# pangenome/sweepga

Hardware: AMD Instinct MI355X
Metric: PAF mappings/sec through plane-sweep+scaffold filter, 1/2/4/8 MI355X (higher is better)
Workload: dtype u32 coordinates, f64 scores; 1 GPU; BASELINE.json configs[3] (synthetic 100 M mappings across 10 k (q,t) groups, 100-genome pangenome shape; S-pan in SURVEY.md 8d): 100000000 mappings per GPU over 9900 genome-pair groups (100 single-chromosome genomes), pipeline=default; flags=(defaults), mappings_per_gpu=100000000, groups_per_gpu=9900

## Files before the change

### sweepga_amd/csrc/swg_chain.hip

```cpp
#include <cmath>
#include <type_traits>

#include "swg_scaffold_internal.h"

namespace swg_scaf {
namespace {

__global__ __launch_bounds__(EW) void sortA_keys_kernel(uint64_t M, const uint32_t* __restrict__ a_idx,
                                                        const uint32_t* __restrict__ q_id,
                                                        const uint32_t* __restrict__ t_id,
                                                        const uint8_t* __restrict__ strand,
                                                        const uint32_t* __restrict__ q_start, uint32_t n_seq,
                                                        int pos_bits, uint64_t* __restrict__ key) {
  uint64_t a = (uint64_t)swg_xcd_block(blockIdx.x, gridDim.x) * EW + threadIdx.x;
  if (a >= M) return;
  const uint32_t i = a_idx[a];
  const uint64_t g = ((uint64_t)q_id[i] * n_seq + t_id[i]) * 2 + (strand[i] ? 1 : 0);
  key[a] = (g << pos_bits) | q_start[i];
}

__global__ __launch_bounds__(EW) void sortA_words_kernel(uint64_t M, const uint32_t* __restrict__ a_idx,
                                                         const uint32_t* __restrict__ q_id, const uint32_t* __restrict__ t_id,
                                                         const uint8_t* __restrict__ strand, uint32_t n_seq, int idx_bits,
                                                         uint64_t* __restrict__ words,
// ... 1417 lines not shown
                ld = d;
                lj2 = j;
              }
            }
          }
          if (!__any(in)) break;
        }
        uint64_t cand = __ballot(lj2 != NONE);
        while (cand) {
          const int l = __builtin_ctzll(cand);
          cand &= cand - 1;
          const uint64_t d = readlane_u64(ld, l);
          const uint32_t j = readlane_u32(lj2, l);
          if (d < best_d || (d == best_d && j < best_j)) {
            best_d = d;
            best_j = j;
          }
        }
      }
      if (best_j == NONE) continue;
      const bool in_ring = best_j - base < (uint32_t)BIGW;
      if (lane == 0) {
        if (in_ring) ring[best_j % BIGW] = best_d;
        __hip_atomic_store(best_j < be ? &own[best_j] : &prev[best_j], best_d, __ATOMIC_RELAXED, __HIP_MEMORY_SCOPE_AGENT);
        (best_j < be ? pred_own : pred_prev)[best_j] = i;
      }
      if (!in_ring) __builtin_amdgcn_fence(__ATOMIC_RELEASE, "workgroup");
      }
    }
  }
}


static int walk_plain_knob() {
  const char* e = getenv("SWG_WALK_PLAIN");
  return e && e[0] == '1';
}

constexpr int WALK_HASH = 256;

__device__ __forceinline__ void wave_lds_sync() {
  __builtin_amdgcn_fence(__ATOMIC_RELEASE, "wavefront");
  __builtin_amdgcn_s_waitcnt(0xc07f);
  __builtin_amdgcn_wave_barrier();
  __builtin_amdgcn_fence(__ATOMIC_ACQUIRE, "wavefront");
}

template <int BIGW, bool FUSED, bool SPEC>
__global__ __launch_bounds__(64) void chain_walk_kernel(uint32_t n_blocks, const SpecBlock* __restrict__ desc, uint32_t m,
                                                        const uint64_t* __restrict__ s_grp,
                                                        const uint32_t* __restrict__ s_qs,
                                                        const uint32_t* __restrict__ s_qe,
                                                        const uint32_t* __restrict__ s_ts,
                                                        const uint32_t* __restrict__ s_te,
                                                        const uint32_t* __restrict__ s_gidx,
                                                        const uint32_t* __restrict__ group_begin, uint32_t n_groups,
                                                        uint64_t max_gap, const unsigned long long* __restrict__ c_d,
                                                        const uint32_t* __restrict__ c_j, const uint32_t* __restrict__ c_n,
                                                        unsigned long long* own, unsigned long long* prev,
                                                        uint32_t* __restrict__ pred_own, uint32_t* __restrict__ pred_prev,
                                                        unsigned long long* __restrict__ wstats,
                                                        const uint32_t* __restrict__ n_blocks_dev = nullptr,
                                                        const uint32_t* __restrict__ gate = nullptr,
                                                        int walk_plain_lists = 0) {
  constexpr bool spec = SPEC;
  if (gate && *gate == 0) return;
  if (n_blocks_dev) n_blocks = min(n_blocks, *n_blocks_dev);
  const bool pair_desc = s_gidx == nullptr;
  __shared__ unsigned long long ring[BIGW];
  __shared__ uint32_t rq[BIGW], rt[BIGW], re[BIGW];
  __shared__ uint32_t hcnt[WALK_HASH];
  __shared__ uint32_t hnum[WALK_HASH];
  __shared__ unsigned long long l_fd[64];
  __shared__ uint32_t l_fj[64];
  const int lane = threadIdx.x;
  const uint64_t INF = ~0ull;
  const uint64_t fifth = max_gap / 5;
  const uint32_t gap32 = max_gap > 0xffffffffull ? 0xffffffffu : (uint32_t)max_gap;
  const uint32_t fifth32 = fifth > 0xffffffffull ? 0xffffffffu : (uint32_t)fifth;
  const bool wrap = max_gap == ~0ull;
  const bool can_cut = max_gap < (uint64_t(1) << 31);
  const bool fast_keys = max_gap <= (uint64_t(1) << 22) && !walk_plain_lists;
  for (int k = lane; k < WALK_HASH; k += 64) {
    hcnt[k] = 0xffffffffu;
    hnum[k] = 0;
  }
  wave_lds_sync();
  for (uint32_t bk = blockIdx.x; bk < n_blocks; bk += gridDim.x) {
    const SpecBlock D = desc[bk];
    const uint32_t b = D.bb, be = D.be, ue = D.ue;
    if (be <= b || ue - b < 2) continue;
    if (!SPEC && pair_desc && be - b >= LABEL_CAP_ELEMS) continue;
    auto view_ptr = [&](uint32_t p) -> unsigned long long* { return (spec && p >= be) ? &prev[p] : &own[p]; };
    auto view_load = [&](uint32_t p) -> uint64_t {
      return __hip_atomic_load(view_ptr(p), __ATOMIC_RELAXED, __HIP_MEMORY_SCOPE_AGENT);
    };
    uint32_t base = b;
    bool far_any = SPEC;
    wave_lds_sync();
    for (uint32_t p = b + lane; p < b + BIGW; p += 64) {
      const bool ok = p < ue;
      ring[p % BIGW] = (ok && SPEC) ? view_load(p) : INF;
      rq[p % BIGW] = ok ? s_qs[p] : 0xffffffffu;
      rt[p % BIGW] = ok ? s_ts[p] : 0u;
      re[p % BIGW] = ok ? s_te[p] : 0u;
    }
    wave_lds_sync();
    auto current = [&](uint32_t j) -> uint64_t {
      if (j - base < (uint32_t)BIGW) return ring[j % BIGW];
      return far_any ? view_load(j) : INF;
    };
    struct Pre {
      uint64_t view;
      uint32_t q, t, e;
      uint64_t bd[KC];
      uint32_t bj[KC];
      uint32_t nv;
      uint32_t qe, ts, te, minus, ei;
    };
    auto prefetch = [&](uint32_t i0n, uint32_t base_n, bool refill) {
      Pre P;
      P.view = INF;
      P.q = 0xffffffffu;
      P.t = P.e = 0;
      if (refill) {
        const uint32_t pn = base_n + BIGW - 64 + lane;
        if (pn < ue) {
          if (far_any) P.view = view_load(pn);
          P.q = s_qs[pn];
          P.t = s_ts[pn];
          P.e = s_te[pn];
        }
      }
      const uint32_t i = i0n + lane;
      const bool valid = i < be && i + 1 < ue;
#pragma unroll
      for (int c = 0; c < KC; ++c) {
        P.bd[c] = INF;
        P.bj[c] = NONE;
      }
      P.nv = 0;
      P.qe = P.ts = P.te = P.minus = 0;
      P.ei = ue;
      if (valid) {
        if (!spec && !pair_desc) {
          const uint32_t g = s_gidx[i];
          const uint32_t ge = (g + 1 < n_groups) ? group_begin[g + 1] : m;
          if (ge < P.ei) P.ei = ge;
        }
        if (FUSED) {
          P.qe = s_qe[i];
          P.ts = s_ts[i];
          P.te = s_te[i];
          P.minus = pair_desc ? D.pad : (uint32_t)(s_grp[i] & 1ull);
        } else {
#pragma unroll
          for (int c = 0; c < KC; ++c) {
            P.bd[c] = c_d[(uint64_t)c * m + i];
            P.bj[c] = c_j[(uint64_t)c * m + i];
          }
          P.nv = c_n[i];
        }
      }
      return P;
    };
    Pre cur = prefetch(b, base, false);
    bool far_dirty = false;
    for (uint32_t i0 = b; i0 < be && i0 + 1 < ue; i0 += 64) {
      if (i0 != b) {
        const uint32_t pn = base + BIGW + lane;
        if (far_dirty && pn < ue) cur.view = view_load(pn);
        far_dirty = false;
        wave_lds_sync();
        ring[pn % BIGW] = cur.view;
        rq[pn % BIGW] = cur.q;
        rt[pn % BIGW] = cur.t;
        re[pn % BIGW] = cur.e;
        base += 64;
        wave_lds_sync();
      }
      const bool more = i0 + 64 < be && i0 + 65 < ue;
      Pre nxt = cur;
      if (more) nxt = prefetch(i0 + 64, base + 64, true);
      const uint32_t i = i0 + lane;
      const bool valid = i < be && i + 1 < ue;
      uint64_t bd[KC];
      uint32_t bj[KC];
      uint32_t nv = cur.nv;
#pragma unroll
      for (int c = 0; c < KC; ++c) {
        bd[c] = cur.bd[c];
        bj[c] = cur.bj[c];
      }
      const uint32_t e_i = cur.ei;
      bool listed = false;
      uint32_t j_next = i + 1;
      bool open_next = valid;
      if (FUSED && fast_keys) {
        const uint32_t qe_i = cur.qe;
        const bool minus = cur.minus != 0;
        const uint64_t bound64 = (uint64_t)qe_i + max_gap;
        const uint32_t bound = bound64 > 0xffffffffull ? 0xffffffffu : (uint32_t)bound64;
        const uint32_t r_i = minus ? cur.ts : cur.te;
        const uint32_t* r_ring = minus ? re : rt;
        const uint32_t e_ring = min(e_i, base + (uint32_t)BIGW);
        constexpr uint64_t KEY_INF = 0x7ff0000000000000ull, KEY_BIT = 1ull << 62;
        double kb[KC];
#pragma unroll
        for (int c = 0; c < KC; ++c) kb[c] = __longlong_as_double((long long)KEY_INF);
        uint32_t off = 1, cnt = 0, sl = ((i + 1) % BIGW) * 4u;
        const uint32_t off_end = e_ring > i ? e_ring - i : 0u;
        uint32_t gap_v = gap32, fifth_v = fifth32, key_hi = (uint32_t)(KEY_BIT >> 32);
        asm volatile("" : "+v"(gap_v), "+v"(fifth_v), "+v"(key_hi));
        const char* const rq_b = reinterpret_cast<const char*>(rq);
        const char* const rr_b = reinterpret_cast<const char*>(r_ring);
        bool open = valid;
        for (;;) {
          const bool in = open && off < off_end;
          if (__ballot(in) == 0ull) break;
          uint32_t qs_j = *reinterpret_cast<const uint32_t*>(rq_b + sl), r_j = *reinterpret_cast<const uint32_t*>(rr_b + sl);
          asm volatile("" : "+v"(qs_j), "+v"(r_j));
          const bool inw = in && qs_j <= bound;
          open = open && !(in && qs_j > bound);
          const uint32_t q_gap = absdiff_vv(qs_j, qe_i), r_gap = absdiff_vv(r_j, r_i);
          const uint32_t lim_q = qs_j < qe_i ? fifth_v : gap_v;
          const uint32_t lim_r = ((r_j > r_i) != minus) ? gap_v : fifth_v;
          const bool ok = inw && q_gap <= lim_q && r_gap <= lim_r;
          const uint32_t qa = q_gap << 8, ra = r_gap << 8;
          const uint64_t add = ((uint64_t)key_hi << 32) | off;
          uint64_t key = (uint64_t)qa * qa + ((uint64_t)ra * ra + add);
          key = ok ? key : KEY_INF;
          cnt += ok ? 1u : 0u;
          const uint32_t step = in ? 1u : 0u;
          off += step;
          sl = (sl + (step << 2)) & (BIGW * 4u - 1u);
          double t = __longlong_as_double((long long)key);
#pragma unroll
          for (int c = 0; c < KC; ++c) {
            double hi = t;
            if (c + 1 < KC) asm("v_max_f64 %0, %1, %2" : "=v"(hi) : "v"(kb[c]), "v"(t));
            asm("v_min_f64 %0, %0, %1" : "+v"(kb[c]) : "v"(t));
            t = hi;
          }
        }
        const uint32_t j = i + off;
        nv = cnt < (uint32_t)KC + 1u ? cnt : (uint32_t)KC + 1u;
#pragma unroll
        for (int c = 0; c < KC; ++c) {
          const uint64_t bits = (uint64_t)__double_as_longlong(kb[c]);
          const bool none = bits == KEY_INF;
          bd[c] = none ? INF : (bits & ~KEY_BIT) >> 16;
          bj[c] = none ? NONE : i + (uint32_t)(bits & 0xffffu);
        }
        listed = true;
        j_next = j;
        open_next = open;
      }
      if (FUSED && valid && (!listed || (open_next && j_next < e_i))) {
        const uint32_t qe_i = cur.qe;
        const bool minus = cur.minus != 0;
        const uint64_t bound64 = (uint64_t)qe_i + max_gap;
        const uint32_t bound = bound64 > 0xffffffffull ? 0xffffffffu : (uint32_t)bound64;
        const uint32_t r_i = minus ? cur.ts : cur.te;
        const uint32_t* r_ring = minus ? re : rt;
        const uint32_t* __restrict__ r_mem = minus ? s_te : s_ts;
        auto consider = [&](uint32_t j, uint32_t qs_j, uint32_t r_j) {
          const uint32_t q_gap = absdiff_vv(qs_j, qe_i), r_gap = absdiff_vv(r_j, r_i);
          const uint32_t lim_q = qs_j >= qe_i ? gap32 : fifth32;
          const uint32_t lim_r = (minus ? r_j <= r_i : r_j >= r_i) ? gap32 : fifth32;
          if ((q_gap > lim_q) | (r_gap > lim_r)) return;
          const uint64_t d = (uint64_t)q_gap * q_gap + (uint64_t)r_gap * r_gap;
          if (nv <= (uint32_t)KC) ++nv;
          if (d < bd[KC - 1]) {
            uint64_t cd = d;
            uint32_t cj = j;
            bool placed = false;
#pragma unroll
            for (int c = 0; c < KC; ++c) {
              if (placed || cd < bd[c]) {
                placed = true;
                const uint64_t td = bd[c];
                const uint32_t tj = bj[c];
                bd[c] = cd;
                bj[c] = cj;
                cd = td;
                cj = tj;
              }
            }
          }
        };
        const uint32_t e_ring = listed ? j_next : min(e_i, base + (uint32_t)BIGW);
        uint32_t j = j_next;
        bool open = true;
        for (; j < e_ring; ++j) {
          uint32_t qs_j = rq[j % BIGW], r_j = r_ring[j % BIGW];
          asm volatile("" : "+v"(qs_j), "+v"(r_j));
          if (qs_j > bound) {
            open = false;
            break;
          }
          consider(j, qs_j, r_j);
        }
        if (open)
          for (; j < e_i; ++j) {
            const uint32_t qs_j = s_qs[j];
            if (qs_j > bound) break;
            consider(j, qs_j, r_mem[j]);
          }
      }
      uint32_t acc = 0;
#pragma unroll
      for (int c = 0; c < KC; ++c)
        if ((uint32_t)c < nv && bd[c] < current(bj[c])) acc |= 1u << c;
      uint64_t fd = INF;
      uint32_t fj = NONE;
#pragma unroll
      for (int c = KC - 1; c >= 0; --c)
        if (acc & (1u << c)) {
          fd = bd[c];
          fj = bj[c];
        }
      constexpr bool PAIR_TEST = SPEC;
      const uint32_t hs = fj & (WALK_HASH - 1);
      if (fj != NONE) {
        atomicMin(&hcnt[hs], (uint32_t)lane);
        if (PAIR_TEST) atomicAdd(&hnum[hs], 1u);
      }
      if (PAIR_TEST) {
        l_fd[lane] = fd;
        l_fj[lane] = fj;
      }
      wave_lds_sync();
      bool shared_j = false;
      if (fj != NONE) {
        const uint32_t low = hcnt[hs];
        if (low != (uint32_t)lane) shared_j = !PAIR_TEST || hnum[hs] > 2u || (l_fj[low] == fj && (uint64_t)l_fd[low] <= fd);
      }
      wave_lds_sync();
      if (fj != NONE) {
        hcnt[hs] = 0xffffffffu;
        if (PAIR_TEST) hnum[hs] = 0;
      }
      uint64_t work = __ballot(shared_j || (fj == NONE && nv > (uint32_t)KC));
      if (wstats && lane == 0) {
        atomicAdd(&wstats[0], 1ull);
        atomicAdd(&wstats[1], (unsigned long long)__popcll(work));
      }
      uint32_t committed = 0;
      auto commit = [&](uint32_t upto) {
        const bool me = (uint32_t)lane >= committed && (uint32_t)lane < upto && fj != NONE;
        const bool inr = me && (fj - base < (uint32_t)BIGW);
        if (inr) atomicMin(&ring[fj % BIGW], (unsigned long long)fd);
        wave_lds_sync();
        if (inr && (uint64_t)ring[fj % BIGW] == fd) {
          ((spec && fj >= be) ? pred_prev : pred_own)[fj] = i;
          if (spec && fj >= be)
            __hip_atomic_store(&prev[fj], fd, __ATOMIC_RELAXED, __HIP_MEMORY_SCOPE_AGENT);
        }
        uint64_t far = __ballot(me && !inr);
        if (far) {
          far_dirty = true;
          if (!far_any) {
            for (uint32_t p = base + BIGW + lane; p < ue; p += 64) own[p] = INF;
            __threadfence();
            far_any = true;
          }
        }
        while (far) {
          const int l = __builtin_ctzll(far);
          far &= far - 1;
          if (lane == l) {
            const unsigned long long old = atomicMin(view_ptr(fj), (unsigned long long)fd);
            if (old > fd) ((spec && fj >= be) ? pred_prev : pred_own)[fj] = i;
          }
        }
        committed = upto;
      };
      while (work) {
        const int l = __builtin_ctzll(work);
        work &= work - 1;
        const uint32_t nv_l = readlane_u32(nv, l), acc_l = readlane_u32(acc, l);
        uint64_t nd = INF;
        uint32_t nj = NONE;
        const uint64_t lower = l ? (~0ull >> (64 - l)) : 0ull;
#pragma unroll
        for (int c = 0; c < KC; ++c) {
          if (nj == NONE && (acc_l & (1u << c))) {
            const uint64_t d = readlane_u64(bd[c], l);
            const uint32_t j = readlane_u32(bj[c], l);
            if ((__ballot(fj == j && fd <= d) & lower) == 0) {
              nd = d;
              nj = j;
            }
          }
        }
        if (nj == NONE && nv_l > (uint32_t)KC) {
          commit((uint32_t)l);
          if (wstats && lane == 0) atomicAdd(&wstats[2], 1ull);
          const uint32_t ii = i0 + l;
          const uint64_t qe_l = s_qe[ii], ts_l = s_ts[ii], te_l = s_te[ii];
          const bool minus_l = pair_desc ? D.pad != 0 : (s_grp[ii] & 1ull) != 0;
          const uint32_t e_l = readlane_u32(e_i, l);
          const uint64_t bound = qe_l + max_gap;
          uint64_t ld = INF;
          uint32_t lj2 = NONE;
          for (uint32_t j0 = ii + 1; j0 < e_l; j0 += 64) {
            if (wstats && lane == 0) atomicAdd(&wstats[3], 1ull);
            if (can_cut) {
              const uint64_t wmin = wave_min_u64(ld);
              const uint64_t q0 = (j0 - base) < (uint32_t)BIGW ? (uint64_t)rq[j0 % BIGW] : (uint64_t)s_qs[j0];
              if (wmin != INF && q0 >= qe_l && (q0 - qe_l) * (q0 - qe_l) >= wmin) break;
            }
            const uint32_t j = j0 + lane;
            bool in = j < e_l;
            const bool inring = in && (j - base) < (uint32_t)BIGW;
            uint64_t qs_j = 0;
            if (in) {
              qs_j = inring ? rq[j % BIGW] : s_qs[j];
              in = qs_j <= bound;
            }
            if (in) {
              uint64_t d;
              const uint64_t ts_j = inring ? rt[j % BIGW] : s_ts[j], te_j = inring ? re[j % BIGW] : s_te[j];
              if (chain_dist(minus_l, qe_l, ts_l, te_l, qs_j, ts_j, te_j, max_gap, fifth, &d)) {
                const uint64_t cur = current(j);
                if (d < cur && d < ld) {
                  ld = d;
                  lj2 = j;
                }
              }
            }
            if (!__any(in)) break;
          }
          uint64_t cand = __ballot(lj2 != NONE);
          while (cand) {
            const int c2 = __builtin_ctzll(cand);
            cand &= cand - 1;
            const uint64_t d = readlane_u64(ld, c2);
            const uint32_t j = readlane_u32(lj2, c2);
            if (d < nd || (d == nd && j < nj)) {
              nd = d;
              nj = j;
            }
          }
        }
        const uint32_t old_j = readlane_u32(fj, l);
        if (lane == l) {
          fd = nd;
          fj = nj;
        }
        if (nj != NONE && nj != old_j) {
          const uint64_t woken = __ballot(fj == nj && fd >= nd) & ~lower & ~(1ull << l);
          if (wstats && lane == 0) atomicAdd(&wstats[4], (unsigned long long)__popcll(woken & ~work));
          work |= woken;
        }
      }
      commit(64u);
      cur = nxt;
    }
  }
}


constexpr uint32_t PAIR_LONG_WINDOW_MAX = 512;
__global__ __launch_bounds__(EW) void pair_long_plan_kernel(uint32_t cap_long, const uint32_t* __restrict__ n_long_dev,
                                                            const uint32_t* __restrict__ long_list, const SpecBlock* __restrict__ chunks,
                                                            const uint32_t* __restrict__ s_qs, const uint32_t* __restrict__ s_qe,
                                                            uint64_t max_gap, SpecBlock* __restrict__ desc, uint32_t cap_spec,
                                                            uint32_t* __restrict__ counters ,
                                                            unsigned long long* __restrict__ ext, uint32_t* __restrict__ flags,
                                                            uint32_t fallback_bit) {
  __shared__ uint32_t wmaxs[EW / 64];
  __shared__ uint32_t sh_off;
  const uint32_t n_long = *n_long_dev < cap_long ? *n_long_dev : cap_long;
  for (uint32_t c = blockIdx.x; c < n_long; c += gridDim.x) {
    const SpecBlock D = chunks[long_list[c]];
    const uint32_t b = D.bb, e = D.be;
    uint32_t ml = 0;
    for (uint32_t p = b + threadIdx.x; p < e; p += EW) {
      const uint32_t len = s_qe[p] - s_qs[p];
      ml = len > ml ? len : ml;
      ext[p] = ~0ull;
    }
#pragma unroll
    for (int o = 32; o > 0; o >>= 1) {
      const uint32_t t = __shfl_xor(ml, o, 64);
      if (t > ml) ml = t;
    }
    __syncthreads();
    if ((threadIdx.x & 63) == 0) wmaxs[threadIdx.x >> 6] = ml;
    __syncthreads();
    for (int k = 0; k < EW / 64; ++k)
      if (wmaxs[k] > ml) ml = wmaxs[k];
    const uint64_t reach = (uint64_t)ml + (max_gap > (uint64_t(1) << 33) ? (uint64_t(1) << 33) : max_gap);
    uint32_t w = 0;
    for (uint32_t p0 = b + threadIdx.x * 64u; p0 < e; p0 += EW * 64u) {
      const uint32_t last = p0 + 63 < e ? p0 + 63 : e - 1;
      const uint64_t bound = (uint64_t)s_qs[last] + reach;
      uint32_t lo = last + 1, hi = e;
      while (lo < hi) {
        const uint32_t mid = lo + ((hi - lo) >> 1);
        if ((uint64_t)s_qs[mid] <= bound)
          lo = mid + 1;
        else
          hi = mid;
      }
      const uint32_t x = lo - 1 - p0;
      w = x > w ? x : w;
    }
#pragma unroll
    for (int o = 32; o > 0; o >>= 1) {
      const uint32_t t = __shfl_xor(w, o, 64);
      if (t > w) w = t;
    }
    __syncthreads();
    if ((threadIdx.x & 63) == 0) wmaxs[threadIdx.x >> 6] = w;
    __syncthreads();
    for (int k = 0; k < EW / 64; ++k)
      if (wmaxs[k] > w) w = wmaxs[k];
    if (w > PAIR_LONG_WINDOW_MAX) {
      if (threadIdx.x == 0) atomicOr(flags, fallback_bit);
      continue;
    }
    uint32_t S = ((w + 1 + 63) / 64) * 64;
    if (S < 512) S = 512;
    const uint32_t nb = (e - b + S - 1) / S;
    if (threadIdx.x == 0) sh_off = atomicAdd(&counters[0], nb);
    __syncthreads();
    const uint32_t off = sh_off;
    if (off + nb > cap_spec) {
      if (threadIdx.x == 0) counters[1] = 1;
      continue;
    }
    for (uint32_t k = threadIdx.x; k < nb; k += EW) {
      SpecBlock d;
      d.ue = e;
      d.bb = b + k * S;
      d.be = d.bb + S < e ? d.bb + S : e;
      d.pad = D.pad;
      desc[off + k] = d;
    }
  }
}
__global__ void pair_long_verdict_kernel(const uint32_t* __restrict__ counters, const uint32_t* __restrict__ changed_last,
                                         uint32_t* __restrict__ flags, uint32_t bit) {
  if (threadIdx.x == 0 && blockIdx.x == 0 && (counters[1] || *changed_last)) atomicOr(flags, bit);
}

__global__ __launch_bounds__(EW) void chunk_flag_kernel(uint32_t n_units, const uint32_t* __restrict__ unit_begin,
                                                        const uint8_t* __restrict__ is_big, uint8_t* __restrict__ flag) {
  uint32_t u = blockIdx.x * EW + threadIdx.x;
  if (u >= n_units) return;
  bool f = u == 0 || is_big[u] || is_big[u - 1];
  if (!f) f = unit_begin[u] / WALK_CHUNK != unit_begin[u - 1] / WALK_CHUNK;
// ... 927 lines not shown
```

### sweepga_amd/csrc/swg_chain_table.hip

```cpp
#include "swg_scaffold_internal.h"

namespace swg_scaf {
namespace {

__global__ __launch_bounds__(EW) void seg_compose_kernel(uint64_t m, const uint32_t* __restrict__ s_gidx,
                                                         const uint32_t* __restrict__ v, int complement,
                                                         uint64_t* __restrict__ out) {
  uint64_t p = (uint64_t)blockIdx.x * EW + threadIdx.x;
  if (p < m) out[p] = ((uint64_t)s_gidx[p] << 32) | (complement ? 0xffffffffu - v[p] : v[p]);
}
__global__ __launch_bounds__(EW) void group_first_from_scan_kernel(uint64_t m, const uint32_t* __restrict__ head_flag,
                                                                   const uint64_t* __restrict__ run_max,
                                                                   uint32_t* __restrict__ group_first) {
  uint64_t p = (uint64_t)blockIdx.x * EW + threadIdx.x;
  if (p >= m) return;
  if (p + 1 == m || head_flag[p + 1]) {
    const uint64_t v = run_max[p];
    group_first[(uint32_t)(v >> 32)] = 0xffffffffu - (uint32_t)v;
  }
}

constexpr int HEAD_SPAN = 1024;
__global__ __launch_bounds__(EW) void head_init_kernel(uint64_t m, const uint32_t* __restrict__ pred,
                                                       uint32_t* __restrict__ hd, const uint8_t* __restrict__ only,
// ... 183 lines not shown
    unsigned long long L[U];
    bool live[U];
    uint32_t first_i = 0xffffffffu;
    unsigned long long first_L = 0;
#pragma unroll
    for (int u = 0; u < U; ++u) {
      const uint64_t i = i0 + u;
      live[u] = i < n && alive[i] != 0;
      L[u] = live[u] ? ((unsigned long long)seq_genome[q_id[i]] << 32) | seq_genome[t_id[i]] : 0ull;
      if (live[u] && first_i == 0xffffffffu) {
        first_i = (uint32_t)i;
        first_L = L[u];
      }
    }
    uint32_t vmin = first_i;
#pragma unroll
    for (int o = 32; o > 0; o >>= 1) {
      const uint32_t x = __shfl_xor(vmin, o, 64);
      if (x < vmin) vmin = x;
    }
    if (vmin == 0xffffffffu) continue;
    const uint64_t holder = __ballot(first_i == vmin);
    const unsigned long long L0 = __shfl(first_L, __builtin_ctzll(holder), 64);
    bool same = true;
#pragma unroll
    for (int u = 0; u < U; ++u) same = same && (!live[u] || L[u] == L0);
    if (__all(same)) {
      if (lane == 0) {
        uint32_t* slot = pair_slot(table, (uint32_t)(L0 >> 32), (uint32_t)L0);
        if (*slot > vmin) atomicMin(slot, vmin);
      }
    } else {
#pragma unroll
      for (int u = 0; u < U; ++u)
        if (live[u]) {
          uint32_t* slot = pair_slot(table, (uint32_t)(L[u] >> 32), (uint32_t)L[u]);
          if (*slot > (uint32_t)(i0 + u)) atomicMin(slot, (uint32_t)(i0 + u));
        }
    }
  }
}

__global__ __launch_bounds__(EW) void genome_pair_first_groups_kernel(uint32_t n_groups, const uint32_t* __restrict__ group_begin,
                                                                      const uint32_t* __restrict__ s_idx,
                                                                      const uint32_t* __restrict__ group_first,
                                                                      const uint32_t* __restrict__ q_id,
                                                                      const uint32_t* __restrict__ t_id,
                                                                      const uint32_t* __restrict__ seq_genome, PairTable table) {
  uint32_t g = blockIdx.x * EW + threadIdx.x;
  if (g >= n_groups) return;
  const uint32_t i = s_idx[group_begin[g]];
  atomicMin(pair_slot(table, seq_genome[q_id[i]], seq_genome[t_id[i]]), group_first[g]);
}

__device__ __forceinline__ uint32_t heads_before(const uint32_t* __restrict__ ch_head, uint32_t nc, uint32_t p) {
  uint32_t l = 0, r = nc;
  while (l < r) {
    const uint32_t mid = l + ((r - l) >> 1);
    if (ch_head[mid] < p)
      l = mid + 1;
    else
      r = mid;
  }
  return l;
}
__global__ __launch_bounds__(EW) void group_keys_kernel(uint32_t n_groups, const uint32_t* __restrict__ group_begin,
                                                        uint32_t m, const uint32_t* __restrict__ ch_head, uint32_t nc,
                                                        const uint32_t* __restrict__ s_idx,
                                                        const uint32_t* __restrict__ group_first,
                                                        const uint32_t* __restrict__ q_id,
                                                        const uint32_t* __restrict__ t_id,
                                                        const uint32_t* __restrict__ seq_genome, bool pair_major,
                                                        PairTable gp_first, int idx_bits,
                                                        uint64_t* __restrict__ g_key, uint32_t* __restrict__ g_val,
                                                        uint32_t* __restrict__ g_first_chain,
                                                        uint32_t* __restrict__ g_nchains) {
  uint32_t g = blockIdx.x * EW + threadIdx.x;
  if (g >= n_groups) return;
  const uint32_t b = group_begin[g];
  const uint32_t first = heads_before(ch_head, nc, b);
  const uint32_t next = (g + 1 < n_groups) ? heads_before(ch_head, nc, group_begin[g + 1]) : nc;
  (void)m;
  g_first_chain[g] = first;
  g_nchains[g] = next - first;
  const uint32_t i = s_idx[b];
  uint64_t hi = 0;
  if (pair_major) hi = pair_get(gp_first, seq_genome[q_id[i]], seq_genome[t_id[i]]);
  g_key[g] = (hi << idx_bits) | group_first[g];
  g_val[g] = g;
}
__global__ __launch_bounds__(EW) void group_sizes_sorted_kernel(uint32_t n_groups, const uint32_t* __restrict__ g_sorted,
                                                                const uint32_t* __restrict__ g_nchains,
                                                                uint32_t* __restrict__ sizes) {
  uint32_t r = blockIdx.x * EW + threadIdx.x;
  if (r < n_groups) sizes[r] = g_nchains[g_sorted[r]];
}
__global__ __launch_bounds__(EW) void group_base_kernel(uint32_t n_groups, const uint32_t* __restrict__ g_sorted,
                                                        const uint32_t* __restrict__ base_sorted,
                                                        uint32_t* __restrict__ g_base) {
  uint32_t r = blockIdx.x * EW + threadIdx.x;
  if (r < n_groups) g_base[g_sorted[r]] = base_sorted[r];
}
__global__ __launch_bounds__(EW) void chain_place_kernel(uint64_t nc, const uint32_t* __restrict__ ch_head,
                                                         const uint32_t* __restrict__ s_gidx,
                                                         const uint32_t* __restrict__ g_first_chain,
                                                         const uint32_t* __restrict__ g_base, uint32_t* __restrict__ order) {
  uint64_t c = (uint64_t)blockIdx.x * EW + threadIdx.x;
  if (c >= nc) return;
  const uint32_t g = s_gidx[ch_head[c]];
  order[g_base[g] + ((uint32_t)c - g_first_chain[g])] = (uint32_t)c;
}

__global__ __launch_bounds__(EW) void chain_ok_kernel(uint64_t m, const uint32_t* __restrict__ is_head,
                                                      const uint32_t* __restrict__ s_qs, const uint32_t* __restrict__ h_qe,
                                                      const uint32_t* __restrict__ h_ts, const uint32_t* __restrict__ h_te,
                                                      const unsigned long long* __restrict__ h_sm,
                                                      const unsigned long long* __restrict__ h_sb,
                                                      const uint64_t* __restrict__ s_grp, uint64_t min_len,
                                                      double min_ident, uint8_t* __restrict__ ok_head,
                                                      HeadRec* __restrict__ rec, const uint8_t* __restrict__ only,
                                                      const uint8_t* __restrict__ span) {
  const uint64_t n_span = (m + HEAD_SPAN - 1) / HEAD_SPAN;
  for (uint64_t sp = blockIdx.x; sp < n_span; sp += gridDim.x) {
    if (span && !span[sp]) continue;
    for (int k = threadIdx.x; k < HEAD_SPAN; k += EW) {
      const uint64_t p = sp * HEAD_SPAN + k;
      if (p >= m) break;
      if (only && !only[p]) continue;
      bool ok = false;
      if (is_head[p] != 0) {
        const uint64_t total_length = (uint64_t)h_qe[p] - (uint64_t)s_qs[p];
        ok = total_length >= min_len;
        if (ok) {
          const double wid = chain_weighted_identity(total_length, h_sm[p], h_sb[p]);
          ok = wid >= min_ident;
          if (ok) {
            HeadRec hr;
            hr.qs = s_qs[p];
            hr.qe = h_qe[p];
            hr.ts = h_ts[p];
            hr.te = h_te[p];
            hr.wid = wid;
            hr.grp = s_grp[p];
            rec[p] = hr;
          }
        }
      }
      ok_head[p] = ok ? 1 : 0;
    }
  }
}

constexpr int LABEL_CAP = (int)(WALK_CHUNK + BIG_UNIT);
constexpr int LABEL_FAST = 1536;
constexpr int LABEL_NT = 512;
static_assert(LABEL_FAST * (2 + 2 + 3 * 4) >= LABEL_CAP * 2, "the two layouts share one LDS buffer");
template <int NT, bool MB>
__global__ __launch_bounds__(NT) void chain_label_kernel(uint32_t n_chunks, const SpecBlock* __restrict__ chunks,
                                                         const uint32_t* __restrict__ pred,
                                                         const uint32_t* __restrict__ s_qs, const uint32_t* __restrict__ s_qe,
                                                         const uint32_t* __restrict__ s_ts, const uint32_t* __restrict__ s_te,
                                                         const uint32_t* __restrict__ s_m, const uint32_t* __restrict__ s_b,
                                                         const uint64_t* __restrict__ s_grp,
                                                         uint64_t min_len, double min_ident, uint32_t* __restrict__ hd,
                                                         uint8_t* __restrict__ ok_head, HeadRec* __restrict__ rec,
                                                         unsigned long long* __restrict__ n_heads,
                                                         const uint32_t* __restrict__ n_chunks_dev = nullptr) {
  if (n_chunks_dev) n_chunks = min(n_chunks, *n_chunks_dev);
  __shared__ uint32_t lds[LABEL_FAST * (MB ? 6 : 4)];
  uint16_t* succ = reinterpret_cast<uint16_t*>(lds);
  uint16_t* l_hd = succ + LABEL_FAST;
  uint32_t* l_qe = lds + LABEL_FAST;
  uint32_t* l_ts = l_qe + LABEL_FAST;
  uint32_t* l_te = l_ts + LABEL_FAST;
  uint32_t* l_m = MB ? l_te + LABEL_FAST : nullptr;
  uint32_t* l_b = MB ? l_m + LABEL_FAST : nullptr;
  if (!MB) s_m = s_b = nullptr;
  constexpr uint16_t NO = 0xffffu;
  uint32_t heads = 0;
  for (uint32_t c = blockIdx.x; c < n_chunks; c += gridDim.x) {
    const uint32_t b = chunks[c].bb, e = chunks[c].be;
    uint32_t len = e > b ? e - b : 0;
    if (len >= (uint32_t)LABEL_CAP) len = 0;
    __syncthreads();
    for (uint32_t k = threadIdx.x; k < len; k += NT) succ[k] = NO;
    __syncthreads();
    if (len <= (uint32_t)LABEL_FAST) {
      constexpr int U = LABEL_FAST / NT;
      static_assert(LABEL_FAST % NT == 0, "whole rounds");
      uint32_t r_pr[U], r_qe[U], r_ts[U], r_te[U], r_m[U], r_b[U], r_qs[U];
#pragma unroll
      for (int u = 0; u < U; ++u) {
        const uint32_t k = (uint32_t)u * NT + threadIdx.x;
        const uint32_t p = b + (k < len ? k : 0u);
        r_pr[u] = pred[p];
        r_qe[u] = s_qe[p];
        r_ts[u] = s_ts[p];
        r_te[u] = s_te[p];
        r_m[u] = s_m ? s_m[p] : 0u;
        r_b[u] = s_m ? s_b[p] : 0u;
        r_qs[u] = s_qs[p];
      }
#pragma unroll
      for (int u = 0; u < U; ++u) {
        const uint32_t k = (uint32_t)u * NT + threadIdx.x;
        if (k < len) {
          if (r_pr[u] != NONE) succ[r_pr[u] - b] = (uint16_t)k;
          l_hd[k] = r_pr[u] != NONE ? NO : (uint16_t)k;
          l_qe[k] = r_qe[u];
          l_ts[k] = r_ts[u];
          l_te[k] = r_te[u];
          if constexpr (MB) {
            l_m[k] = r_m[u];
            l_b[k] = r_b[u];
          }
        }
      }
      __syncthreads();
#pragma unroll
      for (int u = 0; u < U; ++u) {
        const uint32_t k = (uint32_t)u * NT + threadIdx.x;
        if (k >= len) continue;
        const uint32_t p = b + k;
        if (r_pr[u] != NONE) {
          ok_head[p] = 0;
          continue;
        }
        ++heads;
        uint32_t qe = r_qe[u], ts = r_ts[u], te = r_te[u];
        uint64_t sm = r_m[u], sb = r_b[u];
        for (uint16_t nx = succ[k]; nx != NO; nx = succ[nx]) {
          const uint32_t a = l_qe[nx], t0 = l_ts[nx], t1 = l_te[nx];
          l_hd[nx] = (uint16_t)k;
          qe = a > qe ? a : qe;
          ts = t0 < ts ? t0 : ts;
          te = t1 > te ? t1 : te;
          if constexpr (MB) {
            sm += l_m[nx];
            sb += l_b[nx];
          }
        }
        const uint32_t qs0 = r_qs[u];
        const uint64_t total_length = (uint64_t)qe - (uint64_t)qs0;
        bool ok = total_length >= min_len;
        if (ok) {
          const double wid = chain_weighted_identity(total_length, sm, sb);
          ok = wid >= min_ident;
          if (ok) {
            HeadRec hr;
            hr.qs = qs0;
            hr.qe = qe;
            hr.ts = ts;
            hr.te = te;
            hr.wid = wid;
            hr.grp = s_grp ? s_grp[p] : 0ull;
            rec[p] = hr;
          }
        }
        ok_head[p] = ok ? (uint8_t)(s_grp ? 1u : 1u | (qs0 < qe ? 2u : 0u) | (ts < te ? 4u : 0u)) : (uint8_t)0;
      }
      __syncthreads();
      for (uint32_t k = threadIdx.x; k < len; k += NT) hd[b + k] = b + l_hd[k];
      continue;
    }
    constexpr int LB = 2048 / NT;
    for (uint32_t k0 = 0; k0 < len; k0 += NT * LB) {
      uint32_t pr[LB];
#pragma unroll
      for (int u = 0; u < LB; ++u) {
        const uint32_t k = k0 + (uint32_t)u * NT + threadIdx.x;
        pr[u] = pred[b + (k < len ? k : 0u)];
      }
#pragma unroll
      for (int u = 0; u < LB; ++u) {
        const uint32_t k = k0 + (uint32_t)u * NT + threadIdx.x;
        if (k < len && pr[u] != NONE) succ[pr[u] - b] = (uint16_t)k;
      }
    }
    __syncthreads();
    for (uint32_t k0 = 0; k0 < len; k0 += NT * LB) {
      uint32_t pr[LB], v_qs[LB], v_qe[LB], v_ts[LB], v_te[LB], v_m[LB], v_b[LB];
#pragma unroll
      for (int u = 0; u < LB; ++u) {
        const uint32_t k = k0 + (uint32_t)u * NT + threadIdx.x;
        const uint32_t p = b + (k < len ? k : 0u);
        pr[u] = pred[p];
        v_qs[u] = s_qs[p];
        v_qe[u] = s_qe[p];
        v_ts[u] = s_ts[p];
        v_te[u] = s_te[p];
        v_m[u] = s_m ? s_m[p] : 0u;
        v_b[u] = s_m ? s_b[p] : 0u;
      }
#pragma unroll
      for (int u = 0; u < LB; ++u) {
        const uint32_t k = k0 + (uint32_t)u * NT + threadIdx.x;
        if (k >= len) continue;
        const uint32_t p = b + k;
        if (pr[u] != NONE) {
          ok_head[p] = 0;
          continue;
        }
        ++heads;
        hd[p] = p;
        uint32_t qe = v_qe[u], ts = v_ts[u], te = v_te[u];
        uint64_t sm = v_m[u], sb = v_b[u];
        for (uint16_t nx = succ[k]; nx != NO;) {
          const uint32_t q = b + nx;
          const uint16_t nn = succ[nx];
          const uint32_t a = s_qe[q], t0 = s_ts[q], t1 = s_te[q], mm = s_m ? s_m[q] : 0u, bb = s_m ? s_b[q] : 0u;
          hd[q] = p;
          qe = a > qe ? a : qe;
          ts = t0 < ts ? t0 : ts;
          te = t1 > te ? t1 : te;
          sm += mm;
          sb += bb;
          nx = nn;
        }
        const uint32_t qs0 = v_qs[u];
        const uint64_t total_length = (uint64_t)qe - (uint64_t)qs0;
        bool ok = total_length >= min_len;
        if (ok) {
          const double wid = chain_weighted_identity(total_length, sm, sb);
          ok = wid >= min_ident;
          if (ok) {
            HeadRec hr;
            hr.qs = qs0;
            hr.qe = qe;
            hr.ts = ts;
            hr.te = te;
            hr.wid = wid;
            hr.grp = s_grp ? s_grp[p] : 0ull;
            rec[p] = hr;
          }
        }
        ok_head[p] = ok ? (uint8_t)(s_grp ? 1u : 1u | (qs0 < qe ? 2u : 0u) | (ts < te ? 4u : 0u)) : (uint8_t)0;
      }
    }
  }
#pragma unroll
  for (int o = 32; o > 0; o >>= 1) heads += __shfl_down(heads, o, 64);
  __syncthreads();
  if ((threadIdx.x & 63) == 0) lds[threadIdx.x >> 6] = heads;
  __syncthreads();
  if (threadIdx.x == 0) {
    uint32_t all = 0;
    for (int w = 0; w < NT / 64; ++w) all += lds[w];
    if (all) atomicAdd(n_heads, (unsigned long long)all);
  }
}
__global__ __launch_bounds__(1024) void chain_label_long_kernel(uint32_t cap_long, const uint32_t* __restrict__ n_long_dev,
                                                                const uint32_t* __restrict__ long_list,
                                                                const SpecBlock* __restrict__ chunks, const uint32_t* __restrict__ pred,
                                                                const uint32_t* __restrict__ s_qs, const uint32_t* __restrict__ s_qe,
                                                                const uint32_t* __restrict__ s_ts, const uint32_t* __restrict__ s_te,
                                                                const uint32_t* __restrict__ s_m, const uint32_t* __restrict__ s_b,
                                                                uint64_t min_len, double min_ident, uint32_t* hd,
                                                                uint8_t* __restrict__ ok_head, HeadRec* rec,
                                                                unsigned long long* __restrict__ n_heads) {
  __shared__ uint32_t changed;
  const uint32_t n_long = *n_long_dev < cap_long ? *n_long_dev : cap_long;
  uint32_t heads = 0;
  for (uint32_t c = blockIdx.x; c < n_long; c += gridDim.x) {
    const SpecBlock D = chunks[long_list[c]];
    const uint32_t b = D.bb, e = D.be;
    for (uint32_t p = b + threadIdx.x; p < e; p += 1024) {
      const uint32_t pr = pred[p];
      hd[p] = pr == NONE ? p : pr;
      if (pr == NONE) {
        HeadRec hr;
        hr.qs = s_qs[p];
        hr.qe = s_qe[p];
        hr.ts = s_ts[p];
        hr.te = s_te[p];
        hr.wid = __longlong_as_double((long long)(unsigned long long)(s_m ? s_b[p] : 0u));
        hr.grp = s_m ? s_m[p] : 0u;
        rec[p] = hr;
      }
    }
    for (;;) {
      __syncthreads();
      if (threadIdx.x == 0) changed = 0;
      __syncthreads();
      bool ch = false;
      for (uint32_t p = b + threadIdx.x; p < e; p += 1024) {
        const uint32_t h = __hip_atomic_load(&hd[p], __ATOMIC_RELAXED, __HIP_MEMORY_SCOPE_WORKGROUP);
        const uint32_t hh = __hip_atomic_load(&hd[h], __ATOMIC_RELAXED, __HIP_MEMORY_SCOPE_WORKGROUP);
        if (hh != h) {
          __hip_atomic_store(&hd[p], hh, __ATOMIC_RELAXED, __HIP_MEMORY_SCOPE_WORKGROUP);
          ch = true;
        }
      }
      if (ch) changed = 1;
      __syncthreads();
      if (!changed) break;
    }
    for (uint32_t p = b + threadIdx.x; p < e; p += 1024) {
      const uint32_t h = hd[p];
      if (h == p) continue;
      ok_head[p] = 0;
      atomicMax(&rec[h].qe, s_qe[p]);
      atomicMin(&rec[h].ts, s_ts[p]);
      atomicMax(&rec[h].te, s_te[p]);
      if (s_m) {
        atomicAdd(reinterpret_cast<unsigned long long*>(&rec[h].wid), (unsigned long long)s_b[p]);
        atomicAdd(reinterpret_cast<unsigned long long*>(&rec[h].grp), (unsigned long long)s_m[p]);
      }
    }
    __syncthreads();
    for (uint32_t p = b + threadIdx.x; p < e; p += 1024) {
      if (hd[p] != p) continue;
      ++heads;
      const HeadRec hr = rec[p];
      const uint64_t sb = (uint64_t)__double_as_longlong(hr.wid), sm = hr.grp;
      const uint64_t total_length = (uint64_t)hr.qe - (uint64_t)hr.qs;
      bool ok = total_length >= min_len;
      if (ok) {
        const double wid = chain_weighted_identity(total_length, sm, sb);
        ok = wid >= min_ident;
        if (ok) {
          rec[p].wid = wid;
          rec[p].grp = 0;
        }
      }
      ok_head[p] = ok ? (uint8_t)(1u | (hr.qs < hr.qe ? 2u : 0u) | (hr.ts < hr.te ? 4u : 0u)) : (uint8_t)0;
    }
  }
#pragma unroll
  for (int o = 32; o > 0; o >>= 1) heads += __shfl_down(heads, o, 64);
  if ((threadIdx.x & 63) == 0 && heads) atomicAdd(n_heads, (unsigned long long)heads);
}
__global__ __launch_bounds__(EW) void chain_columns_kernel(
    uint64_t nc, const uint32_t* __restrict__ order, const uint32_t* __restrict__ ch_head, const HeadRec* __restrict__ rec,
    const uint32_t* __restrict__ s_a,
    const uint32_t* __restrict__ a_dpair, uint32_t n_seq,
    uint32_t* __restrict__ C_qid, uint32_t* __restrict__ C_tid, uint32_t* __restrict__ C_qs,
    uint32_t* __restrict__ C_qe, uint32_t* __restrict__ C_ts, uint32_t* __restrict__ C_te,
    double* __restrict__ C_wid, uint8_t* __restrict__ C_strand, uint32_t* __restrict__ C_dpair,
    uint32_t* __restrict__ rank_of_poschain, uint32_t* __restrict__ head_of_chain) {
  uint64_t c2 = (uint64_t)blockIdx.x * EW + threadIdx.x;
  if (c2 >= nc) return;
  const uint32_t c = order[c2];
  rank_of_poschain[c] = (uint32_t)c2;
  const uint32_t p = ch_head[c];
  head_of_chain[c2] = p;
  const HeadRec hr = rec[p];
  const uint64_t g = hr.grp;
  const uint64_t pair = g >> 1;
  const uint32_t qs = hr.qs, qe = hr.qe, ts = hr.ts, te = hr.te;
  C_qid[c2] = (uint32_t)(pair / n_seq);
  C_tid[c2] = (uint32_t)(pair % n_seq);
  C_strand[c2] = (uint8_t)(g & 1);
  C_qs[c2] = qs;
  C_qe[c2] = qe;
  C_ts[c2] = ts;
  C_te[c2] = te;
  C_dpair[c2] = a_dpair[s_a ? s_a[p] : p];
  C_wid[c2] = hr.wid;
}

__global__ __launch_bounds__(EW) void survivor_chain_kernel(uint64_t m, const uint32_t* __restrict__ hd,
                                                            const uint8_t* __restrict__ ok_head,
                                                            const uint32_t* __restrict__ ch_head, uint32_t nc,
                                                            const uint32_t* __restrict__ rank_of_poschain,
                                                            uint32_t* __restrict__ s_chain) {
  uint64_t p = (uint64_t)blockIdx.x * EW + threadIdx.x;
  if (p >= m) return;
  const uint32_t h = hd[p];
  s_chain[p] = ok_head[h] ? rank_of_poschain[heads_before(ch_head, nc, h)] : NONE;
}

}

int pair_table_make(swg_ctx* ctx, uint32_t n_genome, uint64_t bound, PairTable* t) {
  hipStream_t st = ctx->stream;
  t->n_genome = n_genome;
  t->dense = nullptr;
  t->keys = nullptr;
  t->vals = nullptr;
  t->mask = 0;
  const uint64_t g2 = (uint64_t)n_genome * n_genome;
  if (g2 <= DENSE_PAIR_LIMIT) {
    t->dense = swg_alloc<uint32_t>(ctx, g2);
    SWG_CHECK_ARENA(ctx);
    SWG_HIP(ctx, hipMemsetAsync(t->dense, 0xff, g2 * sizeof(uint32_t), st));
    return SWG_OK;
  }
  uint64_t cap = 1024;
  while (cap < 2 * bound) cap <<= 1;
  if (cap > (uint64_t(1) << 32)) return swg_set_error(ctx, SWG_ERR_RANGE, "genome-pair table beyond 2^32 slots");
  t->keys = swg_alloc<unsigned long long>(ctx, cap);
  t->vals = swg_alloc<uint32_t>(ctx, cap);
  SWG_CHECK_ARENA(ctx);
  t->mask = (uint32_t)(cap - 1);
  SWG_LAUNCH(ctx, "fill", fill_u64_kernel<<<nblk(cap), EW, 0, st>>>(cap, reinterpret_cast<uint64_t*>(t->keys), ~0ull));
  SWG_KERNEL_CHECK(ctx);
  SWG_LAUNCH(ctx, "fill", fill_u32_kernel<<<nblk(cap), EW, 0, st>>>(cap, t->vals, NONE));
  SWG_KERNEL_CHECK(ctx);
  return SWG_OK;
}

int chain_table_build(swg_ctx* ctx, const swg_records* r, const uint8_t* alive, uint64_t min_len, double min_ident,
                      bool genome_pair_major, ChainBuild* out, const ChainWork& W) {
  const uint64_t n = r->n;
  hipStream_t st = ctx->stream;
  ChainBuild& B = *out;
  const uint64_t m = B.m, n_groups = W.n_groups;
  uint32_t *s_qs = W.s_qs, *s_qe = W.s_qe, *s_ts = W.s_ts, *s_te = W.s_te, *s_m = W.s_m, *s_b = W.s_b;
  uint64_t* s_grp = W.s_grp;
  uint32_t *head_flag = W.head_flag, *s_gidx = W.s_gidx, *group_begin = W.group_begin, *pred = W.pred;
  uint64_t* d_tot = W.d_tot;
  uint32_t* hd = swg_alloc<uint32_t>(ctx, m);
  uint32_t* h_qe = swg_alloc<uint32_t>(ctx, m);
  uint32_t* h_ts = swg_alloc<uint32_t>(ctx, m);
  uint32_t* h_te = swg_alloc<uint32_t>(ctx, m);
  unsigned long long* h_sm = swg_alloc<unsigned long long>(ctx, m);
  unsigned long long* h_sb = swg_alloc<unsigned long long>(ctx, m);
  uint32_t* is_head = swg_alloc<uint32_t>(ctx, m);
  uint32_t* group_first = swg_alloc<uint32_t>(ctx, n_groups);
  PairTable gp_first;
  uint32_t* changed = swg_alloc<uint32_t>(ctx, 2);
  SWG_CHECK_ARENA(ctx);
  HeadRec* head_rec = swg_alloc<HeadRec>(ctx, m);
  uint8_t* ok_head = swg_alloc<uint8_t>(ctx, m);
  SWG_CHECK_ARENA(ctx);
  SWG_HIP(ctx, hipMemsetAsync(d_tot + 1, 0, 8, st));
  unsigned long long* n_heads = reinterpret_cast<unsigned long long*>(d_tot + 1);
  const uint8_t* only = nullptr;
  const uint8_t* span = nullptr;
  bool generic = true;
  if (W.n_chunks) {
    static const uint64_t lper = getenv("SWG_LABEL_BLOCKS") ? (uint64_t)atoi(getenv("SWG_LABEL_BLOCKS")) : 128;
    const uint64_t lb = W.n_chunks < (uint64_t)ctx->num_cu * lper ? W.n_chunks : (uint64_t)ctx->num_cu * lper;
    if (s_m)
      SWG_LAUNCH(ctx, "chain_label", chain_label_kernel<LABEL_NT, true><<<(unsigned)lb, LABEL_NT, 0, st>>>((uint32_t)W.n_chunks, W.chunks, pred, s_qs, s_qe, s_ts, s_te,
                                                                        s_m, s_b, s_grp, min_len, min_ident, hd, ok_head, head_rec, n_heads));
    else
      SWG_LAUNCH(ctx, "chain_label", chain_label_kernel<LABEL_NT, false><<<(unsigned)lb, LABEL_NT, 0, st>>>((uint32_t)W.n_chunks, W.chunks, pred, s_qs, s_qe, s_ts, s_te,
                                                                        s_m, s_b, s_grp, min_len, min_ident, hd, ok_head, head_rec, n_heads));
    SWG_KERNEL_CHECK(ctx);
    only = W.big_member;
    span = W.span_big;
    generic = only != nullptr;
  }
  if (generic) {
    const uint64_t n_span_all = (m + HEAD_SPAN - 1) / HEAD_SPAN;
    const unsigned span_grid = (unsigned)(n_span_all < (uint64_t)ctx->num_cu * 16 ? n_span_all : (uint64_t)ctx->num_cu * 16);
    SWG_LAUNCH(ctx, "head_init", head_init_kernel<<<span_grid, EW, 0, st>>>(m, pred, hd, only, span));
    SWG_KERNEL_CHECK(ctx);
    for (int round = 0; round < 64; ++round) {
      SWG_HIP(ctx, hipMemsetAsync(changed, 0, 8, st));
      SWG_LAUNCH(ctx, "head_jump", head_jump_kernel<<<span_grid, EW, 0, st>>>(m, hd, changed, only, span));
      SWG_KERNEL_CHECK(ctx);
      SWG_LAUNCH(ctx, "head_jump", head_jump_kernel<<<span_grid, EW, 0, st>>>(m, hd, changed, only, span));
      SWG_KERNEL_CHECK(ctx);
      uint64_t ch = 0;
      SWG_TRY(swg_read_scalars(ctx, reinterpret_cast<uint64_t*>(changed), &ch, 1));
      if ((uint32_t)ch == 0) break;
    }
    SWG_LAUNCH(ctx, "chain_aggregate_init", chain_aggregate_init_kernel<<<span_grid, EW, 0, st>>>(m, hd, s_qe, s_ts, s_te, s_m, s_b, h_qe, h_ts,
                                                                                    h_te, h_sm, h_sb, is_head, only, span, n_heads));
    SWG_KERNEL_CHECK(ctx);
    SWG_LAUNCH(ctx, "chain_aggregate", chain_aggregate_kernel<<<span_grid, EW, 0, st>>>(
                                           m, hd, s_qe, s_ts, s_te, s_m, s_b, h_qe, h_ts, h_te, h_sm, h_sb, only, span));
    SWG_KERNEL_CHECK(ctx);
    SWG_LAUNCH(ctx, "chain_ok", chain_ok_kernel<<<span_grid, EW, 0, st>>>(
                                    m, is_head, s_qs, h_qe, h_ts, h_te, h_sm, h_sb, s_grp, min_len, min_ident, ok_head, head_rec, only, span));
    SWG_KERNEL_CHECK(ctx);
  }
  swg_flag_scan ok_scan;
  SWG_TRY(swg_flags_count(ctx, ok_head, m, &ok_scan, d_tot));
  uint64_t h2[2];
  SWG_TRY(swg_read_scalars(ctx, d_tot, h2, 2));
  const uint64_t nc = h2[0];
  B.n_chains_all = h2[1];
  B.T.nc = nc;
  if (nc == 0) return SWG_OK;
  SWG_LAUNCH(ctx, "fill", fill_u32_kernel<<<nblk(n_groups), EW, 0, st>>>(n_groups, group_first, NONE));
  SWG_KERNEL_CHECK(ctx);
  SWG_TRY(pair_table_make(ctx, r->n_genome_last, B.n_pairs, &gp_first));
  if (m / n_groups > 8192) {
    swg_arena_mark mk = swg_arena_save(ctx);
    uint64_t* comp = swg_alloc<uint64_t>(ctx, m);
    SWG_CHECK_ARENA(ctx);
    SWG_LAUNCH(ctx, "seg_compose", seg_compose_kernel<<<nblk(m), EW, 0, st>>>(m, s_gidx, B.s_idx, 1, comp));
    SWG_KERNEL_CHECK(ctx);
    SWG_TRY(swg_inclusive_max_scan_u64(ctx, comp, comp, m));
    SWG_LAUNCH(ctx, "group_first_from_scan", group_first_from_scan_kernel<<<nblk(m), EW, 0, st>>>(m, head_flag, comp, group_first));
    swg_arena_restore(ctx, mk);
  } else {
    uint64_t blocks = (n_groups + 3) / 4;
    const uint64_t max_blocks = (uint64_t)ctx->num_cu * 16;
    if (blocks > max_blocks) blocks = max_blocks;
    SWG_LAUNCH(ctx, "group_first", group_first_kernel<<<(unsigned)blocks, EW, 0, st>>>((uint32_t)n_groups, group_begin, (uint32_t)m,
                                                                               B.s_idx, group_first));
  }
  SWG_KERNEL_CHECK(ctx);
  if (B.m == B.M) {
    SWG_LAUNCH(ctx, "genome_pair_first_groups", genome_pair_first_groups_kernel<<<nblk(n_groups), EW, 0, st>>>(
                                             (uint32_t)n_groups, group_begin, B.s_idx, group_first, r->q_id, r->t_id,
                                             r->seq_genome_last, gp_first));
  } else {
    SWG_LAUNCH(ctx, "genome_pair_first", genome_pair_first_kernel<<<ctx->num_cu * 8, EW, 0, st>>>(n, alive, r->q_id, r->t_id,
                                                                                      r->seq_genome_last, gp_first));
  }
  SWG_KERNEL_CHECK(ctx);
  uint32_t* ch_head = swg_alloc<uint32_t>(ctx, nc);
  SWG_CHECK_ARENA(ctx);
  SWG_TRY(swg_flags_compact(ctx, ok_scan, ch_head));
  uint32_t* order = swg_alloc<uint32_t>(ctx, nc);
  uint32_t* rank_of = swg_alloc<uint32_t>(ctx, nc);
  uint32_t* head_of_chain = swg_alloc<uint32_t>(ctx, nc);
  uint64_t* g_key = swg_alloc<uint64_t>(ctx, n_groups);
  uint64_t* g_key_tmp = swg_alloc<uint64_t>(ctx, n_groups);
  uint32_t* g_sorted = swg_alloc<uint32_t>(ctx, n_groups);
  uint32_t* g_sorted_tmp = swg_alloc<uint32_t>(ctx, n_groups);
  uint32_t* g_first_chain = swg_alloc<uint32_t>(ctx, n_groups);
  uint32_t* g_nchains = swg_alloc<uint32_t>(ctx, n_groups);
  uint32_t* g_sizes = swg_alloc<uint32_t>(ctx, n_groups);
  uint32_t* g_base = swg_alloc<uint32_t>(ctx, n_groups);
  ChainTable& T = B.T;
  T.nc = nc;
  T.qid = swg_alloc<uint32_t>(ctx, nc);
  T.tid = swg_alloc<uint32_t>(ctx, nc);
  T.qs = swg_alloc<uint32_t>(ctx, nc);
  T.qe = swg_alloc<uint32_t>(ctx, nc);
  T.ts = swg_alloc<uint32_t>(ctx, nc);
  T.te = swg_alloc<uint32_t>(ctx, nc);
  T.wid = swg_alloc<double>(ctx, nc);
  B.C_strand = swg_alloc<uint8_t>(ctx, nc);
  B.C_dpair = swg_alloc<uint32_t>(ctx, nc);
  SWG_CHECK_ARENA(ctx);
  const int idx_bits = swg_bits_for(n) ? swg_bits_for(n) : 1;
  const unsigned gblk = nblk(n_groups);
  SWG_LAUNCH(ctx, "group_keys", group_keys_kernel<<<gblk, EW, 0, st>>>((uint32_t)n_groups, group_begin, (uint32_t)m, ch_head, (uint32_t)nc,
                                                           B.s_idx, group_first, r->q_id, r->t_id, r->seq_genome_last,
                                                           genome_pair_major, gp_first, idx_bits, g_key, g_sorted, g_first_chain,
                                                           g_nchains));
  SWG_KERNEL_CHECK(ctx);
  SWG_TRY(swg_radix_sort_pairs(ctx, &g_key, &g_sorted, &g_key_tmp, &g_sorted_tmp, n_groups, 0, 2 * idx_bits));
  SWG_LAUNCH(ctx, "group_sizes_sorted", group_sizes_sorted_kernel<<<gblk, EW, 0, st>>>((uint32_t)n_groups, g_sorted, g_nchains, g_sizes));
  SWG_KERNEL_CHECK(ctx);
  SWG_TRY(swg_exclusive_scan_u32(ctx, g_sizes, g_sizes, n_groups, nullptr));
  SWG_LAUNCH(ctx, "group_base", group_base_kernel<<<gblk, EW, 0, st>>>((uint32_t)n_groups, g_sorted, g_sizes, g_base));
  SWG_KERNEL_CHECK(ctx);
  SWG_LAUNCH(ctx, "chain_place", chain_place_kernel<<<nblk(nc), EW, 0, st>>>(nc, ch_head, s_gidx, g_first_chain, g_base, order));
  SWG_KERNEL_CHECK(ctx);
  SWG_LAUNCH(ctx, "chain_columns", chain_columns_kernel<<<nblk(nc), EW, 0, st>>>(
                                       nc, order, ch_head, head_rec, B.s_a, B.a_dpair,
                                       r->n_seq, T.qid, T.tid, T.qs, T.qe, T.ts, T.te, T.wid, B.C_strand, B.C_dpair, rank_of, head_of_chain));
  SWG_KERNEL_CHECK(ctx);
  B.m_head_of_chain = head_of_chain;
  B.m_hd = hd;
  B.m_ok_head = ok_head;
  B.m_rank_of = rank_of;
  if (B.want_s_chain) {
    SWG_LAUNCH(ctx, "survivor_chain", survivor_chain_kernel<<<nblk(m), EW, 0, st>>>(m, hd, ok_head, ch_head, (uint32_t)nc, rank_of, B.s_chain));
    SWG_KERNEL_CHECK(ctx);
  }
  return SWG_OK;
}

int pair_label_launch(swg_ctx* ctx, uint32_t cap_chunks, const uint32_t* n_chunks_dev, const SpecBlock* chunks, const uint32_t* pred,
                      const uint32_t* s_qs, const uint32_t* s_qe, const uint32_t* s_ts, const uint32_t* s_te, const uint32_t* s_m,
                      const uint32_t* s_b, uint64_t min_len, double min_ident, uint32_t* hd, uint8_t* ok_head, HeadRec* rec,
                      unsigned long long* n_heads) {
  if (cap_chunks == 0) return SWG_OK;
  static const uint64_t lper = getenv("SWG_LABEL_BLOCKS") ? (uint64_t)atoi(getenv("SWG_LABEL_BLOCKS")) : 128;
  const uint64_t lb = cap_chunks < (uint64_t)ctx->num_cu * lper ? cap_chunks : (uint64_t)ctx->num_cu * lper;
  if (s_m)
    SWG_LAUNCH(ctx, "chain_label", chain_label_kernel<LABEL_NT, true><<<(unsigned)lb, LABEL_NT, 0, ctx->stream>>>(cap_chunks, chunks, pred, s_qs, s_qe, s_ts, s_te, s_m, s_b,
                                                                             nullptr, min_len, min_ident, hd, ok_head, rec, n_heads,
                                                                             n_chunks_dev));
  else
    SWG_LAUNCH(ctx, "chain_label", chain_label_kernel<LABEL_NT, false><<<(unsigned)lb, LABEL_NT, 0, ctx->stream>>>(cap_chunks, chunks, pred, s_qs, s_qe, s_ts, s_te, s_m, s_b,
                                                                             nullptr, min_len, min_ident, hd, ok_head, rec, n_heads,
                                                                             n_chunks_dev));
  SWG_KERNEL_CHECK(ctx);
  return SWG_OK;
}

int pair_label_long_launch(swg_ctx* ctx, hipStream_t st, uint32_t cap_long, const uint32_t* n_long_dev, const uint32_t* long_list, const SpecBlock* chunks,
                           const uint32_t* pred, const uint32_t* s_qs, const uint32_t* s_qe, const uint32_t* s_ts, const uint32_t* s_te,
                           const uint32_t* s_m, const uint32_t* s_b, uint64_t min_len, double min_ident, uint32_t* hd, uint8_t* ok_head,
                           HeadRec* rec, unsigned long long* n_heads) {
  if (cap_long == 0) return SWG_OK;
  swg_on_stream on(ctx, st);
  const unsigned lg = cap_long < (uint32_t)ctx->num_cu * 2 ? cap_long : (unsigned)ctx->num_cu * 2;
  SWG_LAUNCH(ctx, "chain_label_long", chain_label_long_kernel<<<lg, 1024, 0, st>>>(cap_long, n_long_dev, long_list, chunks, pred, s_qs, s_qe, s_ts,
                                                                       s_te, s_m, s_b, min_len, min_ident, hd, ok_head, rec, n_heads));
  SWG_KERNEL_CHECK(ctx);
  return SWG_OK;
}

}
```

### sweepga_amd/csrc/swg_pair.hip

```cpp
#include <cmath>
#include <type_traits>

#include "swg_scaffold_internal.h"

namespace swg_scaf {
namespace {

constexpr uint32_t PAIR_CELL = WALK_CHUNK;
constexpr uint32_t PAIR_S_MAX = 1024, PAIR_M_MAX = 4096, PAIR_L_MAX = 32768, PAIR_XL_MAX = uint32_t(1) << 18;
constexpr uint32_t PAIR_XL_CELLS = PAIR_XL_MAX / PAIR_CELL;
constexpr uint32_t PAIR_HASH_MAX = 65536;
constexpr uint32_t PAIR_MX_MAX = 16384, PAIR_MX_CUT_DEFAULT = 8192;
constexpr uint32_t ORDER_BIN_L = 128;
constexpr uint32_t ORDERED = 0x80000000u;
constexpr uint32_t PF_NOT_GROUPED = 1, PF_RUN_OVERFLOW = 2, PF_TOO_LONG = 4, PF_FALLBACK = 8;

struct PairRun {
  uint32_t a, n;
};
struct PairInfo {
  uint32_t m;
  uint32_t m_plus;
  uint32_t M;
  uint32_t first_alive;
// ... 229 lines not shown
  const uint32_t lo = cls == 2 ? PAIR_M_MAX : PAIR_L_MAX;
  const uint32_t bw = cls == 2 ? ORDER_BIN_L : (PAIR_XL_MAX - PAIR_L_MAX) / (uint32_t)ORDER_BINS;
  uint32_t* const t = tmp + (size_t)blockIdx.x * cap_tmp;
  auto bin_of = [&](uint32_t len) -> uint32_t {
    const uint32_t b = (len - lo - 1u) / bw;
    return (uint32_t)ORDER_BINS - 1u - (b < (uint32_t)ORDER_BINS ? b : (uint32_t)ORDER_BINS - 1u);
  };
  const uint32_t cut_bin = (uint32_t)ORDER_BINS - (cut > lo ? (cut - lo) / bw : 0u);
  for (int b = tid; b < ORDER_BINS; b += ORDER_NT) bin_at[b] = 0u;
  __syncthreads();
  for (uint32_t i = tid; i < cnt; i += ORDER_NT) {
    const uint32_t k = list[i];
    t[i] = k;
    atomicAdd(&bin_at[bin_of(runs[k].n)], 1u);
  }
  __syncthreads();
  if (tid < 64) {
    constexpr int PER = ORDER_BINS / 64;
    uint32_t v[PER], s = 0;
#pragma unroll
    for (int j = 0; j < PER; ++j) {
      v[j] = bin_at[tid * PER + j];
      s += v[j];
    }
    uint32_t inc = s;
#pragma unroll
    for (int d = 1; d < 64; d <<= 1) {
      const uint32_t x = __shfl_up(inc, d, 64);
      if (tid >= d) inc += x;
    }
    uint32_t o = inc - s;
#pragma unroll
    for (int j = 0; j < PER; ++j) {
      if (cls == 2 && (uint32_t)(tid * PER + j) == cut_bin) C->n_above = ORDERED | o;
      bin_at[tid * PER + j] = o;
      o += v[j];
    }
    if (cls == 2 && cut_bin == (uint32_t)ORDER_BINS && tid == 63) C->n_above = ORDERED | o;
  }
  __syncthreads();
  for (uint32_t i = tid; i < cnt; i += ORDER_NT) {
    const uint32_t k = t[i];
    list[atomicAdd(&bin_at[bin_of(runs[k].n)], 1u)] = k;
  }
}

__global__ __launch_bounds__(256) void pair_hash_kernel(uint32_t n, const uint32_t* __restrict__ q_id, const uint32_t* __restrict__ t_id,
                                                        unsigned long long* __restrict__ table, uint32_t tmask,
                                                        uint32_t* __restrict__ count, uint32_t* __restrict__ slot_of) {
  const uint32_t i = blockIdx.x * 256u + threadIdx.x;
  if (i >= n) return;
  const unsigned long long key = (((unsigned long long)q_id[i] << 32) | t_id[i]) + 1ull;
  uint32_t h = (uint32_t)((key * 0x9e3779b97f4a7c15ull) >> 32) & tmask;
  for (;;) {
    unsigned long long old = __hip_atomic_load(&table[h], __ATOMIC_RELAXED, __HIP_MEMORY_SCOPE_AGENT);
    if (old == 0ull) {
      old = atomicCAS(&table[h], 0ull, key);
      if (old == 0ull) old = key;
    }
    if (old == key) break;
    h = (h + 1) & tmask;
  }
  slot_of[i] = h;
  atomicAdd(&count[h], 1u);
}
__global__ __launch_bounds__(256) void pair_slots_kernel(uint32_t tsize, const uint32_t* __restrict__ count, uint32_t* __restrict__ start,
                                                         PairRun* __restrict__ runs, uint32_t* __restrict__ class_list, uint32_t cap,
                                                         PairCounters* __restrict__ C, uint32_t* __restrict__ cursor) {
  const uint32_t h = blockIdx.x * 256u + threadIdx.x;
  const uint32_t c = h < tsize ? count[h] : 0u;
  if (!c) return;
  const uint32_t k = atomicAdd(&C->n_runs, 1u), o = atomicAdd(cursor, c);
  start[h] = o;
  if (k >= cap) {
    atomicOr(&C->flags, PF_RUN_OVERFLOW);
    return;
  }
  PairRun r;
  r.a = o;
  r.n = c;
  runs[k] = r;
  if (c > PAIR_L_MAX) {
    atomicOr(&C->flags, PF_TOO_LONG);
  } else {
    const int cls = c <= PAIR_S_MAX ? 0 : (c <= PAIR_M_MAX ? 1 : 2);
    class_list[(size_t)cls * cap + atomicAdd(&C->n_class[cls], 1u)] = k;
  }
}
__global__ __launch_bounds__(256) void pair_perm_kernel(uint32_t n, const uint32_t* __restrict__ slot_of, uint32_t* __restrict__ start,
                                                        uint32_t* __restrict__ perm) {
  const uint32_t i = blockIdx.x * 256u + threadIdx.x;
  if (i < n) perm[atomicAdd(&start[slot_of[i]], 1u)] = i;
}

struct BucketMap {
  uint32_t kmin[2];
  float scale[2];
  uint32_t off[2], nb[2];
};
__device__ __forceinline__ void bucket_map_make(BucketMap& B, uint32_t nbk, uint32_t m0, uint32_t m1, const uint32_t* kmin,
                                                const uint32_t* kmax) {
  const uint32_t m = m0 + m1;
  uint32_t nb0 = m ? (uint32_t)(((uint64_t)nbk * m0) / m) : 0u;
  if (m0 && nb0 == 0) nb0 = 1;
  if (m1 && nb0 >= nbk) nb0 = nbk - 1;
  B.nb[0] = nb0;
  B.nb[1] = nbk - nb0;
  B.off[0] = 0;
  B.off[1] = nb0;
#pragma unroll
  for (int s = 0; s < 2; ++s) {
    B.kmin[s] = kmin[s];
    const float range = (float)(kmax[s] - kmin[s]) + 1.0f;
    B.scale[s] = (float)B.nb[s] / range;
  }
#pragma unroll
  for (int s = 0; s < 2; ++s) {
    B.kmin[s] = (uint32_t)__builtin_amdgcn_readfirstlane((int)B.kmin[s]);
    B.scale[s] = __int_as_float(__builtin_amdgcn_readfirstlane(__float_as_int(B.scale[s])));
    B.off[s] = (uint32_t)__builtin_amdgcn_readfirstlane((int)B.off[s]);
    B.nb[s] = (uint32_t)__builtin_amdgcn_readfirstlane((int)B.nb[s]);
  }
}
__device__ __forceinline__ uint32_t bucket_of(const BucketMap& B, uint32_t st, uint32_t k) {
  const uint32_t kmin = st ? B.kmin[1] : B.kmin[0], nb = st ? B.nb[1] : B.nb[0], off = st ? B.off[1] : B.off[0];
  const float scale = st ? B.scale[1] : B.scale[0];
  const float f = (float)(k - kmin) * scale;
  uint32_t b = (uint32_t)f;
  const uint32_t top = nb - 1u;
  b = b < top ? b : top;
  return off + b;
}

struct PairSortArgs {
  const uint32_t *q_id, *t_id, *q_start, *q_end, *t_start, *t_end, *matches, *block_len;
  const double* identity;
  const uint8_t* strand;
  const uint8_t *alive_in, *member_in;
  uint64_t min_block;
  int keep_self;
  double min_identity;
  int check_degenerate;
  uint64_t max_gap;
  const PairRun* runs;
  const uint32_t* list;
  const uint32_t* perm;
  const uint32_t* orig;
  uint8_t* code;
  uint32_t *s_qs, *s_qe, *s_ts, *s_te, *s_m, *s_b, *s_idx, *pred;
  PairInfo* info;
  SpecBlock* chunks;
  uint32_t cap_chunks;
  int chunks_by_place;
  uint32_t* long_list;
  uint32_t cap_long;
  PairCounters* C;
  PairTable gl_first;
  const uint32_t* seq_genome_last;
};

__device__ __forceinline__ void emit_chunks(const PairSortArgs& A, uint32_t rk_run, uint32_t a, uint32_t m, uint32_t m_plus, const uint32_t* cellmin, int n_cell) {
  const int lane = threadIdx.x & 63;
  const unsigned long long below = (1ull << lane) - 1ull;
  uint32_t n_start = 0, n_lt = 0, before_mp = NONE, last = NONE;
  bool mp_is_start = false;
  for (int c0 = 0; c0 < n_cell; c0 += 64) {
    const uint32_t v = c0 + lane < n_cell ? cellmin[c0 + lane] : NONE;
    const unsigned long long mask = __ballot(v != NONE);
    if (!mask) continue;
    const unsigned long long lt = __ballot(v != NONE && v < m_plus);
    mp_is_start |= __ballot(v == m_plus) != 0ull;
    n_start += (uint32_t)__popcll(mask);
    n_lt += (uint32_t)__popcll(lt);
    if (lt) before_mp = (uint32_t)__shfl((int)v, 63 - __clzll(lt), 64);
    last = (uint32_t)__shfl((int)v, 63 - __clzll(mask), 64);
  }
  const bool mp_ins = m_plus > 0 && m_plus < m && !mp_is_start;
  const uint32_t count = n_start + (mp_ins ? 1u : 0u);
  if (count == 0) return;
  auto begin_of = [&](uint32_t v, unsigned long long mask, uint32_t carry) -> uint32_t {
    const unsigned long long lower = mask & below;
    const uint32_t pv = (uint32_t)__shfl((int)v, lower ? 63 - __clzll(lower) : 0, 64);
    uint32_t b = lower ? pv : carry;
    if (mp_ins && m_plus < v && (b == NONE || b < m_plus)) b = m_plus;
    return b;
  };
  const bool mp_chunk = mp_ins && before_mp != NONE;
  const bool mp_long = mp_chunk && m_plus - before_mp >= LABEL_CAP_ELEMS;
  const uint32_t last_b = mp_ins && (last == NONE || last < m_plus) ? m_plus : last;
  const bool last_long = m - last_b >= LABEL_CAP_ELEMS;
  uint32_t n_long = (mp_long ? 1u : 0u) + (last_long ? 1u : 0u), n_long_lt = 0;
  {
    uint32_t carry = NONE;
    for (int c0 = 0; c0 < n_cell; c0 += 64) {
      const uint32_t v = c0 + lane < n_cell ? cellmin[c0 + lane] : NONE;
      const unsigned long long mask = __ballot(v != NONE);
      if (!mask) continue;
      const uint32_t b = begin_of(v, mask, carry);
      const bool lf = v != NONE && b != NONE && v - b >= LABEL_CAP_ELEMS;
      n_long += (uint32_t)__popcll(__ballot(lf));
      n_long_lt += (uint32_t)__popcll(__ballot(lf && v < m_plus));
      carry = (uint32_t)__shfl((int)v, 63 - __clzll(mask), 64);
    }
  }
  uint32_t slot = 0, lslot = 0;
  if (lane == 0) {
    slot = A.chunks_by_place ? a / PAIR_CELL + 2u * rk_run : atomicAdd(&A.C->n_chunks, count);
    lslot = n_long ? atomicAdd(&A.C->n_long, n_long) : 0u;
  }
  slot = (uint32_t)__shfl((int)slot, 0, 64);
  lslot = (uint32_t)__shfl((int)lslot, 0, 64);
  if (slot + count > A.cap_chunks || (n_long && lslot + n_long > A.cap_long)) {
    if (lane == 0) atomicOr(&A.C->flags, PF_FALLBACK);
    return;
  }
  auto emit = [&](uint32_t k, uint32_t b, uint32_t e, bool is_long, uint32_t lpos) {
    SpecBlock d;
    d.bb = a + b;
    d.be = a + e;
    d.ue = d.be;
    d.pad = b >= m_plus ? 1u : 0u;
    if (is_long) A.long_list[lslot + lpos] = slot + k;
    A.chunks[slot + k] = d;
  };
  uint32_t carry = NONE, base = 0, lbase = 0;
  for (int c0 = 0; c0 < n_cell; c0 += 64) {
    const uint32_t v = c0 + lane < n_cell ? cellmin[c0 + lane] : NONE;
    const unsigned long long mask = __ballot(v != NONE);
    if (!mask) continue;
    const uint32_t b = begin_of(v, mask, carry);
    const bool lf = v != NONE && b != NONE && v - b >= LABEL_CAP_ELEMS;
    const unsigned long long lmask = __ballot(lf);
    if (v != NONE && b != NONE) {
      const uint32_t k = base + (uint32_t)__popcll(mask & below) + (mp_ins && v > m_plus ? 1u : 0u) - 1u;
      emit(k, b, v, lf, lbase + (uint32_t)__popcll(lmask & below) + (mp_long && v > m_plus ? 1u : 0u));
    }
    base += (uint32_t)__popcll(mask);
    lbase += (uint32_t)__popcll(lmask);
    carry = (uint32_t)__shfl((int)v, 63 - __clzll(mask), 64);
  }
  if (lane == 0) {
    if (mp_chunk) emit(n_lt - 1u, before_mp, m_plus, mp_long, n_long_lt);
    emit(count - 1u, last_b, m, last_long, n_long - 1u);
  }
}
template <int NT, int E>
__device__ __forceinline__ void unit_starts(const uint32_t (&qs)[E], const uint32_t (&qe)[E], uint32_t mb, uint32_t base, uint32_t m_plus,
                                            uint64_t max_gap, uint64_t* ws64, uint32_t* cellmin, uint64_t* carry_max) {
  const uint32_t p0 = (uint32_t)threadIdx.x * E;
  uint64_t tmax = 0;
#pragma unroll
  for (int e = 0; e < E; ++e)
    if (p0 + e < mb) {
      const uint64_t c = ((uint64_t)(base + p0 + e >= m_plus ? 1u : 0u) << 32) | qe[e];
      tmax = c > tmax ? c : tmax;
    }
  uint64_t tot;
  uint64_t prev = block_excl_max<NT>(tmax, ws64, &tot);
  prev = prev > *carry_max ? prev : *carry_max;
#pragma unroll
  for (int e = 0; e < E; ++e)
    if (p0 + e < mb) {
      const uint32_t pa = base + p0 + e;
      uint64_t lim = (prev & 0xffffffffull) + max_gap;
      if (lim < max_gap) lim = ~0ull;
      if (pa == 0 || pa == m_plus || (uint64_t)qs[e] > lim) atomicMin(&cellmin[pa / PAIR_CELL], pa);
      const uint64_t c = ((uint64_t)(pa >= m_plus ? 1u : 0u) << 32) | qe[e];
      prev = c > prev ? c : prev;
    }
  *carry_max = tot > *carry_max ? tot : *carry_max;
}
template <int E>
__device__ __forceinline__ void read_block(const uint32_t* lds, uint32_t (&out)[E]) {
  static_assert(E % 4 == 0, "whole 16-byte reads");
  const uint4* v = reinterpret_cast<const uint4*>(lds) + (size_t)threadIdx.x * (E / 4);
#pragma unroll
  for (int j = 0; j < E / 4; ++j) {
    const uint4 x = v[j];
    out[4 * j] = x.x;
    out[4 * j + 1] = x.y;
    out[4 * j + 2] = x.z;
    out[4 * j + 3] = x.w;
  }
}

#ifdef SWG_PAIR_TIMING
__device__ unsigned long long g_pair_t[16];
#define PT_STAMP(k) do { __syncthreads(); if (threadIdx.x == 0) { const unsigned long long t_ = wall_clock64(); atomicAdd(&g_pair_t[k], t_ - pt_last); pt_last = t_; } } while (0)
#define FT_STAMP(k) do { __syncthreads(); if (threadIdx.x == 0) { const unsigned long long t_ = wall_clock64(); atomicAdd(&g_fin_t[k], t_ - pt_last); pt_last = t_; } } while (0)
__device__ unsigned long long g_fin_t[16];
#else
#define PT_STAMP(k) do { } while (0)
#define FT_STAMP(k) do { } while (0)
#endif
constexpr size_t lds_align_up(size_t off, size_t align) { return (off + align - 1) / align * align; }
template <int NT, int ES, int ER, int NBK, int NBIN, bool PERM>
constexpr size_t pair_sort_lds_bytes() {
  return (size_t)NT * ES * (PERM ? 10 : 8) + (size_t)NBK * 4 + (size_t)NBIN * 4 + 17 * 4 + (size_t)((NT * ER + PAIR_CELL - 1) / PAIR_CELL) * 4 +
         (size_t)(NT / 64 + 1) * 12 + 16 * 4 + 128;
}
template <int NT, int ES, int ER, int NBK, int NBIN, bool PERM>
__device__ __forceinline__ void pair_sort_body(const PairSortArgs& A, const uint32_t rk_run, char* lds_raw) {
  using IT = typename std::conditional<PERM, uint32_t, uint16_t>::type;
  constexpr int CAP = NT * ES, NREC = NT * ER, MAXB = 16, H = 8;
  constexpr int NCELL = (NREC + (int)PAIR_CELL - 1) / (int)PAIR_CELL;
  static_assert(ER <= 32 && ER % H == 0 && ES % 4 == 0 && NREC <= 65536, "record masks are 32 bits wide, indices 16");
  static_assert(NBIN >= 2 && NBIN <= 4096, "each strand needs a coarse bin of its own (the members are ordered strand first)");
  constexpr size_t O_K = 0, O_I = O_K + (size_t)CAP * 4, O_RR = O_I + (size_t)CAP * sizeof(IT), O_CNT = lds_align_up(O_RR + (size_t)CAP * 2, 4),
                   O_BINS = O_CNT + (size_t)NBK * 4, O_BLO = O_BINS + (size_t)NBIN * 4, O_CELL = O_BLO + (size_t)(MAXB + 1) * 4,
                   O_WS64 = lds_align_up(O_CELL + (size_t)NCELL * 4, 8), O_WS = O_WS64 + (size_t)(NT / 64 + 1) * 8,
                   O_SH = O_WS + (size_t)(NT / 64 + 1) * 4;
  static_assert(O_SH + 13 * 4 <= pair_sort_lds_bytes<NT, ES, ER, NBK, NBIN, PERM>(), "LDS block of the work-group");
  static_assert(O_CNT - O_I >= (size_t)CAP * 4 && O_I % 16 == 0, "B1 holds CAP words, read 16 bytes at a time");
  uint32_t* const K = reinterpret_cast<uint32_t*>(lds_raw + O_K);
  IT* const I = reinterpret_cast<IT*>(lds_raw + O_I);
  uint16_t* const RR = reinterpret_cast<uint16_t*>(lds_raw + O_RR);
  uint32_t* const B0 = K;
  uint32_t* const B1 = reinterpret_cast<uint32_t*>(lds_raw + O_I);
  uint32_t* const cnt = reinterpret_cast<uint32_t*>(lds_raw + O_CNT);
  uint32_t* const bins = reinterpret_cast<uint32_t*>(lds_raw + O_BINS);
  uint32_t* const b_lo = reinterpret_cast<uint32_t*>(lds_raw + O_BLO);
  uint32_t* const cellmin = reinterpret_cast<uint32_t*>(lds_raw + O_CELL);
  uint64_t* const ws64 = reinterpret_cast<uint64_t*>(lds_raw + O_WS64);
  uint32_t* const ws = reinterpret_cast<uint32_t*>(lds_raw + O_WS);
  uint32_t* const sh_cnt = reinterpret_cast<uint32_t*>(lds_raw + O_SH);
  uint32_t* const sh_kmin = sh_cnt + 4;
  uint32_t* const sh_kmax = sh_cnt + 6;
  uint32_t* const sh_first = sh_cnt + 8;
  uint32_t& sh_nb = sh_cnt[11];
  uint32_t& sh_bad = sh_cnt[12];
#ifdef SWG_PAIR_TIMING
  unsigned long long pt_last = wall_clock64();
#endif
  const int tid = threadIdx.x;
  const PairRun run = A.runs[rk_run];
  const uint32_t a = run.a, n = run.n;
  if (n > (uint32_t)NREC) {
    if (tid == 0) atomicOr(&A.C->flags, PF_FALLBACK);
    return;
  }
  if (tid < 4) sh_cnt[tid] = 0;
  if (tid < 2) {
    sh_kmin[tid] = 0xffffffffu;
    sh_kmax[tid] = 0;
  }
  if (tid < 3) sh_first[tid] = NONE;
  if (tid == 0) sh_bad = 0;
  for (int c = tid; c < NCELL; c += NT) cellmin[c] = NONE;
  for (int b = tid; b < NBIN; b += NT) bins[b] = 0;
  lds_barrier();
  auto fresh_tid = [&]() -> uint32_t {
    uint32_t t = (uint32_t)tid;
    asm volatile("" : "+v"(t));
    return t;
  };
  uint32_t tid_v = (uint32_t)tid, n_v = n;
  auto rec_index = [&](int e) -> uint32_t {
    const uint32_t li = tid_v + (uint32_t)e * NT;
    const uint32_t lc = li < n_v ? li : 0u;
    return PERM ? A.perm[a + lc] : lc;
  };
  const uint32_t cb = PERM ? 0u : a;
  const uint32_t* c_qs = A.q_start + cb;
  const uint32_t* c_qe = A.q_end + cb;
  const uint32_t* c_ts = A.t_start + cb;
  const uint32_t* c_te = A.t_end + cb;
  const uint32_t* c_m = A.matches + cb;
  const uint32_t* c_b = A.block_len + cb;
  const uint8_t* c_st = A.strand + cb;
  const double* c_id = A.identity ? A.identity + cb : nullptr;
  const uint8_t* c_alive = A.alive_in ? A.alive_in + cb : nullptr;
  const uint8_t* c_member = A.member_in ? A.member_in + cb : nullptr;
  uint32_t* o_qs = A.s_qs + a;
  uint32_t* o_qe = A.s_qe + a;
// ... 786 lines not shown
          const uint32_t hi = cnt[b], lo = b ? cnt[b - 1] : 0u;
          uint32_t r = lo;
          for (uint32_t x = lo; x < hi; ++x) {
            const uint32_t kx = K[x], lx = I[x];
            r += (kx < k || (kx == k && lx < li)) ? 1u : 0u;
          }
          rk[e] = k;
          rl[e] = li;
          rr[e] = r;
        }
      }
      __syncthreads();
#pragma unroll
      for (int e = 0; e < E; ++e)
        if (rr[e] != NONE) {
          K[rr[e]] = rk[e];
          I[rr[e]] = rl[e];
        }
    }
    __syncthreads();
    PT_STAMP(6);
    {
      uint32_t li[E], qe[E], ts[E], te[E], mm[E], bb[E];
#pragma unroll
      for (int e = 0; e < E; ++e) {
        const uint32_t p = (uint32_t)tid + (uint32_t)e * NT;
        li[e] = p < mb ? I[p] : 0u;
      }
#pragma unroll
      for (int e = 0; e < E; ++e) {
        const uint32_t i = a + li[e];
        qe[e] = A.q_end[i];
        ts[e] = A.t_start[i];
        te[e] = A.t_end[i];
        mm[e] = A.s_m ? A.matches[i] : 0u;
        bb[e] = A.s_m ? A.block_len[i] : 0u;
      }
#pragma unroll
      for (int e = 0; e < E; ++e) {
        const uint32_t p = (uint32_t)tid + (uint32_t)e * NT;
        if (p >= mb) continue;
        const uint32_t o = a + base + p, qs = K[p];
        QE[p] = qe[e];
        A.s_qs[o] = qs;
        A.s_idx[o] = a + li[e];
        A.pred[o] = NONE;
        A.s_qe[o] = qe[e];
        A.s_ts[o] = ts[e];
        A.s_te[o] = te[e];
        if (A.s_m) {
          A.s_m[o] = mm[e];
          A.s_b[o] = bb[e];
        }
        degenerate |= qs >= qe[e] || ts[e] >= te[e];
      }
    }
    __syncthreads();
    PT_STAMP(7);
    {
      uint32_t qs_r[E], qe_r[E];
      read_block<E>(K, qs_r);
      read_block<E>(QE, qe_r);
      unit_starts<NT, E>(qs_r, qe_r, mb, base, m_plus, A.max_gap, ws64, cellmin, &carry_max);
    }
    base += mb;
    __syncthreads();
    PT_STAMP(8);
  }
  if (A.check_degenerate && __any(degenerate) && (tid & 63) == 0) atomicOr(&A.C->flags, PF_FALLBACK);
  if (tid < 64) emit_chunks(A, rk_run, a, m, m_plus, cellmin, (int)PAIR_XL_CELLS);
  PT_STAMP(9);
}

template <int NT, int ES, int ER, int NBK, int NBIN, bool PERM>
__global__ __launch_bounds__(NT) void pair_sort_kernel(PairSortArgs A) {
  __shared__ __attribute__((aligned(16))) char raw[pair_sort_lds_bytes<NT, ES, ER, NBK, NBIN, PERM>()];
  pair_sort_body<NT, ES, ER, NBK, NBIN, PERM>(A, A.list[blockIdx.x], raw);
}
template <>
__global__ __launch_bounds__(512) __attribute__((amdgpu_waves_per_eu(4))) void pair_sort_kernel<512, 16, 32, 2048, 1024, false>(PairSortArgs A) {
  __shared__ __attribute__((aligned(16))) char raw[pair_sort_lds_bytes<512, 16, 32, 2048, 1024, false>()];
  pair_sort_body<512, 16, 32, 2048, 1024, false>(A, A.list[blockIdx.x], raw);
}
static_assert(2 * pair_sort_lds_bytes<512, 16, 32, 2048, 1024, false>() <= 160 * 1024, "two work-groups in the LDS of a CU");
constexpr size_t PAIR_BIG_LDS = pair_sort_lds_bytes<1024, 16, 32, 4096, 1024, false>() > pair_sort_xl_lds_bytes<1024, 8, 4096>()
                                    ? pair_sort_lds_bytes<1024, 16, 32, 4096, 1024, false>()
                                    : pair_sort_xl_lds_bytes<1024, 8, 4096>();
static_assert(PAIR_BIG_LDS <= 160 * 1024, "LDS of a CU");
__global__ __launch_bounds__(1024) void pair_sort_big_kernel(PairSortArgs A, const uint32_t* __restrict__ list_xl, uint32_t n_xl) {
  __shared__ __attribute__((aligned(16))) char raw[PAIR_BIG_LDS];
  if (blockIdx.x < n_xl)
    pair_sort_xl_body<1024, 8, 4096>(A, list_xl[blockIdx.x], raw);
  else
    pair_sort_body<1024, 16, 32, 4096, 1024, false>(A, A.list[blockIdx.x - n_xl], raw);
}

__global__ __launch_bounds__(1024) void pair_totals_kernel(uint32_t n_runs, const PairInfo* __restrict__ info, const PairSum* __restrict__ sum,
                                                           const uint32_t* __restrict__ n_out_pair, PairCounters* __restrict__ C) {
  __shared__ unsigned long long part[16][4];
  unsigned long long v[4] = {0, 0, 0, 0};
  const bool finished = !(C->flags & PF_FALLBACK);
  for (uint32_t k = blockIdx.x * 1024u + threadIdx.x; k < n_runs; k += gridDim.x * 1024u) {
    const PairInfo pi = info[k];
    v[0] += pi.M;
    v[1] += pi.m;
    if (finished) {
      v[2] += pi.M ? sum[k].n_kept : 0u;
      v[3] += n_out_pair[k];
    }
  }
#pragma unroll
  for (int j = 0; j < 4; ++j) {
#pragma unroll
    for (int o = 32; o > 0; o >>= 1) v[j] += __shfl_xor(v[j], o, 64);
    if ((threadIdx.x & 63) == 0) part[threadIdx.x >> 6][j] = v[j];
  }
  __syncthreads();
  if (threadIdx.x < 4) {
    unsigned long long t = 0;
    for (int w = 0; w < 16; ++w) t += part[w][threadIdx.x];
    unsigned long long* dst = threadIdx.x == 0 ? &C->n_alive : threadIdx.x == 1 ? &C->n_members : threadIdx.x == 2 ? &C->n_kept : &C->n_out;
    if (t) atomicAdd(dst, t);
  }
}
__global__ void pair_gate_kernel(PairCounters* __restrict__ C) {
  if (threadIdx.x == 0 && (C->flags & PF_FALLBACK)) {
    C->n_chunks = 0u;
    C->n_long = 0u;
  }
}

struct PairFinishArgs {
  const PairRun* runs;
  const uint32_t* list;
  const uint32_t* list_xl;
  uint32_t n_xl;
  const PairInfo* info;
  PairSum* sum;
  const uint32_t *s_qs, *s_qe, *s_ts, *s_te, *s_idx, *hd;
  const uint8_t* ok_head;
  const HeadRec* rec;
  uint32_t* head_num;
  uint32_t *f_qs, *f_qe, *f_ts, *f_pm;
  uint8_t* status;
  uint32_t* chain;
  int scaffolds_only;
  uint64_t gap;
  uint64_t max_dev;
  uint64_t rescue_d;
  uint64_t max_s2;
  const uint8_t* kept_in;
  const uint32_t* chain_base;
  const uint32_t* np;
  uint32_t* fin;
  uint32_t* anum;
  uint32_t* n_out_pair;
  PairCounters* C;
};
constexpr uint32_t NEVER = 0xfffffffeu;

struct PairChainArgs {
  const PairRun* runs;
  const uint32_t* list;
  const uint32_t* list_xl;
  uint32_t n_xl;
  const PairInfo* info;
  const uint8_t* ok_head;
  const HeadRec* rec;
  uint32_t *T_qs, *T_qe, *T_ts, *T_te;
  double* T_wid;
  uint64_t* T_seg;
  uint32_t *chain_base, *np;
  uint32_t *cnt, *has, *stretch;
  PairRun* T_runs;
  unsigned long long* totals;
  const PairCounters* C;
};
template <int NT, int PHASE>
__global__ __launch_bounds__(NT) void pair_chains_kernel(PairChainArgs A) {
  constexpr int U = 4;
  __shared__ uint32_t ws[NT / 64 + 1];
  __shared__ uint64_t ws64[NT / 64 + 1];
  __shared__ uint32_t sh_base;
  const int tid = threadIdx.x;
  if (A.C->flags & PF_FALLBACK) return;
  const uint32_t rk = blockIdx.x < A.n_xl ? A.list_xl[blockIdx.x] : A.list[blockIdx.x - A.n_xl];
  const PairRun run = A.runs[rk];
  const PairInfo pi = A.info[rk];
  const uint32_t a = run.a, m = pi.m, m_plus = pi.m_plus;
  if (PHASE == 0) {
    uint32_t c0 = 0, c1 = 0, mx = 0;
    for (uint32_t p0 = 0; p0 < m; p0 += NT * U) {
      uint8_t ok[U];
#pragma unroll
      for (int u = 0; u < U; ++u) {
        const uint32_t p = p0 + (uint32_t)u * NT + (uint32_t)tid;
        ok[u] = p < m ? A.ok_head[a + p] : (uint8_t)0;
      }
#pragma unroll
      for (int u = 0; u < U; ++u) {
        const uint32_t p = p0 + (uint32_t)u * NT + (uint32_t)tid;
        if (ok[u]) {
          const HeadRec hr = A.rec[a + p];
          if (p < m_plus) ++c0; else ++c1;
          const uint32_t e = hr.qe > hr.te ? hr.qe : hr.te;
          mx = e > mx ? e : mx;
        }
      }
    }
    const uint32_t nP = block_sum<NT>(c0, ws), nM = block_sum<NT>(c1, ws);
#pragma unroll
    for (int o = 32; o > 0; o >>= 1) {
      const uint32_t t = __shfl_xor(mx, o, 64);
      mx = t > mx ? t : mx;
    }
    if ((tid & 63) == 0 && (unsigned long long)mx > __hip_atomic_load(&A.totals[1], __ATOMIC_RELAXED, __HIP_MEMORY_SCOPE_AGENT))
      atomicMax(&A.totals[1], (unsigned long long)mx);
    if (tid == 0) {
      A.np[2 * rk] = nP;
      A.np[2 * rk + 1] = nM;
      A.cnt[rk] = nP + nM;
      A.has[rk] = nP + nM ? 1u : 0u;
    }
    return;
  }
  const uint32_t nP = A.np[2 * rk], nM = A.np[2 * rk + 1];
  if (nP + nM == 0) return;
  const uint32_t cb = A.chain_base[rk];
  if (tid == 0) {
    PairRun tr;
    tr.a = cb;
    tr.n = nP + nM;
    A.T_runs[A.stretch[rk]] = tr;
  }
  (void)sh_base;
  const bool plus_first = pi.first_mem[0] < pi.first_mem[1];
  uint32_t before = 0;
  for (uint32_t p0 = 0; p0 < m; p0 += NT * U) {
    uint8_t ok[U];
    uint64_t packed = 0;
#pragma unroll
    for (int u = 0; u < U; ++u) {
      const uint32_t p = p0 + (uint32_t)u * NT + (uint32_t)tid;
      ok[u] = p < m ? A.ok_head[a + p] : (uint8_t)0;
      packed |= (uint64_t)(ok[u] ? 1u : 0u) << (16 * u);
    }
    uint64_t inc = packed;
    const int lane = tid & 63, w = tid >> 6;
#pragma unroll
    for (int d = 1; d < 64; d <<= 1) {
      const uint64_t t = __shfl_up(inc, d, 64);
      if (lane >= d) inc += t;
    }
    uint64_t off = 0, tot = 0;
    if (NT == 64) {
      tot = __shfl(inc, 63, 64);
    } else {
      __syncthreads();
      if (lane == 63) ws64[w] = inc;
      __syncthreads();
#pragma unroll
      for (int k = 0; k < NT / 64; ++k) {
        const uint64_t x = ws64[k];
        off += k < w ? x : 0ull;
        tot += x;
      }
    }
    const uint64_t ex = off + inc - packed;
    uint32_t row_base = before;
#pragma unroll
    for (int u = 0; u < U; ++u) {
      const uint32_t p = p0 + (uint32_t)u * NT + (uint32_t)tid;
      if (ok[u]) {
        const uint32_t c_pos = row_base + (uint32_t)((ex >> (16 * u)) & 0xffffu);
        const uint32_t c_all = plus_first ? c_pos : (p >= m_plus ? c_pos - nP : c_pos + nM);
        const HeadRec hr = A.rec[a + p];
        const uint32_t c = cb + c_all;
        A.T_qs[c] = hr.qs;
        A.T_qe[c] = hr.qe;
        A.T_ts[c] = hr.ts;
        A.T_te[c] = hr.te;
        A.T_wid[c] = hr.wid;
        A.T_seg[c] = rk;
      }
      row_base += (uint32_t)((tot >> (16 * u)) & 0xffffu);
    }
    before = row_base;
  }
}

template <int NT, int KP>
__global__ __launch_bounds__(NT, NT >= 512 ? 4 : 1) void pair_finish_kernel(PairFinishArgs A) {
  constexpr int U = 4;
  __shared__ uint32_t ws[NT / 64 + 1];
  __shared__ uint64_t ws64[NT / 64 + 1];
  __shared__ uint64_t ws64n[2 * (NT / 64 + 1)];
  __shared__ uint32_t l_all[4 * KP];
  uint32_t* const l_qs = l_all;
  uint32_t* const l_qe = l_all + KP;
  uint32_t* const l_ts = l_all + 2 * KP;
  uint32_t* const l_pm = l_all + 3 * KP;
  const int tid = threadIdx.x;
#ifdef SWG_PAIR_TIMING
  unsigned long long pt_last = wall_clock64();
#endif
  if (A.C->flags & PF_FALLBACK) return;
// ... 21 lines not shown
    for (int d = 1; d < 64; d <<= 1) {
      const uint64_t t = __shfl_up(inc, d, 64);
      if (lane >= d) inc += t;
    }
    uint64_t off = 0, tot = 0;
    if (NT == 64) {
      tot = __shfl(inc, 63, 64);
    } else {
      lds_barrier();
      if (lane == 63) ws64[w] = inc;
      lds_barrier();
#pragma unroll
      for (int k = 0; k < NT / 64; ++k) {
        const uint64_t x = ws64[k];
        off += k < w ? x : 0ull;
        tot += x;
      }
    }
    *tot_out = tot;
    return off + inc - packed;
  };
  auto row_scan_n = [&](auto g_c, const uint64_t (&packed)[decltype(g_c)::value], uint64_t (&ex)[decltype(g_c)::value],
                        uint64_t (&tot)[decltype(g_c)::value]) {
    constexpr int G = decltype(g_c)::value;
    uint64_t inc[G];
    const int lane = tid & 63, w = tid >> 6;
#pragma unroll
    for (int g = 0; g < G; ++g) inc[g] = packed[g];
#pragma unroll
    for (int d = 1; d < 64; d <<= 1) {
#pragma unroll
      for (int g = 0; g < G; ++g) {
        const uint64_t t = __shfl_up(inc[g], d, 64);
        if (lane >= d) inc[g] += t;
      }
    }
    if (NT == 64) {
#pragma unroll
      for (int g = 0; g < G; ++g) {
        tot[g] = __shfl(inc[g], 63, 64);
        ex[g] = inc[g] - packed[g];
      }
      return;
    }
    lds_barrier();
    if (lane == 63) {
#pragma unroll
      for (int g = 0; g < G; ++g) ws64n[g * (NT / 64 + 1) + w] = inc[g];
    }
    lds_barrier();
#pragma unroll
    for (int g = 0; g < G; ++g) {
      uint64_t off = 0, t = 0;
#pragma unroll
      for (int k = 0; k < NT / 64; ++k) {
        const uint64_t x = ws64n[g * (NT / 64 + 1) + k];
        off += k < w ? x : 0ull;
        t += x;
      }
      tot[g] = t;
      ex[g] = off + inc[g] - packed[g];
    }
  };
  constexpr int US = NT >= 512 ? 8 : 4;
  constexpr int GS = US / 4;
  auto sweep = [&](const bool exact) {
    uint32_t kept_before = 0, ok_before = 0, c0 = 0, c1 = 0, cq = 0, cd = 0, cp = 0;
    for (uint32_t p0 = 0; p0 < m; p0 += NT * US) {
      uint8_t ok[US];
      uint32_t h_qs[US], h_qe[US], h_ts[US];
#pragma unroll
      for (int u = 0; u < US; ++u) {
        const uint32_t p = p0 + (uint32_t)u * NT + (uint32_t)tid;
        ok[u] = p < m ? A.ok_head[a + p] : (uint8_t)0;
      }
      bool kept[US];
      if (given) {
        uint64_t okp[GS], ex_ok[GS], tot_ok[GS];
#pragma unroll
        for (int g = 0; g < GS; ++g) okp[g] = 0;
#pragma unroll
        for (int u = 0; u < US; ++u) okp[u / 4] |= (uint64_t)(ok[u] ? 1u : 0u) << (16 * (u % 4));
        row_scan_n(std::integral_constant<int, GS>{}, okp, ex_ok, tot_ok);
        uint32_t rb = ok_before;
#pragma unroll
        for (int u = 0; u < US; ++u) {
          const uint32_t p = p0 + (uint32_t)u * NT + (uint32_t)tid;
          kept[u] = false;
          if (ok[u]) {
            const uint32_t c_pos = rb + (uint32_t)((ex_ok[u / 4] >> (16 * (u % 4))) & 0xffffu);
            const uint32_t c_all = plus_first0 ? c_pos : (p >= m_plus ? c_pos - g_nP : c_pos + g_nM);
            kept[u] = A.kept_in[g_cb + c_all] != 0;
          }
          rb += (uint32_t)((tot_ok[u / 4] >> (16 * (u % 4))) & 0xffffu);
        }
        ok_before = rb;
      }
      uint64_t packed[GS], ex[GS], tot[GS];
#pragma unroll
      for (int g = 0; g < GS; ++g) packed[g] = 0;
#pragma unroll
      for (int u = 0; u < US; ++u) {
        const uint32_t p = p0 + (uint32_t)u * NT + (uint32_t)tid;
        if (!given) kept[u] = false;
        if (ok[u]) {
          const bool hq = (ok[u] & 2u) != 0, ht = (ok[u] & 4u) != 0;
          if (!given) kept[u] = exact ? (all_q || hq) && (all_t || ht) : hq && ht;
          if (p < m_plus) ++c0; else ++c1;
          cq += hq ? 1u : 0u;
          cd += (given || (hq && ht)) ? 0u : 1u;
          cp += (kept[u] && p < m_plus) ? 1u : 0u;
        }
        packed[u / 4] |= (uint64_t)(kept[u] ? 1u : 0u) << (16 * (u % 4));
      }
#pragma unroll
      for (int u = 0; u < US; ++u) {
        const uint32_t p = p0 + (uint32_t)u * NT + (uint32_t)tid;
        h_qs[u] = h_qe[u] = h_ts[u] = 0;
        if (kept[u] && p < m_plus) {
          const HeadRec* hp = A.rec + a + p;
          h_qs[u] = hp->qs;
          h_qe[u] = hp->qe;
          h_ts[u] = hp->ts;
        }
      }
      row_scan_n(std::integral_constant<int, GS>{}, packed, ex, tot);
      uint32_t row_base = kept_before;
#pragma unroll
      for (int u = 0; u < US; ++u) {
        const uint32_t p = p0 + (uint32_t)u * NT + (uint32_t)tid;
        const uint32_t r = row_base + (uint32_t)((ex[u / 4] >> (16 * (u % 4))) & 0xffffu);
        if (p < m) A.head_num[a + p] = kept[u] ? r : (ok[u] ? NEVER : NONE);
        if (kept[u] && p < m_plus) {
          A.f_qs[a + r] = h_qs[u];
          A.f_qe[a + r] = h_qe[u];
          A.f_ts[a + r] = h_ts[u];
          if (r < (uint32_t)KP) {
            l_qs[r] = h_qs[u];
            l_qe[r] = h_qe[u];
            l_ts[r] = h_ts[u];
          }
        }
        row_base += (uint32_t)((tot[u / 4] >> (16 * (u % 4))) & 0xffffu);
      }
      kept_before = row_base;
    }
    n_kept = kept_before;
    n_pass0 = block_sum<NT>(c0, ws);
    n_pass1 = block_sum<NT>(c1, ws);
    n_q = block_sum<NT>(cq, ws);
    n_deg = block_sum<NT>(cd, ws);
    kP = block_sum<NT>(cp, ws);
  };
  sweep(false);
  const uint32_t n_ch = n_pass0 + n_pass1;
  if (n_ch == 0) {
    if (tid == 0) A.sum[rk] = sm;
    return;
  }
  if (n_deg) {
    all_q = n_ch <= 1;
    all_t = (all_q ? n_ch : n_q) <= 1;
    __syncthreads();
    sweep(true);
  }
  const uint32_t kM = n_kept - kP;
  const bool plus_first = pi.first_mem[0] < pi.first_mem[1];
  sm.n_pass = n_ch;
  sm.n_kept = n_kept;
  sm.minmem = n_pass0 && n_pass1 ? (pi.first_mem[0] < pi.first_mem[1] ? pi.first_mem[0] : pi.first_mem[1]) : (n_pass0 ? pi.first_mem[0] : pi.first_mem[1]);
  if (tid == 0) A.sum[rk] = sm;
  if (n_kept == 0) return;
  __syncthreads();
  auto local_number = [&](uint32_t r, bool minus) -> uint32_t {
    if (plus_first) return r + 1;
    return minus ? r - kP + 1 : r + kM + 1;
  };
  FT_STAMP(0);
  uint32_t out = 0;
  for (uint32_t p0 = 0; p0 < m; p0 += NT * US) {
    uint32_t h[US], idx[US], r[US];
#pragma unroll
    for (int u = 0; u < US; ++u) {
      const uint32_t p = p0 + (uint32_t)u * NT + (uint32_t)tid;
      h[u] = p < m ? A.hd[a + p] : a;
      idx[u] = (p < m && !A.fin) ? A.s_idx[a + p] : 0u;
    }
#pragma unroll
    for (int u = 0; u < US; ++u) r[u] = A.head_num[h[u]];
#pragma unroll
    for (int u = 0; u < US; ++u) {
      const uint32_t p = p0 + (uint32_t)u * NT + (uint32_t)tid;
      uint32_t an = 0;
      if (p < m && r[u] < NEVER) {
        an = local_number(r[u], h[u] - a >= m_plus);
        if (!A.fin) {
          A.chain[idx[u]] = an;
          A.status[idx[u]] = SWG_ST_SCAFFOLD;
        }
        ++out;
      } else if (r[u] == NEVER) {
        an = NEVER;
      }
      if (A.fin && p < m) A.fin[a + p] = (an != 0u && an != NEVER) ? ((uint32_t)SWG_ST_SCAFFOLD << 30) | an : 0u;
      if (A.rescue_d && p < m) A.anum[a + p] = an;
    }
  }
  for (uint32_t p = m + (uint32_t)tid; p < M; p += NT) {
    if (A.rescue_d) A.anum[a + p] = 0u;
    if (A.fin) A.fin[a + p] = 0u;
  }
  FT_STAMP(1);
  if (!A.scaffolds_only && kP > 0 && M > m_plus) {
    const bool in_lds = kP <= (uint32_t)KP;
    uint64_t carry = 0;
    for (uint32_t c0b = 0; c0b < kP; c0b += NT) {
      const uint32_t c = c0b + tid;
      const uint64_t v = c < kP ? (uint64_t)(in_lds ? l_qe[c] : A.f_qe[a + c]) : 0ull;
      uint64_t tot;
      uint64_t ex = block_excl_max<NT>(v, ws64, &tot);
      ex = ex > carry ? ex : carry;
      if (c < kP) {
        const uint32_t pm = (uint32_t)(v > ex ? v : ex);
        if (in_lds) l_pm[c] = pm; else A.f_pm[a + c] = pm;
      }
      carry = tot > carry ? tot : carry;
    }
    __syncthreads();
    const uint32_t* __restrict__ c_qs = in_lds ? l_qs : A.f_qs + a;
    const uint32_t* __restrict__ c_qe = in_lds ? l_qe : A.f_qe + a;
    const uint32_t* __restrict__ c_ts = in_lds ? l_ts : A.f_ts + a;
    const uint32_t* __restrict__ c_pm = in_lds ? l_pm : A.f_pm + a;
    const uint64_t gap = A.gap, max_dev = A.max_dev;
    for (uint32_t p = m_plus + tid; p < M; p += NT) {
      const uint32_t iw = A.s_idx[a + p];
      if (p >= m && (iw >> 31) == 0) continue;
      const uint32_t i = iw & 0x7fffffffu;
      const uint64_t qs = A.s_qs[a + p], qe = A.s_qe[a + p], ts = A.s_ts[a + p], te = A.s_te[a + p];
      if (A.fin ? A.fin[a + p] != 0u : A.chain[i] != 0u) continue;
      const uint64_t qc = (qs + qe) / 2, tc = (ts + te) / 2;
      const uint64_t lim = qe > ~0ull - gap ? ~0ull : qe + gap;
      uint32_t l = 0, r = kP;
      while (l < r) {
        const uint32_t mid = l + ((r - l) >> 1);
        if ((uint64_t)c_qs[mid] <= lim) l = mid + 1; else r = mid;
      }
      uint32_t lo = 0, hi = l;
      while (lo < hi) {
        const uint32_t mid = lo + ((hi - lo) >> 1);
        const uint64_t pm = c_pm[mid];
        if ((pm > ~0ull - gap ? ~0ull : pm + gap) < qs) lo = mid + 1; else hi = mid;
      }
      uint32_t best = NONE;
      for (uint32_t c = lo; c < l; ++c) {
        const uint64_t cqe = c_qe[c];
        if ((cqe > ~0ull - gap ? ~0ull : cqe + gap) < qs) continue;
        const int64_t diag = (int64_t)c_ts[c] - (int64_t)c_qs[c];
        const int64_t dev = (int64_t)tc - (int64_t)qc - diag;
        const uint64_t deviation = dev < 0 ? (uint64_t)0 - (uint64_t)dev : (uint64_t)dev;
        if (deviation <= max_dev) {
          best = c;
          break;
        }
      }
      if (best != NONE) {
        const uint32_t num = local_number(best, false);
        if (A.fin) {
          A.fin[a + p] = ((uint32_t)SWG_ST_SCAFFOLD << 30) | num;
        } else {
          A.chain[i] = num;
          A.status[i] = SWG_ST_SCAFFOLD;
        }
        if (A.rescue_d) A.anum[a + p] = num;
        ++out;
      }
    }
  }
  FT_STAMP(2);
  if (!A.scaffolds_only && A.rescue_d) {
    __syncthreads();
    const uint64_t D = A.rescue_d, max_s2 = A.max_s2;
    int cell_sh = 0;
    while (cell_sh < 32 && (1ull << cell_sh) <= D) ++cell_sh;
    constexpr uint32_t NB = (uint32_t)KP / 2u, KA = (4u * (uint32_t)KP - NB - 1u) / 3u, BT = NB / NT;
    static_assert(KA >= (uint32_t)NT * U && KA < 65536u && NB % (2 * NT) == 0, "one round of anchors fits a batch; whole words of bins per thread");
    uint32_t* const g_qc = l_all;
    uint32_t* const g_tc = l_all + KA;
    uint32_t* const g_ix = l_all + 2 * KA;
    uint16_t* const b_start = reinterpret_cast<uint16_t*>(l_all + 3 * KA);
    uint32_t* const b_cur = l_all + 3 * KA + (NB + 2) / 2;
    auto bump = [&](uint32_t b) -> uint32_t {
      const uint32_t sh = 16u * (b & 1u);
      return (atomicAdd(&b_cur[b >> 1], 1u << sh) >> sh) & 0xffffu;
    };
    uint32_t* const c_num = A.f_qe + a;
    auto is_anchor = [](uint32_t an) { return an != 0u && an < 0x80000000u; };
    static_assert((NB & (NB - 1u)) == 0u && NB >= 4u, "bins by the cell's low bits");
    auto cell_of = [&](uint32_t qc) -> uint32_t { return cell_sh < 32 ? qc >> cell_sh : 0u; };
    auto bin_of = [&](uint32_t qc) -> uint32_t { return cell_of(qc) & (NB - 1u); };
    uint32_t pb = 0, r0 = 0;
    while (pb < M) {
      for (uint32_t b = tid; b < NB / 2; b += NT) b_cur[b] = 0u;
      __syncthreads();
      uint32_t cnt = 0, pe = pb;
      for (uint32_t p0 = pb; p0 < M; p0 += NT * U) {
        uint32_t an[U], qs[U], qe[U];
#pragma unroll
        for (int u = 0; u < U; ++u) {
          const uint32_t p = p0 + (uint32_t)u * NT + (uint32_t)tid;
          const uint32_t j = a + (p < M ? p : 0u);
          an[u] = p < M ? A.anum[j] : 0u;
          qs[u] = A.s_qs[j];
          qe[u] = A.s_qe[j];
        }
        uint32_t mine = 0;
#pragma unroll
        for (int u = 0; u < U; ++u) mine += is_anchor(an[u]) ? 1u : 0u;
        const uint32_t rt = block_sum<NT>(mine, ws);
        if (cnt + rt > KA) break;
#pragma unroll
        for (int u = 0; u < U; ++u)
          if (is_anchor(an[u])) (void)bump(bin_of((uint32_t)(((uint64_t)qs[u] + qe[u]) / 2)));
        cnt += rt;
        pe = p0 + NT * U < M ? p0 + NT * U : M;
      }
      __syncthreads();
      {
        uint32_t c[BT], sum = 0;
#pragma unroll
        for (uint32_t k = 0; k < BT; k += 2) {
          const uint32_t w = b_cur[((uint32_t)tid * BT + k) >> 1];
          c[k] = w & 0xffffu;
          c[k + 1] = w >> 16;
          sum += c[k] + c[k + 1];
        }
        uint32_t tot;
        uint32_t run = block_excl_sum<NT>(sum, ws, &tot);
#pragma unroll
        for (uint32_t k = 0; k < BT; k += 2) {
          const uint32_t s0 = run, s1 = run + c[k];
          b_start[(uint32_t)tid * BT + k] = (uint16_t)s0;
          b_start[(uint32_t)tid * BT + k + 1] = (uint16_t)s1;
          b_cur[((uint32_t)tid * BT + k) >> 1] = s0 | (s1 << 16);
          run = s1 + c[k + 1];
        }
        if (tid == NT - 1) b_start[NB] = (uint16_t)run;
      }
      __syncthreads();
      for (uint32_t p0 = pb; p0 < pe; p0 += NT * U) {
        uint32_t an[U], qs[U], qe[U], ts[U], te[U], ix[U];
#pragma unroll
        for (int u = 0; u < U; ++u) {
          const uint32_t p = p0 + (uint32_t)u * NT + (uint32_t)tid;
          const uint32_t j = a + (p < pe ? p : 0u);
          an[u] = p < pe ? A.anum[j] : 0u;
          qs[u] = A.s_qs[j];
          qe[u] = A.s_qe[j];
          ts[u] = A.s_ts[j];
          te[u] = A.s_te[j];
          ix[u] = A.s_idx[j];
        }
#pragma unroll
        for (int u = 0; u < U; ++u) {
          if (!is_anchor(an[u])) continue;
          const uint32_t qc = (uint32_t)(((uint64_t)qs[u] + qe[u]) / 2);
          const uint32_t e = bump(bin_of(qc));
          g_qc[e] = qc;
          g_tc[e] = (uint32_t)(((uint64_t)ts[u] + te[u]) / 2);
          g_ix[e] = ix[u] & 0x7fffffffu;
          c_num[r0 + e] = an[u];
        }
      }
      __syncthreads();
      FT_STAMP(3);
      for (uint32_t p0 = 0; cnt && p0 < M; p0 += NT * U) {
        uint32_t an[U], qs[U], qe[U], ts[U], te[U];
#pragma unroll
        for (int u = 0; u < U; ++u) {
          const uint32_t p = p0 + (uint32_t)u * NT + (uint32_t)tid;
          const uint32_t j = a + (p < M ? p : 0u);
          an[u] = A.anum[j];
          qs[u] = A.s_qs[j];
          qe[u] = A.s_qe[j];
          ts[u] = A.s_ts[j];
          te[u] = A.s_te[j];
// ... 451 lines not shown
  const uint32_t n = (uint32_t)n64;
  hipStream_t st = ctx->stream;
  static const bool dbg = getenv("SWG_DEBUG") != nullptr;
  const swg_arena_mark mark0 = swg_arena_save(ctx);
  const bool by_hash = n <= PAIR_HASH_MAX;
  bool plain = cfg != nullptr;
  if (cfg) {
    const bool sf_limited = cfg->scaffold_filter_mode == SWG_MODE_ONE_TO_ONE || cfg->scaffold_filter_mode == SWG_MODE_ONE_TO_MANY ||
                            cfg->scaffold_max_per_query != 0 || cfg->scaffold_max_per_target != 0;
    const bool mf_limited = cfg->mapping_filter_mode == SWG_MODE_ONE_TO_ONE || cfg->mapping_filter_mode == SWG_MODE_ONE_TO_MANY ||
                            cfg->mapping_max_per_query != 0 || cfg->mapping_max_per_target != 0;
    plain = !sf_limited && !mf_limited && (cfg->scaffolds_only || cfg->scaffold_max_deviation == 0);
  }
  static const uint32_t per_pair_env = getenv("SWG_PAIR_MIN_AVG") && atoi(getenv("SWG_PAIR_MIN_AVG")) > 0 ? (uint32_t)atoi(getenv("SWG_PAIR_MIN_AVG")) : 0u;
  const uint32_t per_pair = per_pair_env ? per_pair_env : (plain ? 96u : 192u);
  const uint32_t cap = by_hash ? (n < 8192u ? n : 8192u) : (n / per_pair > 8192u ? n / per_pair : 8192u);
  uint32_t tsize = 1;
  while (tsize < 2 * (by_hash ? n : cap)) tsize <<= 1;
  PairCounters* C = nullptr;
  PairRun* runs = swg_alloc<PairRun>(ctx, cap);
  uint32_t* class_list = swg_alloc<uint32_t>(ctx, (size_t)4 * cap);
  uint32_t* perm = nullptr;
  if (by_hash) {
    char* z = static_cast<char*>(swg_arena_alloc(ctx, (size_t)tsize * 12 + sizeof(PairCounters) + 8));
    uint32_t* slot_of = swg_alloc<uint32_t>(ctx, n);
    uint32_t* start = swg_alloc<uint32_t>(ctx, tsize);
    perm = swg_alloc<uint32_t>(ctx, n);
    SWG_CHECK_ARENA(ctx);
    unsigned long long* table = reinterpret_cast<unsigned long long*>(z);
    uint32_t* count = reinterpret_cast<uint32_t*>(z + (size_t)tsize * 8);
    C = reinterpret_cast<PairCounters*>(z + (size_t)tsize * 12);
    uint32_t* cursor = reinterpret_cast<uint32_t*>(z + (size_t)tsize * 12 + sizeof(PairCounters));
    SWG_HIP(ctx, hipMemsetAsync(z, 0, (size_t)tsize * 12 + sizeof(PairCounters) + 8, st));
    SWG_LAUNCH(ctx, "pair_hash", pair_hash_kernel<<<(n + 255) / 256, 256, 0, st>>>(n, r->q_id, r->t_id, table, tsize - 1, count, slot_of));
    SWG_LAUNCH(ctx, "pair_slots", pair_slots_kernel<<<(tsize + 255) / 256, 256, 0, st>>>(tsize, count, start, runs, class_list, cap, C, cursor));
    SWG_LAUNCH(ctx, "pair_perm", pair_perm_kernel<<<(n + 255) / 256, 256, 0, st>>>(n, slot_of, start, perm));
    SWG_KERNEL_CHECK(ctx);
  } else {
    C = swg_alloc<PairCounters>(ctx, 1);
    const uint32_t n_words = (n + 63) / 64;
    unsigned long long* bitmap = swg_alloc<unsigned long long>(ctx, n_words + 1);
    uint32_t* wcnt = swg_alloc<uint32_t>(ctx, n_words + 1);
    uint32_t* wpre = swg_alloc<uint32_t>(ctx, n_words + 1);
    uint32_t* starts = swg_alloc<uint32_t>(ctx, (size_t)cap + 2);
    unsigned long long* table = swg_alloc<unsigned long long>(ctx, tsize);
    uint64_t* d_nr = swg_alloc<uint64_t>(ctx, 1);
    static const bool order_knob = !(getenv("SWG_PAIR_ORDER") && atoi(getenv("SWG_PAIR_ORDER")) == 0);
    const uint32_t cap_tmp = n / PAIR_M_MAX + 1u < cap ? n / PAIR_M_MAX + 1u : cap;
    uint32_t* order_tmp = order_knob ? swg_alloc<uint32_t>(ctx, (size_t)2 * cap_tmp) : nullptr;
    SWG_CHECK_ARENA(ctx);
    SWG_HIP(ctx, hipMemsetAsync(C, 0, sizeof(PairCounters), st));
    SWG_HIP(ctx, hipMemsetAsync(table, 0xff, (size_t)tsize * 8, st));
    SWG_LAUNCH(ctx, "pair_boundary", pair_boundary_kernel<<<(n + 1023) / 1024, 256, 0, st>>>(n, r->q_id, r->t_id, bitmap, wcnt));
    SWG_KERNEL_CHECK(ctx);
    SWG_TRY(swg_exclusive_scan_u32(ctx, wcnt, wpre, n_words, d_nr));
    SWG_LAUNCH(ctx, "pair_runs", pair_starts_kernel<<<(n_words + 255) / 256, 256, 0, st>>>(n, n_words, bitmap, wpre, d_nr, cap, starts));
    SWG_KERNEL_CHECK(ctx);
    SWG_LAUNCH(ctx, "pair_runs", pair_runs_kernel<<<(cap + 255) / 256, 256, 0, st>>>(n, cap, d_nr, starts, r->q_id, r->t_id, table, tsize - 1, runs, class_list, C));
    SWG_KERNEL_CHECK(ctx);
    if (order_knob && n > PAIR_M_MAX) {
      SWG_LAUNCH(ctx, "pair_order", pair_order_kernel<<<2, ORDER_NT, 0, st>>>(runs, class_list, cap, order_tmp, cap_tmp, pair_mx_cut(), C));
      SWG_KERNEL_CHECK(ctx);
    }
  }
  uint64_t h[4];
  static_assert(offsetof(PairCounters, n_above) == 24, "the first four words are read back: the counts and pair_order's cut");
  SWG_TRY(swg_read_scalars(ctx, reinterpret_cast<const uint64_t*>(C), h, 4));
  const uint32_t n_runs = (uint32_t)h[0], flags = (uint32_t)(h[0] >> 32);
  if (flags || n_runs == 0) {
    if (dbg) fprintf(stderr, "[swg] pair path: not applicable (%u runs, flags %u)\n", n_runs, flags);
    plan->not_grouped = !by_hash && (flags & (PF_NOT_GROUPED | PF_RUN_OVERFLOW)) && !(flags & PF_TOO_LONG);
    swg_arena_restore(ctx, mark0);
    return SWG_OK;
  }
  if ((uint64_t)n / n_runs > PAIR_L_MAX) {
    if (dbg) fprintf(stderr, "[swg] pair path: %u pairs of %llu records on average: left to the global-sort stage\n", n_runs, (unsigned long long)n / n_runs);
    swg_arena_restore(ctx, mark0);
    return SWG_OK;
  }
  plan->valid = 1;
  plan->by_hash = by_hash;
  plan->n_runs = n_runs;
  plan->ncls[0] = (uint32_t)h[1];
  plan->ncls[1] = (uint32_t)(h[1] >> 32);
  plan->ncls[2] = (uint32_t)h[2];
  plan->ncls[3] = (uint32_t)(h[2] >> 32);
  const uint32_t above = (uint32_t)h[3];
  if (pair_mx_cut() && (above & ORDERED) && (above & ~ORDERED) <= plan->ncls[2]) {
    plan->cut = pair_mx_cut();
    plan->n_above = above & ~ORDERED;
  }
  plan->cap = cap;
  plan->counters = C;
  plan->runs = runs;
  plan->class_list = class_list;
  plan->perm = perm;
  if (dbg)
    fprintf(stderr, "[swg] pair path: %u pairs (%u / %u / %u / %u by size class)%s\n", n_runs, plan->ncls[0], plan->ncls[1], plan->ncls[2],
            plan->ncls[3], by_hash ? ", found through the hash table" : "");
  return SWG_OK;
}

int scaffold_stage_pairs(swg_ctx* ctx, const swg_records* r, const swg_config* cfg, const uint8_t* alive, const uint8_t* member,
                         bool sweep_assumed_identity, uint8_t* status_out, uint32_t* chain_out, swg_stats* stats, int* taken,
                         const PairPlan* plan_in) {
  *taken = 0;
  PairPlan own;
  if (!plan_in) {
    SWG_TRY(pair_plan(ctx, r, cfg, &own));
    plan_in = &own;
  }
  if (!plan_in->valid) return SWG_OK;
  uint64_t kq, kt;
  if (cfg->scaffold_filter_mode == SWG_MODE_ONE_TO_ONE) {
    kq = kt = 1;
  } else {
    kq = cfg->scaffold_max_per_query ? cfg->scaffold_max_per_query : SWG_K_INF;
    kt = cfg->scaffold_max_per_target ? cfg->scaffold_max_per_target : SWG_K_INF;
  }
  const bool limited = kq != SWG_K_INF || kt != SWG_K_INF;
  const bool rescue = !cfg->scaffolds_only && cfg->scaffold_max_deviation != 0;
  const bool need_wid = limited || !(cfg->min_scaffold_identity <= 0.0);
  const uint32_t n = (uint32_t)r->n;
  hipStream_t st = ctx->stream;
  static const bool dbg = getenv("SWG_DEBUG") != nullptr;
  const swg_arena_mark mark0 = swg_arena_save(ctx);
  const bool by_hash = plan_in->by_hash;
  const uint32_t cap = plan_in->cap, n_runs = plan_in->n_runs;
  const uint32_t ncls[4] = {plan_in->ncls[0], plan_in->ncls[1], plan_in->ncls[2], plan_in->ncls[3]};
  PairCounters* C = static_cast<PairCounters*>(plan_in->counters);
  PairRun* runs = static_cast<PairRun*>(plan_in->runs);
  uint32_t* class_list = static_cast<uint32_t*>(plan_in->class_list);
  uint32_t* perm = static_cast<uint32_t*>(plan_in->perm);
  SWG_HIP(ctx, hipMemsetAsync(reinterpret_cast<char*>(C) + offsetof(PairCounters, flags), 0, sizeof(uint32_t), st));
  SWG_HIP(ctx, hipMemsetAsync(reinterpret_cast<char*>(C) + offsetof(PairCounters, n_chunks), 0, sizeof(PairCounters) - offsetof(PairCounters, n_chunks), st));
  uint8_t* code = swg_alloc<uint8_t>(ctx, n);
  uint32_t* s_qs = swg_alloc<uint32_t>(ctx, n);
  uint32_t* s_qe = swg_alloc<uint32_t>(ctx, n);
  uint32_t* s_ts = swg_alloc<uint32_t>(ctx, n);
  uint32_t* s_te = swg_alloc<uint32_t>(ctx, n);
  uint32_t* s_m = swg_alloc<uint32_t>(ctx, n);
  uint32_t* s_b = swg_alloc<uint32_t>(ctx, n);
  uint32_t* s_idx = swg_alloc<uint32_t>(ctx, n);
  uint32_t* pred = swg_alloc<uint32_t>(ctx, n);
  uint32_t* hd = swg_alloc<uint32_t>(ctx, n);
  uint8_t* ok_head = swg_alloc<uint8_t>(ctx, n);
  unsigned long long* bps = swg_alloc<unsigned long long>(ctx, n);
  HeadRec* head_rec = swg_alloc<HeadRec>(ctx, n);
  uint32_t* anum = rescue ? swg_alloc<uint32_t>(ctx, n) : nullptr;
  PairInfo* info = swg_alloc<PairInfo>(ctx, n_runs);
  PairSum* sum = swg_alloc<PairSum>(ctx, n_runs);
  uint32_t* n_out_pair = swg_alloc<uint32_t>(ctx, n_runs);
  const uint32_t cap_chunks = n / PAIR_CELL + 2 * n_runs + 16;
  SpecBlock* chunks = swg_alloc<SpecBlock>(ctx, cap_chunks);
  const uint32_t cap_long = n / LABEL_CAP_ELEMS + 1;
  uint32_t* long_list = swg_alloc<uint32_t>(ctx, cap_long);
  SWG_CHECK_ARENA(ctx);
  PairTable gl_first, gp2_first;
  SWG_TRY(pair_table_make(ctx, r->n_genome_last, n_runs, &gl_first));
  SWG_TRY(pair_table_make(ctx, r->n_genome_two, n_runs, &gp2_first));
  uint32_t* fin = by_hash ? nullptr : swg_alloc<uint32_t>(ctx, n);
  SWG_CHECK_ARENA(ctx);
  if (by_hash) {
    SWG_HIP(ctx, hipMemsetAsync(chain_out, 0, (size_t)n * sizeof(uint32_t), st));
    SWG_HIP(ctx, hipMemsetAsync(status_out, 0, n, st));
  }
  SWG_HIP(ctx, hipMemsetAsync(n_out_pair, 0, (size_t)n_runs * sizeof(uint32_t), st));
  if (!by_hash) {
    SWG_HIP(ctx, hipMemsetAsync(chunks, 0, (size_t)cap_chunks * sizeof(SpecBlock), st));
    SWG_HIP(ctx, hipMemsetD32Async(reinterpret_cast<hipDeviceptr_t>(&C->n_chunks), (int)cap_chunks, 1, st));
  }
  PairSortArgs SA{};
  SA.q_id = r->q_id; SA.t_id = r->t_id; SA.q_start = r->q_start; SA.q_end = r->q_end; SA.t_start = r->t_start; SA.t_end = r->t_end;
  SA.matches = r->matches; SA.block_len = r->block_len; SA.identity = r->identity; SA.strand = r->strand;
  SA.alive_in = alive; SA.member_in = member;
  SA.min_block = cfg->min_block_length; SA.keep_self = cfg->keep_self; SA.min_identity = cfg->min_identity;
  SA.check_degenerate = sweep_assumed_identity ? 1 : 0;
  SA.max_gap = cfg->scaffold_gap;
  SA.runs = runs;
  SA.perm = perm;
  SA.orig = plan_in->orig;
  SA.code = code; SA.s_qs = s_qs; SA.s_qe = s_qe; SA.s_ts = s_ts; SA.s_te = s_te; SA.s_m = need_wid ? s_m : nullptr; SA.s_b = need_wid ? s_b : nullptr; SA.s_idx = s_idx; SA.pred = pred;
  SA.info = info; SA.chunks = chunks; SA.cap_chunks = cap_chunks; SA.chunks_by_place = by_hash ? 0 : 1; SA.long_list = long_list; SA.cap_long = cap_long; SA.C = C; SA.gl_first = gl_first; SA.seq_genome_last = r->seq_genome_last;
  if (by_hash) {
    for (int c = 2; c >= 0; --c) {
      if (!ncls[c]) continue;
      SA.list = class_list + (size_t)c * cap;
      if (c == 0)
        SWG_LAUNCH_N(ctx, "pair_sort_ps", 0, pair_sort_kernel<64, 16, 16, 256, 64, true><<<ncls[c], 64, 0, st>>>(SA));
      else if (c == 1)
        SWG_LAUNCH_N(ctx, "pair_sort_pm", 0, pair_sort_kernel<256, 16, 16, 1024, 64, true><<<ncls[c], 256, 0, st>>>(SA));
      else
        SWG_LAUNCH_N(ctx, "pair_sort_pl", 0, pair_sort_kernel<1024, 8, 32, 2048, 1024, true><<<ncls[c], 1024, 0, st>>>(SA));
      SWG_KERNEL_CHECK(ctx);
    }
  } else {
    const uint32_t n_above = plan_in->cut ? plan_in->n_above : ncls[2], n_mx = ncls[2] - n_above;
    if (dbg && ncls[2]) fprintf(stderr, "[swg] pair_sort: %u pairs under pair_sort_big, %u under pair_sort_mx (cut %u)\n", n_above + ncls[3], n_mx, plan_in->cut);
    if (n_above + ncls[3]) {
      SA.list = class_list + (size_t)2 * cap;
      SWG_LAUNCH_N(ctx, "pair_sort_big", 0, pair_sort_big_kernel<<<n_above + ncls[3], 1024, 0, st>>>(SA, class_list + (size_t)3 * cap, ncls[3]));
      SWG_KERNEL_CHECK(ctx);
    }
    if (n_mx) {
      SA.list = class_list + (size_t)2 * cap + n_above;
      SWG_LAUNCH_N(ctx, "pair_sort_mx", 0, pair_sort_kernel<512, 16, 32, 2048, 1024, false><<<n_mx, 512, 0, st>>>(SA));
      SWG_KERNEL_CHECK(ctx);
    }
    for (int c = 1; c >= 0; --c) {
      if (!ncls[c]) continue;
      SA.list = class_list + (size_t)c * cap;
      if (c == 0)
        SWG_LAUNCH_N(ctx, "pair_sort_s", 0, pair_sort_kernel<64, 16, 16, 256, 64, false><<<ncls[c], 64, 0, st>>>(SA));
      else
        SWG_LAUNCH_N(ctx, "pair_sort_m", 0, pair_sort_kernel<256, 16, 16, 1024, 64, false><<<ncls[c], 256, 0, st>>>(SA));
      SWG_KERNEL_CHECK(ctx);
    }
  }
  if (!by_hash) {
    SWG_LAUNCH(ctx, "pair_gate", pair_gate_kernel<<<1, 64, 0, st>>>(C));
    SWG_KERNEL_CHECK(ctx);
  }
  const bool long_possible = ncls[2] + ncls[3] > 0;
  const uint32_t* lab_m = need_wid ? s_m : nullptr;
  const uint32_t* lab_b = need_wid ? s_b : nullptr;
  auto short_leg = [&]() -> int {
    SWG_TRY(pair_walk_launch(ctx, cap_chunks, &C->n_chunks, chunks, s_qs, s_qe, s_ts, s_te, cfg->scaffold_gap, bps, pred));
    return SWG_OK;
  };
  auto short_label = [&]() -> int {
    return pair_label_launch(ctx, cap_chunks, &C->n_chunks, chunks, pred, s_qs, s_qe, s_ts, s_te, lab_m, lab_b, cfg->min_scaffold_length,
                             cfg->min_scaffold_identity, hd, ok_head, head_rec, &C->n_heads);
  };
  auto long_walk = [&](hipStream_t ls) -> int {
    SWG_TRY(pair_walk_long_launch(ctx, ls, cap_long, &C->n_long, long_list, chunks, n, s_qs, s_qe, s_ts, s_te, cfg->scaffold_gap, bps, pred,
                                  &C->flags, PF_FALLBACK));
    if (!by_hash) {
      swg_on_stream on(ctx, ls);
      SWG_LAUNCH(ctx, "pair_gate", pair_gate_kernel<<<1, 64, 0, ls>>>(C));
      SWG_KERNEL_CHECK(ctx);
    }
    return SWG_OK;
  };
  auto long_label = [&](hipStream_t ls) -> int {
    return pair_label_long_launch(ctx, ls, cap_long, &C->n_long, long_list, chunks, pred, s_qs, s_qe, s_ts, s_te, lab_m, lab_b,
                                  cfg->min_scaffold_length, cfg->min_scaffold_identity, hd, ok_head, head_rec, &C->n_heads);
  };
  static const bool overlap_knob = !(getenv("SWG_PAIR_OVERLAP") && atoi(getenv("SWG_PAIR_OVERLAP")) == 0);
  if (overlap_knob && long_possible && !by_hash) {
    hipStream_t side = nullptr;
    SWG_TRY(swg_side_stream(ctx, &side));
    SWG_HIP(ctx, hipEventRecord(ctx->ev_fork, st));
    SWG_HIP(ctx, hipStreamWaitEvent(side, ctx->ev_fork, 0));
    int rc = long_walk(side);
    if (rc == SWG_OK) rc = long_label(side);
    if (rc == SWG_OK) rc = short_leg();
    if (rc == SWG_OK) rc = short_label();
    hipError_t je = hipEventRecord(ctx->ev_join, side);
    if (je == hipSuccess) je = hipStreamWaitEvent(st, ctx->ev_join, 0);
    if (je != hipSuccess || rc != SWG_OK) (void)hipStreamSynchronize(side);
    SWG_TRY(rc);
    SWG_HIP(ctx, je);
  } else {
    SWG_TRY(short_leg());
    if (long_possible) SWG_TRY(long_walk(st));
    SWG_TRY(short_label());
    if (long_possible) SWG_TRY(long_label(st));
  }
  uint8_t* kept_flags = nullptr;
  uint32_t *chain_base = nullptr, *np_arr = nullptr;
  if (limited) {
    PairChainArgs CA{};
    CA.runs = runs; CA.info = info; CA.ok_head = ok_head; CA.rec = head_rec; CA.C = C;
    CA.T_qs = swg_alloc<uint32_t>(ctx, n);
    CA.T_qe = swg_alloc<uint32_t>(ctx, n);
    CA.T_ts = swg_alloc<uint32_t>(ctx, n);
    CA.T_te = swg_alloc<uint32_t>(ctx, n);
    CA.T_wid = swg_alloc<double>(ctx, n);
    CA.T_seg = swg_alloc<uint64_t>(ctx, n);
    CA.chain_base = chain_base = swg_alloc<uint32_t>(ctx, n_runs);
    CA.np = np_arr = swg_alloc<uint32_t>(ctx, (size_t)2 * n_runs);
    CA.totals = swg_alloc<unsigned long long>(ctx, 3);
    CA.T_runs = swg_alloc<PairRun>(ctx, n_runs);
    CA.cnt = swg_alloc<uint32_t>(ctx, n_runs);
    CA.has = swg_alloc<uint32_t>(ctx, n_runs);
    CA.stretch = swg_alloc<uint32_t>(ctx, n_runs);
    kept_flags = swg_alloc<uint8_t>(ctx, n);
    SWG_CHECK_ARENA(ctx);
    SWG_HIP(ctx, hipMemsetAsync(CA.totals, 0, 24, st));
    SWG_HIP(ctx, hipMemsetAsync(CA.cnt, 0, (size_t)n_runs * sizeof(uint32_t), st));
    SWG_HIP(ctx, hipMemsetAsync(CA.has, 0, (size_t)n_runs * sizeof(uint32_t), st));
    for (int phase = 0; phase < 2; ++phase) {
      for (int c = 0; c < 3; ++c) {
        const uint32_t nb = c == 2 ? ncls[2] + ncls[3] : ncls[c];
        if (!nb) continue;
        CA.list = class_list + (size_t)c * cap;
        CA.list_xl = c == 2 ? class_list + (size_t)3 * cap : nullptr;
        CA.n_xl = c == 2 ? ncls[3] : 0u;
        if (phase == 0) {
          switch (c) {
            case 0: SWG_LAUNCH(ctx, "pair_chains_s", pair_chains_kernel<64, 0><<<nb, 64, 0, st>>>(CA)); break;
            case 1: SWG_LAUNCH(ctx, "pair_chains_m", pair_chains_kernel<256, 0><<<nb, 256, 0, st>>>(CA)); break;
            default: SWG_LAUNCH(ctx, "pair_chains", pair_chains_kernel<512, 0><<<nb, 512, 0, st>>>(CA)); break;
          }
        } else {
          switch (c) {
            case 0: SWG_LAUNCH(ctx, "pair_chains_s", pair_chains_kernel<64, 1><<<nb, 64, 0, st>>>(CA)); break;
            case 1: SWG_LAUNCH(ctx, "pair_chains_m", pair_chains_kernel<256, 1><<<nb, 256, 0, st>>>(CA)); break;
            default: SWG_LAUNCH(ctx, "pair_chains", pair_chains_kernel<512, 1><<<nb, 512, 0, st>>>(CA)); break;
          }
        }
        SWG_KERNEL_CHECK(ctx);
      }
      if (phase == 0) {
        SWG_TRY(swg_exclusive_scan_u32(ctx, CA.cnt, chain_base, n_runs, reinterpret_cast<uint64_t*>(CA.totals)));
        SWG_TRY(swg_exclusive_scan_u32(ctx, CA.has, CA.stretch, n_runs, reinterpret_cast<uint64_t*>(CA.totals + 2)));
      }
    }
    uint64_t ht[3];
    SWG_TRY(swg_read_scalars(ctx, reinterpret_cast<const uint64_t*>(CA.totals), ht, 3));
    const uint64_t n_table = ht[0];
    if (n_table) {
      const int seg_bits = swg_bits_for(n_runs) ? swg_bits_for(n_runs) : 1, pos_bits = swg_bits_for(ht[1]) ? swg_bits_for(ht[1]) : 1;
      SWG_TRY(scaffold_sweep_segments(ctx, n_table, CA.T_seg, seg_bits, CA.T_qs, CA.T_qe, CA.T_ts, CA.T_te, CA.T_wid, kq, kt,
                                      cfg->scaffold_overlap_threshold, cfg->scoring_function, pos_bits, kept_flags, CA.T_runs, (uint32_t)ht[2]));
    }
  }
  PairFinishArgs FA{};
  FA.kept_in = kept_flags; FA.chain_base = chain_base; FA.np = np_arr;
  FA.runs = runs; FA.info = info; FA.sum = sum;
  FA.s_qs = s_qs; FA.s_qe = s_qe; FA.s_ts = s_ts; FA.s_te = s_te; FA.s_idx = s_idx; FA.hd = hd; FA.ok_head = ok_head; FA.rec = head_rec;
  FA.head_num = pred;
  FA.f_qs = s_m; FA.f_qe = s_b; FA.f_ts = reinterpret_cast<uint32_t*>(bps); FA.f_pm = reinterpret_cast<uint32_t*>(bps) + n;
  FA.status = status_out; FA.chain = chain_out; FA.scaffolds_only = cfg->scaffolds_only; FA.gap = cfg->scaffold_gap; FA.max_dev = pair_max_deviation(cfg->scaffold_gap); FA.C = C;
  FA.rescue_d = rescue ? cfg->scaffold_max_deviation : 0;
  FA.max_s2 = rescue ? pair_max_dist2(cfg->scaffold_max_deviation) : 0;
  FA.anum = anum;
  FA.n_out_pair = n_out_pair;
  FA.fin = fin;
  for (int c = 0; c < 3; ++c) {
    const uint32_t nb = c == 2 ? ncls[2] + ncls[3] : ncls[c];
    if (!nb) continue;
    FA.list = class_list + (size_t)c * cap;
    FA.list_xl = c == 2 ? class_list + (size_t)3 * cap : nullptr;
    FA.n_xl = c == 2 ? ncls[3] : 0u;
    switch (c) {
      case 0: SWG_LAUNCH(ctx, "pair_finish_s", pair_finish_kernel<64, 256><<<nb, 64, 0, st>>>(FA)); break;
      case 1: SWG_LAUNCH(ctx, "pair_finish_m", pair_finish_kernel<256, 1024><<<nb, 256, 0, st>>>(FA)); break;
      default: SWG_LAUNCH(ctx, "pair_finish", pair_finish_kernel<512, 4096><<<nb, 512, 0, st>>>(FA)); break;
    }
    SWG_KERNEL_CHECK(ctx);
  }
  if (n_runs <= (uint32_t)NUMBER_SMALL) {
    SWG_LAUNCH(ctx, "pair_number", pair_number_small_kernel<<<1, 512, 0, st>>>(n_runs, info, sum, gl_first, r->seq_genome_last, gp2_first,
                                                                     r->seq_genome_two, C));
    SWG_KERNEL_CHECK(ctx);
  } else if (n_runs <= NUMBER_COUNT_MAX) {
    uint64_t* key = swg_alloc<uint64_t>(ctx, n_runs);
    uint32_t* val = swg_alloc<uint32_t>(ctx, n_runs);
    uint32_t* rank1 = swg_alloc<uint32_t>(ctx, n_runs);
    SWG_CHECK_ARENA(ctx);
    constexpr uint32_t per_wg = (NUMBER_NT / 64) * NUMBER_T;
    const unsigned rb = nblk(n_runs), wb = (n_runs + per_wg - 1) / per_wg < (unsigned)ctx->num_cu ? (n_runs + per_wg - 1) / per_wg : (unsigned)ctx->num_cu;
    SWG_LAUNCH(ctx, "pair_number", pair_key1_kernel<<<rb, EW, 0, st>>>(n_runs, info, sum, gl_first, r->seq_genome_last, key, val, C));
    SWG_LAUNCH(ctx, "pair_number", pair_rank_count_kernel<<<wb, NUMBER_NT, 0, st>>>(n_runs, key, info, r->seq_genome_two, gp2_first, rank1));
    SWG_LAUNCH(ctx, "pair_number", pair_key2_kernel<<<rb, EW, 0, st>>>(n_runs, info, sum, rank1, r->seq_genome_two, gp2_first, key, val, C));
    SWG_LAUNCH(ctx, "pair_number", pair_base_count_kernel<<<wb, NUMBER_NT, 0, st>>>(n_runs, key, sum));
    SWG_KERNEL_CHECK(ctx);
  } else {
    uint64_t* key = swg_alloc<uint64_t>(ctx, n_runs);
    uint64_t* key_tmp = swg_alloc<uint64_t>(ctx, n_runs);
    uint32_t* val = swg_alloc<uint32_t>(ctx, n_runs);
    uint32_t* val_tmp = swg_alloc<uint32_t>(ctx, n_runs);
    uint32_t* rank1 = swg_alloc<uint32_t>(ctx, n_runs);
    uint32_t* sizes = swg_alloc<uint32_t>(ctx, n_runs);
    SWG_CHECK_ARENA(ctx);
    const unsigned rb = nblk(n_runs);
    SWG_LAUNCH(ctx, "pair_number", pair_key1_kernel<<<rb, EW, 0, st>>>(n_runs, info, sum, gl_first, r->seq_genome_last, key, val, C));
    SWG_KERNEL_CHECK(ctx);
    SWG_TRY(swg_radix_sort_pairs(ctx, &key, &val, &key_tmp, &val_tmp, n_runs, 0, 64));
    SWG_LAUNCH(ctx, "pair_number", pair_rank1_kernel<<<rb, EW, 0, st>>>(n_runs, val, info, sum, r->seq_genome_two, gp2_first, rank1, C));
    SWG_KERNEL_CHECK(ctx);
    SWG_LAUNCH(ctx, "pair_number", pair_key2_kernel<<<rb, EW, 0, st>>>(n_runs, info, sum, rank1, r->seq_genome_two, gp2_first, key, val, C));
    SWG_KERNEL_CHECK(ctx);
    SWG_TRY(swg_radix_sort_pairs(ctx, &key, &val, &key_tmp, &val_tmp, n_runs, 0, 64));
    SWG_LAUNCH(ctx, "pair_number", pair_sizes_kernel<<<rb, EW, 0, st>>>(n_runs, val, sum, sizes));
    SWG_KERNEL_CHECK(ctx);
    SWG_TRY(swg_exclusive_scan_u32(ctx, sizes, sizes, n_runs, nullptr));
    SWG_LAUNCH(ctx, "pair_number", pair_base_kernel<<<rb, EW, 0, st>>>(n_runs, val, sizes, sum));
    SWG_KERNEL_CHECK(ctx);
  }
  {
    const unsigned gb = n_runs < (unsigned)ctx->num_cu * 16 ? n_runs : (unsigned)ctx->num_cu * 16;
    if (fin) {
      const unsigned cu = (unsigned)ctx->num_cu;
      if (ncls[2] + ncls[3]) {
        const uint32_t nb = ncls[2] + ncls[3];
        SWG_LAUNCH(ctx, "pair_renumber", pair_out_kernel<1024, 16384><<<nb < cu * 8 ? nb : cu * 8, 1024, 0, st>>>(
                                             ncls[3], class_list + (size_t)3 * cap, ncls[2], class_list + (size_t)2 * cap, runs, info, sum, s_idx, fin,
                                             chain_out, status_out, C));
        SWG_KERNEL_CHECK(ctx);
      }
      if (ncls[1]) {
        SWG_LAUNCH(ctx, "pair_renumber", pair_out_kernel<256, 4096><<<ncls[1] < cu * 16 ? ncls[1] : cu * 16, 256, 0, st>>>(
                                             0u, nullptr, ncls[1], class_list + (size_t)1 * cap, runs, info, sum, s_idx, fin, chain_out, status_out, C));
        SWG_KERNEL_CHECK(ctx);
      }
      if (ncls[0]) {
        SWG_LAUNCH(ctx, "pair_renumber", pair_out_kernel<64, 1024><<<ncls[0] < cu * 64 ? ncls[0] : cu * 64, 64, 0, st>>>(
                                             0u, nullptr, ncls[0], class_list, runs, info, sum, s_idx, fin, chain_out, status_out, C));
        SWG_KERNEL_CHECK(ctx);
      }
    } else {
      SWG_LAUNCH(ctx, "pair_renumber", pair_renumber_kernel<<<gb, EW, 0, st>>>(n_runs, runs, sum, chain_out, C, perm));
      SWG_KERNEL_CHECK(ctx);
    }
  }
  SWG_LAUNCH(ctx, "pair_totals", pair_totals_kernel<<<(n_runs + 4095) / 4096 < 64u ? (n_runs + 4095) / 4096 : 64u, 1024, 0, st>>>(n_runs, info, sum, n_out_pair, C));
  SWG_KERNEL_CHECK(ctx);
  uint64_t hc[10];
  static_assert(sizeof(PairCounters) == 80 && offsetof(PairCounters, n_alive) == 40, "PairCounters is read back as ten words");
  SWG_TRY(swg_read_scalars(ctx, reinterpret_cast<const uint64_t*>(C), hc, 10));
  const uint32_t flags2 = (uint32_t)(hc[0] >> 32);
  if (flags2) {
    if (dbg) fprintf(stderr, "[swg] pair path: left on the device's word (flags %u): the global-sort path takes the call\n", flags2);
    swg_arena_restore(ctx, mark0);
    return SWG_OK;
  }
#ifdef SWG_PAIR_TIMING
  {
    unsigned long long ht[16];
    (void)hipMemcpyFromSymbol(ht, HIP_SYMBOL(g_pair_t), sizeof ht);
    fprintf(stderr, "[swg] pair_sort phases (100 MHz ticks summed over work-groups):");
    for (int k = 0; k < 13; ++k) fprintf(stderr, " %d:%llu", k, ht[k]);
    fprintf(stderr, "\n");
    unsigned long long z[16] = {0};
    (void)hipMemcpyToSymbol(HIP_SYMBOL(g_pair_t), z, sizeof z);
    (void)hipMemcpyFromSymbol(ht, HIP_SYMBOL(g_fin_t), sizeof ht);
    fprintf(stderr, "[swg] pair_finish phases:");
    for (int k = 0; k < 8; ++k) fprintf(stderr, " %d:%llu", k, ht[k]);
    fprintf(stderr, "\n");
    (void)hipMemcpyToSymbol(HIP_SYMBOL(g_fin_t), z, sizeof z);
  }
#endif
  if (stats) {
    stats->n_retained = hc[5];
    stats->n_swept = hc[6];
    stats->n_chains = hc[7];
    stats->n_chains_kept = hc[8];
    stats->n_out = hc[9];
  }
  *taken = 1;
  return SWG_OK;
}

}
```

### sweepga_amd/csrc/swg_scaffold_internal.h

```cpp
#pragma once
#include <cstdio>
#include <cstdlib>
#include <vector>

#include "swg_log.h"
#include "swg_pipeline.h"

namespace swg_scaf {

constexpr int EW = 256;
constexpr uint32_t NONE = 0xffffffffu;
inline unsigned nblk(uint64_t n) { return (unsigned)((n + EW - 1) / EW); }

static __global__ __launch_bounds__(EW) void fill_u32_kernel(uint64_t n, uint32_t* __restrict__ p, uint32_t v) {
  uint64_t i = (uint64_t)blockIdx.x * EW + threadIdx.x;
  if (i < n) p[i] = v;
}
static __global__ __launch_bounds__(EW) void fill_u64_kernel(uint64_t n, uint64_t* __restrict__ p, uint64_t v) {
  uint64_t i = (uint64_t)blockIdx.x * EW + threadIdx.x;
  if (i < n) p[i] = v;
}
static __global__ __launch_bounds__(EW) void iota_u32_kernel(uint64_t n, uint32_t* __restrict__ p) {
  uint64_t i = (uint64_t)blockIdx.x * EW + threadIdx.x;
  if (i < n) p[i] = (uint32_t)i;
}

static __global__ void fp_thresholds_kernel(uint64_t gap, uint64_t D, uint64_t* __restrict__ out) {
  if (threadIdx.x != 0 || blockIdx.x != 0) return;
  auto perp_ok = [&](uint64_t deviation) {
    const double pd = __ddiv_rn((double)deviation, 1.4142135623730951);
    const uint64_t perp = pd >= 18446744073709551616.0 ? ~0ull : (uint64_t)pd;
    return perp <= gap;
  };
  auto dist_ok = [&](uint64_t s2) {
    const double dd = __dsqrt_rn((double)s2);
    const uint64_t dist = dd >= 18446744073709551616.0 ? ~0ull : (uint64_t)dd;
    return dist <= D;
  };
  uint64_t res[2];
  for (int which = 0; which < 2; ++which) {
    auto ok = [&](uint64_t x) { return which == 0 ? perp_ok(x) : dist_ok(x); };
    uint64_t lo = 0, hi = ~0ull;
    if (ok(hi)) {
      lo = hi;
    } else {
      while (hi - lo > 1) {
        const uint64_t mid = lo + ((hi - lo) >> 1);
        if (ok(mid))
          lo = mid;
        else
          hi = mid;
      }
    }
    res[which] = lo;
  }
  out[0] = res[0];
  out[1] = res[1];
}


struct PairTable {
  uint32_t* dense;
  unsigned long long* keys;
  uint32_t* vals;
  uint32_t mask;
  uint32_t n_genome;
};
__device__ __forceinline__ uint32_t* pair_slot(const PairTable& t, uint32_t gq, uint32_t gt) {
  if (t.dense) return t.dense + ((size_t)gq * t.n_genome + gt);
  const unsigned long long key = (unsigned long long)gq * t.n_genome + gt;
  uint32_t h = (uint32_t)((key * 0x9e3779b97f4a7c15ull) >> 32) & t.mask;
  for (;;) {
    unsigned long long k = __hip_atomic_load(&t.keys[h], __ATOMIC_RELAXED, __HIP_MEMORY_SCOPE_AGENT);
    if (k == ~0ull) {
      k = atomicCAS(&t.keys[h], ~0ull, key);
      if (k == ~0ull) k = key;
    }
    if (k == key) return t.vals + h;
    h = (h + 1) & t.mask;
  }
}
__device__ __forceinline__ uint32_t pair_get(const PairTable& t, uint32_t gq, uint32_t gt) {
  if (t.dense) return t.dense[(size_t)gq * t.n_genome + gt];
  const unsigned long long key = (unsigned long long)gq * t.n_genome + gt;
  uint32_t h = (uint32_t)((key * 0x9e3779b97f4a7c15ull) >> 32) & t.mask;
  while (t.keys[h] != key) h = (h + 1) & t.mask;
  return t.vals[h];
}
constexpr uint64_t DENSE_PAIR_LIMIT = uint64_t(1) << 28;

int pair_table_make(swg_ctx* ctx, uint32_t n_genome, uint64_t bound, PairTable* t);

struct ChainTable {
  uint64_t nc = 0;
  uint32_t *qid = nullptr, *tid = nullptr, *qs = nullptr, *qe = nullptr, *ts = nullptr, *te = nullptr;
  double* wid = nullptr;
};

struct ChainBuild {
  uint64_t M = 0;
  uint64_t* keyA = nullptr;
  uint32_t* idxA = nullptr;
  uint32_t *a_qe = nullptr, *a_ts = nullptr, *a_te = nullptr, *a_dpair = nullptr;
  uint64_t n_pairs = 0;
  uint64_t m = 0;
  uint32_t* s_a = nullptr;
  uint32_t* s_idx = nullptr;
  uint32_t* s_chain = nullptr;
  bool want_s_chain = true;
  const uint32_t *m_hd = nullptr, *m_rank_of = nullptr;
  const uint8_t* m_ok_head = nullptr;
  const uint32_t* m_head_of_chain = nullptr;
  uint64_t n_chains_all = 0;
  ChainTable T;
  uint8_t* C_strand = nullptr;
  uint32_t* C_dpair = nullptr;
};

struct SpecBlock {
  uint32_t ue;
  uint32_t bb;
  uint32_t be;
  uint32_t pad;
};
constexpr int BIG_SPAN_SHIFT = 10;
constexpr uint32_t WALK_CHUNK = 1024;
constexpr uint32_t BIG_UNIT = 8192;

struct __attribute__((aligned(32))) HeadRec {
  uint32_t qs, qe, ts, te;
  double wid;
  uint64_t grp;
};
#ifdef __HIPCC__
__device__ __forceinline__ double chain_weighted_identity(uint64_t total_length, uint64_t sm, uint64_t sb) {
  const uint64_t gap_length = total_length > sb ? total_length - sb : 0;
  double lcg = 0.0;
  if (gap_length > 0) {
    lcg = swg_log_glibc((double)gap_length);
    if (!(lcg > 0.0)) lcg = 0.0;
  }
  const double eff = __dadd_rn((double)sb, lcg);
  return eff > 0.0 ? __ddiv_rn((double)sm, eff) : 0.0;
}
#endif
constexpr uint32_t LABEL_CAP_ELEMS = WALK_CHUNK + BIG_UNIT;

int pair_walk_launch(swg_ctx* ctx, uint32_t cap_chunks, const uint32_t* n_chunks_dev, const SpecBlock* desc, const uint32_t* s_qs,
                     const uint32_t* s_qe, const uint32_t* s_ts, const uint32_t* s_te, uint64_t max_gap, unsigned long long* bps,
                     uint32_t* pred);
int pair_walk_long_launch(swg_ctx* ctx, hipStream_t st, uint32_t cap_long, const uint32_t* n_long_dev, const uint32_t* long_list, const SpecBlock* chunks,
                          uint32_t n_members_cap, const uint32_t* s_qs, const uint32_t* s_qe, const uint32_t* s_ts, const uint32_t* s_te,
                          uint64_t max_gap, unsigned long long* own, uint32_t* pred, uint32_t* flags, uint32_t fallback_bit);
int pair_label_launch(swg_ctx* ctx, uint32_t cap_chunks, const uint32_t* n_chunks_dev, const SpecBlock* chunks, const uint32_t* pred,
                      const uint32_t* s_qs, const uint32_t* s_qe, const uint32_t* s_ts, const uint32_t* s_te, const uint32_t* s_m,
                      const uint32_t* s_b, uint64_t min_len, double min_ident, uint32_t* hd, uint8_t* ok_head, HeadRec* rec,
                      unsigned long long* n_heads);
int pair_label_long_launch(swg_ctx* ctx, hipStream_t st, uint32_t cap_long, const uint32_t* n_long_dev, const uint32_t* long_list, const SpecBlock* chunks,
                           const uint32_t* pred, const uint32_t* s_qs, const uint32_t* s_qe, const uint32_t* s_ts, const uint32_t* s_te,
                           const uint32_t* s_m, const uint32_t* s_b, uint64_t min_len, double min_ident, uint32_t* hd, uint8_t* ok_head,
                           HeadRec* rec, unsigned long long* n_heads);


struct ChainWork {
  uint64_t n_groups = 0;
  uint32_t *s_qs = nullptr, *s_qe = nullptr, *s_ts = nullptr, *s_te = nullptr, *s_m = nullptr, *s_b = nullptr;
  uint64_t* s_grp = nullptr;
  uint32_t* head_flag = nullptr;
  uint32_t* s_gidx = nullptr;
  uint32_t* group_begin = nullptr;
  uint32_t* pred = nullptr;
  uint64_t* d_tot = nullptr;
  const SpecBlock* chunks = nullptr;
  uint64_t n_chunks = 0;
  const uint8_t* big_member = nullptr;
  const uint8_t* span_big = nullptr;
};

int chain_predecessors(swg_ctx* ctx, const swg_records* r, const uint8_t* alive, const uint8_t* member, uint64_t max_gap,
                       int pos_bits, ChainBuild* out, ChainWork* work, const uint32_t* q_order, uint64_t n_alive,
                       const swg_key_ends* slots);
int chain_table_build(swg_ctx* ctx, const swg_records* r, const uint8_t* alive, uint64_t min_len, double min_ident,
                      bool genome_pair_major, ChainBuild* out, const ChainWork& work);
inline int build_chains(swg_ctx* ctx, const swg_records* r, const uint8_t* alive, const uint8_t* member, uint64_t max_gap,
                        uint64_t min_len, double min_ident, int pos_bits, bool genome_pair_major, ChainBuild* out,
                        const uint32_t* q_order = nullptr, uint64_t n_alive = ~0ull, const swg_key_ends* slots = nullptr) {
  ChainWork W;
  SWG_TRY(chain_predecessors(ctx, r, alive, member, max_gap, pos_bits, out, &W, q_order, n_alive, slots));
  if (out->M == 0 || out->m == 0) return SWG_OK;
  return chain_table_build(ctx, r, alive, min_len, min_ident, genome_pair_major, out, W);
}

int scaffold_sweep_and_number(swg_ctx* ctx, const ChainTable& T, uint32_t n_seq, const uint32_t* seq_genome2,
                              uint32_t n_g2, int mode, uint64_t max_q, uint64_t max_t, double thr, int scoring,
                              int pos_bits, uint8_t* C_kept, uint32_t* C_num, uint64_t* n_kept_out);

int scaffold_sweep_segments(swg_ctx* ctx, uint64_t nc, const uint64_t* seg, int seg_bits, const uint32_t* qs, const uint32_t* qe,
                            const uint32_t* ts, const uint32_t* te, const double* wid, uint64_t kq, uint64_t kt, double thr, int scoring,
                            int pos_bits, uint8_t* kept, const void* runs = nullptr, uint32_t n_runs = 0);

struct PairPlan {
  int valid = 0;
  bool by_hash = false;
  uint32_t n_runs = 0, ncls[4] = {0, 0, 0, 0}, cap = 0;
  uint32_t n_above = 0, cut = 0;
  void *counters = nullptr, *runs = nullptr, *class_list = nullptr, *perm = nullptr;
  bool not_grouped = false;
  const uint32_t* orig = nullptr;
};
int pair_group_records(swg_ctx* ctx, const swg_records* r, swg_records* copy, uint32_t** perm, int* ok);
int pair_ungroup_results(swg_ctx* ctx, uint64_t n, const uint32_t* perm, const uint8_t* st, const uint32_t* ch, uint8_t* status_out, uint32_t* chain_out);
int pair_plan(swg_ctx* ctx, const swg_records* r, const swg_config* cfg, PairPlan* plan);
int scaffold_stage_pairs(swg_ctx* ctx, const swg_records* r, const swg_config* cfg, const uint8_t* alive, const uint8_t* member,
                         bool sweep_assumed_identity, uint8_t* status_out, uint32_t* chain_out, swg_stats* stats, int* taken,
                         const PairPlan* plan = nullptr);

}
```

Measured before the change: 12.59 billion mappings/s.

## Add ranked chunk form so pair labeling emits compact per-chunk head ranks

For pair runs whose chunks all fit the fast LDS label path, the label kernel now ranks passing chain heads inside each chunk with a block prefix scan. It writes compact head tables (qs/qe/ts) and per-chunk pass counts, and stores each element's head rank directly instead of writing ok_head flags and HeadRec records. The finalize kernel then numbers chains from chunk bases and ranks, skipping the separate head numbering and head_num gather, and the plus-strand scan reads the compact tables. This removes global head-compaction work and scattered reads, at the cost of extra scan and sync work in the label kernel, chunk-size limits with a fallback, and a larger chunk allocation.

```diff
diff --git a/sweepga_amd/csrc/swg_chain.hip b/sweepga_amd/csrc/swg_chain.hip
--- a/sweepga_amd/csrc/swg_chain.hip
+++ b/sweepga_amd/csrc/swg_chain.hip
@@ -1593,7 +1593,7 @@
           P.qe = s_qe[i];
           P.ts = s_ts[i];
           P.te = s_te[i];
-          P.minus = pair_desc ? D.pad : (uint32_t)(s_grp[i] & 1ull);
+          P.minus = pair_desc ? D.pad & 1u : (uint32_t)(s_grp[i] & 1ull);
         } else {
 #pragma unroll
           for (int c = 0; c < KC; ++c) {
@@ -1840,7 +1840,7 @@
           if (wstats && lane == 0) atomicAdd(&wstats[2], 1ull);
           const uint32_t ii = i0 + l;
           const uint64_t qe_l = s_qe[ii], ts_l = s_ts[ii], te_l = s_te[ii];
-          const bool minus_l = pair_desc ? D.pad != 0 : (s_grp[ii] & 1ull) != 0;
+          const bool minus_l = pair_desc ? (D.pad & 1u) != 0 : (s_grp[ii] & 1ull) != 0;
           const uint32_t e_l = readlane_u32(e_i, l);
           const uint64_t bound = qe_l + max_gap;
           uint64_t ld = INF;
diff --git a/sweepga_amd/csrc/swg_chain_table.hip b/sweepga_amd/csrc/swg_chain_table.hip
--- a/sweepga_amd/csrc/swg_chain_table.hip
+++ b/sweepga_amd/csrc/swg_chain_table.hip
@@ -359,11 +359,11 @@
 }
 
 constexpr int LABEL_CAP = (int)(WALK_CHUNK + BIG_UNIT);
-constexpr int LABEL_FAST = 1536;
+constexpr int LABEL_FAST = (int)LABEL_FAST_ELEMS;
 constexpr int LABEL_NT = 512;
 static_assert(LABEL_FAST * (2 + 2 + 3 * 4) >= LABEL_CAP * 2, "the two layouts share one LDS buffer");
-template <int NT, bool MB>
-__global__ __launch_bounds__(NT) void chain_label_kernel(uint32_t n_chunks, const SpecBlock* __restrict__ chunks,
+template <int NT, bool MB, bool RANKED>
+__global__ __launch_bounds__(NT, RANKED ? 8 : 1) void chain_label_kernel(uint32_t n_chunks, const SpecBlock* __restrict__ chunks,
                                                          const uint32_t* __restrict__ pred,
                                                          const uint32_t* __restrict__ s_qs, const uint32_t* __restrict__ s_qe,
                                                          const uint32_t* __restrict__ s_ts, const uint32_t* __restrict__ s_te,
@@ -372,7 +372,7 @@
                                                          uint64_t min_len, double min_ident, uint32_t* __restrict__ hd,
                                                          uint8_t* __restrict__ ok_head, HeadRec* __restrict__ rec,
                                                          unsigned long long* __restrict__ n_heads,
-                                                         const uint32_t* __restrict__ n_chunks_dev = nullptr) {
+                                                         const uint32_t* __restrict__ n_chunks_dev = nullptr, LabelRanked R = LabelRanked{}) {
   if (n_chunks_dev) n_chunks = min(n_chunks, *n_chunks_dev);
   __shared__ uint32_t lds[LABEL_FAST * (MB ? 6 : 4)];
   uint16_t* succ = reinterpret_cast<uint16_t*>(lds);
@@ -382,6 +382,7 @@
   uint32_t* l_te = l_ts + LABEL_FAST;
   uint32_t* l_m = MB ? l_te + LABEL_FAST : nullptr;
   uint32_t* l_b = MB ? l_m + LABEL_FAST : nullptr;
+  __shared__ uint64_t ws64[RANKED ? NT / 64 : 1];
   if (!MB) s_m = s_b = nullptr;
   constexpr uint16_t NO = 0xffffu;
   uint32_t heads = 0;
@@ -424,13 +425,16 @@
         }
       }
       __syncthreads();
+      const uint32_t pad = RANKED ? chunks[c].pad : 0u;
+      const bool rkd = RANKED && (pad & CHUNK_RANKED) != 0u;
+      uint32_t pass = 0;
 #pragma unroll
       for (int u = 0; u < U; ++u) {
         const uint32_t k = (uint32_t)u * NT + threadIdx.x;
         if (k >= len) continue;
         const uint32_t p = b + k;
         if (r_pr[u] != NONE) {
-          ok_head[p] = 0;
+          if (!rkd) ok_head[p] = 0;
           continue;
         }
         ++heads;
@@ -453,7 +457,7 @@
         if (ok) {
           const double wid = chain_weighted_identity(total_length, sm, sb);
           ok = wid >= min_ident;
-          if (ok) {
+          if (ok && !rkd) {
             HeadRec hr;
             hr.qs = qs0;
             hr.qe = qe;
@@ -464,7 +468,66 @@
             rec[p] = hr;
           }
         }
+        if (rkd) {
+          if (ok) {
+            pass |= 1u << u;
+            l_qe[k] = qe;
+            l_ts[k] = ts;
+            l_te[k] = qs0;
+            if (!(qs0 < qe && ts < te)) atomicOr(R.flags, R.fallback_bit);
+          } else {
+            succ[k] = NO;
+          }
+          continue;
+        }
         ok_head[p] = ok ? (uint8_t)(s_grp ? 1u : 1u | (qs0 < qe ? 2u : 0u) | (ts < te ? 4u : 0u)) : (uint8_t)0;
+      }
+      if constexpr (RANKED) {
+        if (rkd) {
+          uint64_t packed = 0;
+#pragma unroll
+          for (int u = 0; u < U; ++u) packed |= (uint64_t)((pass >> u) & 1u) << (16 * u);
+          static_assert(U <= 4 && NT < 65536, "the rows' counters share a 64-bit word");
+          uint64_t inc = packed;
+          const int lane = threadIdx.x & 63, w = threadIdx.x >> 6;
+#pragma unroll
+          for (int d = 1; d < 64; d <<= 1) {
+            const uint64_t t = __shfl_up(inc, d, 64);
+            if (lane >= d) inc += t;
+          }
+          if (lane == 63) ws64[w] = inc;
+          __syncthreads();
+          uint64_t off = 0, tot = 0;
+#pragma unroll
+          for (int j = 0; j < NT / 64; ++j) {
+            const uint64_t x = ws64[j];
+            off += j < w ? x : 0ull;
+            tot += x;
+          }
+          const uint64_t ex = off + inc - packed;
+          uint32_t row_base = 0;
+#pragma unroll
+          for (int u = 0; u < U; ++u) {
+            const uint32_t k = (uint32_t)u * NT + threadIdx.x;
+            if ((pass >> u) & 1u) {
+              const uint32_t r = row_base + (uint32_t)((ex >> (16 * u)) & 0xffffu);
+              succ[k] = (uint16_t)r;
+              if ((pad & 1u) == 0u) {
+                R.t_qs[b + r] = l_te[k];
+                R.t_qe[b + r] = l_qe[k];
+                reinterpret_cast<uint32_t*>(rec + b)[r] = l_ts[k];
+              }
+            }
+            row_base += (uint32_t)((tot >> (16 * u)) & 0xffffu);
+          }
+          if (threadIdx.x == 0) R.chunk_pass[c] = row_base;
+          __syncthreads();
+          for (uint32_t k = threadIdx.x; k < len; k += NT) {
+            const uint16_t r = succ[l_hd[k]];
+            hd[b + k] = r == NO ? NONE : (uint32_t)r;
+          }
+          continue;
+        }
       }
       __syncthreads();
       for (uint32_t k = threadIdx.x; k < len; k += NT) hd[b + k] = b + l_hd[k];
@@ -740,10 +803,10 @@
     static const uint64_t lper = getenv("SWG_LABEL_BLOCKS") ? (uint64_t)atoi(getenv("SWG_LABEL_BLOCKS")) : 128;
     const uint64_t lb = W.n_chunks < (uint64_t)ctx->num_cu * lper ? W.n_chunks : (uint64_t)ctx->num_cu * lper;
     if (s_m)
-      SWG_LAUNCH(ctx, "chain_label", chain_label_kernel<LABEL_NT, true><<<(unsigned)lb, LABEL_NT, 0, st>>>((uint32_t)W.n_chunks, W.chunks, pred, s_qs, s_qe, s_ts, s_te,
+      SWG_LAUNCH(ctx, "chain_label", chain_label_kernel<LABEL_NT, true, false><<<(unsigned)lb, LABEL_NT, 0, st>>>((uint32_t)W.n_chunks, W.chunks, pred, s_qs, s_qe, s_ts, s_te,
                                                                         s_m, s_b, s_grp, min_len, min_ident, hd, ok_head, head_rec, n_heads));
     else
-      SWG_LAUNCH(ctx, "chain_label", chain_label_kernel<LABEL_NT, false><<<(unsigned)lb, LABEL_NT, 0, st>>>((uint32_t)W.n_chunks, W.chunks, pred, s_qs, s_qe, s_ts, s_te,
+      SWG_LAUNCH(ctx, "chain_label", chain_label_kernel<LABEL_NT, false, false><<<(unsigned)lb, LABEL_NT, 0, st>>>((uint32_t)W.n_chunks, W.chunks, pred, s_qs, s_qe, s_ts, s_te,
                                                                         s_m, s_b, s_grp, min_len, min_ident, hd, ok_head, head_rec, n_heads));
     SWG_KERNEL_CHECK(ctx);
     only = W.big_member;
@@ -871,16 +934,20 @@
 int pair_label_launch(swg_ctx* ctx, uint32_t cap_chunks, const uint32_t* n_chunks_dev, const SpecBlock* chunks, const uint32_t* pred,
                       const uint32_t* s_qs, const uint32_t* s_qe, const uint32_t* s_ts, const uint32_t* s_te, const uint32_t* s_m,
                       const uint32_t* s_b, uint64_t min_len, double min_ident, uint32_t* hd, uint8_t* ok_head, HeadRec* rec,
-                      unsigned long long* n_heads) {
+                      unsigned long long* n_heads, const LabelRanked* ranked) {
   if (cap_chunks == 0) return SWG_OK;
   static const uint64_t lper = getenv("SWG_LABEL_BLOCKS") ? (uint64_t)atoi(getenv("SWG_LABEL_BLOCKS")) : 128;
   const uint64_t lb = cap_chunks < (uint64_t)ctx->num_cu * lper ? cap_chunks : (uint64_t)ctx->num_cu * lper;
-  if (s_m)
-    SWG_LAUNCH(ctx, "chain_label", chain_label_kernel<LABEL_NT, true><<<(unsigned)lb, LABEL_NT, 0, ctx->stream>>>(cap_chunks, chunks, pred, s_qs, s_qe, s_ts, s_te, s_m, s_b,
+  if (ranked && !s_m)
+    SWG_LAUNCH(ctx, "chain_label", chain_label_kernel<LABEL_NT, false, true><<<(unsigned)lb, LABEL_NT, 0, ctx->stream>>>(cap_chunks, chunks, pred, s_qs, s_qe, s_ts, s_te, s_m, s_b,
+                                                                                   nullptr, min_len, min_ident, hd, ok_head, rec, n_heads,
+                                                                                   n_chunks_dev, *ranked));
+  else if (s_m)
+    SWG_LAUNCH(ctx, "chain_label", chain_label_kernel<LABEL_NT, true, false><<<(unsigned)lb, LABEL_NT, 0, ctx->stream>>>(cap_chunks, chunks, pred, s_qs, s_qe, s_ts, s_te, s_m, s_b,
                                                                              nullptr, min_len, min_ident, hd, ok_head, rec, n_heads,
                                                                              n_chunks_dev));
   else
-    SWG_LAUNCH(ctx, "chain_label", chain_label_kernel<LABEL_NT, false><<<(unsigned)lb, LABEL_NT, 0, ctx->stream>>>(cap_chunks, chunks, pred, s_qs, s_qe, s_ts, s_te, s_m, s_b,
+    SWG_LAUNCH(ctx, "chain_label", chain_label_kernel<LABEL_NT, false, false><<<(unsigned)lb, LABEL_NT, 0, ctx->stream>>>(cap_chunks, chunks, pred, s_qs, s_qe, s_ts, s_te, s_m, s_b,
                                                                              nullptr, min_len, min_ident, hd, ok_head, rec, n_heads,
                                                                              n_chunks_dev));
   SWG_KERNEL_CHECK(ctx);
diff --git a/sweepga_amd/csrc/swg_pair.hip b/sweepga_amd/csrc/swg_pair.hip
--- a/sweepga_amd/csrc/swg_pair.hip
+++ b/sweepga_amd/csrc/swg_pair.hip
@@ -405,6 +405,7 @@
   SpecBlock* chunks;
   uint32_t cap_chunks;
   int chunks_by_place;
+  int ranked;
   uint32_t* long_list;
   uint32_t cap_long;
   PairCounters* C;
@@ -443,6 +444,7 @@
   const uint32_t last_b = mp_ins && (last == NONE || last < m_plus) ? m_plus : last;
   const bool last_long = m - last_b >= LABEL_CAP_ELEMS;
   uint32_t n_long = (mp_long ? 1u : 0u) + (last_long ? 1u : 0u), n_long_lt = 0;
+  bool over = (mp_chunk && m_plus - before_mp > LABEL_FAST_ELEMS) || m - last_b > LABEL_FAST_ELEMS || count > RANKED_MAX_CHUNKS;
   {
     uint32_t carry = NONE;
     for (int c0 = 0; c0 < n_cell; c0 += 64) {
@@ -453,6 +455,7 @@
       const bool lf = v != NONE && b != NONE && v - b >= LABEL_CAP_ELEMS;
       n_long += (uint32_t)__popcll(__ballot(lf));
       n_long_lt += (uint32_t)__popcll(__ballot(lf && v < m_plus));
+      over |= __ballot(v != NONE && b != NONE && v - b > LABEL_FAST_ELEMS) != 0ull;
       carry = (uint32_t)__shfl((int)v, 63 - __clzll(mask), 64);
     }
   }
@@ -467,12 +470,13 @@
     if (lane == 0) atomicOr(&A.C->flags, PF_FALLBACK);
     return;
   }
+  const uint32_t mark = A.ranked && !over ? CHUNK_RANKED : 0u;
   auto emit = [&](uint32_t k, uint32_t b, uint32_t e, bool is_long, uint32_t lpos) {
     SpecBlock d;
     d.bb = a + b;
     d.be = a + e;
     d.ue = d.be;
-    d.pad = b >= m_plus ? 1u : 0u;
+    d.pad = (b >= m_plus ? 1u : 0u) | mark;
     if (is_long) A.long_list[lslot + lpos] = slot + k;
     A.chunks[slot + k] = d;
   };
@@ -1565,6 +1569,11 @@
   const uint8_t* kept_in;
   const uint32_t* chain_base;
   const uint32_t* np;
+  const SpecBlock* chunks;
+  uint32_t cap_chunks;
+  const uint32_t* chunk_pass;
+  uint32_t* rec_w;
+  unsigned long long* ranked_stat;
   uint32_t* fin;
   uint32_t* anum;
   uint32_t* n_out_pair;
@@ -1892,85 +1901,207 @@
     n_deg = block_sum<NT>(cd, ws);
     kP = block_sum<NT>(cp, ws);
   };
-  sweep(false);
-  const uint32_t n_ch = n_pass0 + n_pass1;
-  if (n_ch == 0) {
-    if (tid == 0) A.sum[rk] = sm;
-    return;
-  }
-  if (n_deg) {
-    all_q = n_ch <= 1;
-    all_t = (all_q ? n_ch : n_q) <= 1;
-    __syncthreads();
-    sweep(true);
-  }
-  const uint32_t kM = n_kept - kP;
-  const bool plus_first = pi.first_mem[0] < pi.first_mem[1];
-  sm.n_pass = n_ch;
-  sm.n_kept = n_kept;
-  sm.minmem = n_pass0 && n_pass1 ? (pi.first_mem[0] < pi.first_mem[1] ? pi.first_mem[0] : pi.first_mem[1]) : (n_pass0 ? pi.first_mem[0] : pi.first_mem[1]);
-  if (tid == 0) A.sum[rk] = sm;
-  if (n_kept == 0) return;
-  __syncthreads();
+  const bool plus_first = plus_first0;
+  uint32_t kM = 0, out = 0;
   auto local_number = [&](uint32_t r, bool minus) -> uint32_t {
     if (plus_first) return r + 1;
     return minus ? r - kP + 1 : r + kM + 1;
   };
-  FT_STAMP(0);
-  uint32_t out = 0;
-  for (uint32_t p0 = 0; p0 < m; p0 += NT * US) {
-    uint32_t h[US], idx[US], r[US];
-#pragma unroll
-    for (int u = 0; u < US; ++u) {
-      const uint32_t p = p0 + (uint32_t)u * NT + (uint32_t)tid;
-      h[u] = p < m ? A.hd[a + p] : a;
-      idx[u] = (p < m && !A.fin) ? A.s_idx[a + p] : 0u;
-    }
-#pragma unroll
-    for (int u = 0; u < US; ++u) r[u] = A.head_num[h[u]];
-#pragma unroll
-    for (int u = 0; u < US; ++u) {
-      const uint32_t p = p0 + (uint32_t)u * NT + (uint32_t)tid;
-      uint32_t an = 0;
-      if (p < m && r[u] < NEVER) {
-        an = local_number(r[u], h[u] - a >= m_plus);
-        if (!A.fin) {
-          A.chain[idx[u]] = an;
-          A.status[idx[u]] = SWG_ST_SCAFFOLD;
-        }
-        ++out;
-      } else if (r[u] == NEVER) {
-        an = NEVER;
-      }
-      if (A.fin && p < m) A.fin[a + p] = (an != 0u && an != NEVER) ? ((uint32_t)SWG_ST_SCAFFOLD << 30) | an : 0u;
-      if (A.rescue_d && p < m) A.anum[a + p] = an;
-    }
-  }
-  for (uint32_t p = m + (uint32_t)tid; p < M; p += NT) {
-    if (A.rescue_d) A.anum[a + p] = 0u;
-    if (A.fin) A.fin[a + p] = 0u;
+  const uint32_t slot0 = A.chunks ? a / PAIR_CELL + 2u * rk : 0u;
+  const bool ranked = A.chunks && slot0 < A.cap_chunks && (A.chunks[slot0].pad & CHUNK_RANKED) != 0u;
+  if (ranked) {
+    __shared__ uint32_t rk_beg[RANKED_MAX_CHUNKS], rk_base[RANKED_MAX_CHUNKS + 1], rk_n[3];
+    if (A.ranked_stat && tid == 0) {
+      atomicAdd(&A.ranked_stat[0], 1ull);
+      atomicAdd(&A.ranked_stat[1], (unsigned long long)run.n);
+    }
+    if (tid < 64) {
+      uint32_t lim = run.n / PAIR_CELL + 2u;
+      lim = lim < RANKED_MAX_CHUNKS ? lim : RANKED_MAX_CHUNKS;
+      lim = lim < A.cap_chunks - slot0 ? lim : A.cap_chunks - slot0;
+      uint32_t carry = 0, nck = 0, kp = 0;
+      for (uint32_t j0 = 0; j0 < lim; j0 += 64) {
+        const uint32_t j = j0 + (uint32_t)tid;
+        SpecBlock d;
+        d.ue = d.bb = d.be = d.pad = 0u;
+        if (j < lim) d = A.chunks[slot0 + j];
+        const bool valid = d.be > d.bb;
+        const uint32_t cnt = valid ? A.chunk_pass[slot0 + j] : 0u;
+        uint32_t inc = cnt;
+#pragma unroll
+        for (int dd = 1; dd < 64; dd <<= 1) {
+          const uint32_t t = __shfl_up(inc, dd, 64);
+          if (tid >= dd) inc += t;
+        }
+        if (valid) {
+          rk_beg[j] = d.bb - a;
+          rk_base[j] = carry + inc - cnt;
+        }
+        kp += valid && (d.pad & 1u) == 0u ? cnt : 0u;
+        nck += (uint32_t)__popcll(__ballot(valid));
+        carry += __shfl(inc, 63, 64);
+      }
+#pragma unroll
+      for (int o = 32; o > 0; o >>= 1) kp += __shfl_xor(kp, o, 64);
+      if (tid == 0) {
+        rk_base[nck] = carry;
+        rk_n[0] = nck;
+        rk_n[1] = kp;
+        rk_n[2] = carry;
+      }
+    }
+    __syncthreads();
+    const uint32_t nck = rk_n[0];
+    kP = rk_n[1];
+    n_kept = rk_n[2];
+    kM = n_kept - kP;
+    if (n_kept == 0) {
+      if (tid == 0) A.sum[rk] = sm;
+      return;
+    }
+    sm.n_pass = n_kept;
+    sm.n_kept = n_kept;
+    sm.minmem = kP && kM ? (pi.first_mem[0] < pi.first_mem[1] ? pi.first_mem[0] : pi.first_mem[1]) : (kP ? pi.first_mem[0] : pi.first_mem[1]);
+    if (tid == 0) A.sum[rk] = sm;
+    FT_STAMP(0);
+    uint32_t cj = 0, c_base = rk_base[0], c_next = nck > 1u ? rk_beg[1] : NONE;
+    for (uint32_t p0 = 0; p0 < m; p0 += NT * US) {
+      uint32_t r[US];
+#pragma unroll
+      for (int u = 0; u < US; ++u) {
+        const uint32_t p = p0 + (uint32_t)u * NT + (uint32_t)tid;
+        r[u] = p < m ? A.hd[a + p] : NONE;
+      }
+#pragma unroll
+      for (int u = 0; u < US; ++u) {
+        const uint32_t p = p0 + (uint32_t)u * NT + (uint32_t)tid;
+        if (p >= m) continue;
+        while (p >= c_next) {
+          ++cj;
+          c_base = rk_base[cj];
+          c_next = cj + 1u < nck ? rk_beg[cj + 1u] : NONE;
+        }
+        uint32_t f = 0u;
+        if (r[u] != NONE) {
+          f = ((uint32_t)SWG_ST_SCAFFOLD << 30) | local_number(c_base + r[u], p >= m_plus);
+          ++out;
+        }
+        A.fin[a + p] = f;
+      }
+    }
+    for (uint32_t p = m + (uint32_t)tid; p < M; p += NT) A.fin[a + p] = 0u;
+    if (!A.scaffolds_only && kP > 0 && M > m_plus) {
+      const bool in_lds = kP <= (uint32_t)KP;
+      uint32_t *const g_qs = A.f_qs + a, *const g_qe = A.f_qe + a, *const g_ts = A.rec_w + (size_t)8 * a;
+      for (uint32_t c0 = 0; c0 < kP; c0 += NT) {
+        const uint32_t c = c0 + (uint32_t)tid;
+        uint32_t v_qs = 0, v_qe = 0, v_ts = 0;
+        if (c < kP) {
+          uint32_t lo = 0, hi = nck;
+          while (hi - lo > 1u) {
+            const uint32_t mid = (lo + hi) >> 1;
+            if (rk_base[mid] <= c) lo = mid; else hi = mid;
+          }
+          const uint32_t b = rk_beg[lo], i = c - rk_base[lo];
+          v_qs = A.f_qs[a + b + i];
+          v_qe = A.f_qe[a + b + i];
+          v_ts = A.rec_w[(size_t)8 * (a + b) + i];
+        }
+        if (in_lds) {
+          if (c < kP) {
+            l_qs[c] = v_qs;
+            l_qe[c] = v_qe;
+            l_ts[c] = v_ts;
+          }
+        } else {
+          __syncthreads();
+          if (c < kP) {
+            g_qs[c] = v_qs;
+            g_qe[c] = v_qe;
+            g_ts[c] = v_ts;
+          }
+        }
+      }
+      __syncthreads();
+    }
+  } else {
+    sweep(false);
+    const uint32_t n_ch = n_pass0 + n_pass1;
+    if (n_ch == 0) {
+      if (tid == 0) A.sum[rk] = sm;
+      return;
+    }
+    if (n_deg) {
+      all_q = n_ch <= 1;
+      all_t = (all_q ? n_ch : n_q) <= 1;
+      __syncthreads();
+      sweep(true);
+    }
+    kM = n_kept - kP;
+    sm.n_pass = n_ch;
+    sm.n_kept = n_kept;
+    sm.minmem = n_pass0 && n_pass1 ? (pi.first_mem[0] < pi.first_mem[1] ? pi.first_mem[0] : pi.first_mem[1]) : (n_pass0 ? pi.first_mem[0] : pi.first_mem[1]);
+    if (tid == 0) A.sum[rk] = sm;
+    if (n_kept == 0) return;
+    __syncthreads();
+    FT_STAMP(0);
+    for (uint32_t p0 = 0; p0 < m; p0 += NT * US) {
+      uint32_t h[US], idx[US], r[US];
+#pragma unroll
+      for (int u = 0; u < US; ++u) {
+        const uint32_t p = p0 + (uint32_t)u * NT + (uint32_t)tid;
+        h[u] = p < m ? A.hd[a + p] : a;
+        idx[u] = (p < m && !A.fin) ? A.s_idx[a + p] : 0u;
+      }
+#pragma unroll
+      for (int u = 0; u < US; ++u) r[u] = A.head_num[h[u]];
+#pragma unroll
+      for (int u = 0; u < US; ++u) {
+        const uint32_t p = p0 + (uint32_t)u * NT + (uint32_t)tid;
+        uint32_t an = 0;
+        if (p < m && r[u] < NEVER) {
+          an = local_number(r[u], h[u] - a >= m_plus);
+          if (!A.fin) {
+            A.chain[idx[u]] = an;
+            A.status[idx[u]] = SWG_ST_SCAFFOLD;
+          }
+          ++out;
+        } else if (r[u] == NEVER) {
+          an = NEVER;
+        }
+        if (A.fin && p < m) A.fin[a + p] = (an != 0u && an != NEVER) ? ((uint32_t)SWG_ST_SCAFFOLD << 30) | an : 0u;
+        if (A.rescue_d && p < m) A.anum[a + p] = an;
+      }
+    }
+    for (uint32_t p = m + (uint32_t)tid; p < M; p += NT) {
+      if (A.rescue_d) A.anum[a + p] = 0u;
+      if (A.fin) A.fin[a + p] = 0u;
+    }
   }
   FT_STAMP(1);
   if (!A.scaffolds_only && kP > 0 && M > m_plus) {
     const bool in_lds = kP <= (uint32_t)KP;
+    uint32_t *const g_qs = A.f_qs + a, *const g_qe = A.f_qe + a;
+    uint32_t* const g_ts = ranked ? A.rec_w + (size_t)8 * a : A.f_ts + a;
+    uint32_t* const g_pm = ranked ? g_ts + m : A.f_pm + a;
     uint64_t carry = 0;
     for (uint32_t c0b = 0; c0b < kP; c0b += NT) {
       const uint32_t c = c0b + tid;
-      const uint64_t v = c < kP ? (uint64_t)(in_lds ? l_qe[c] : A.f_qe[a + c]) : 0ull;
+      const uint64_t v = c < kP ? (uint64_t)(in_lds ? l_qe[c] : g_qe[c]) : 0ull;
       uint64_t tot;
       uint64_t ex = block_excl_max<NT>(v, ws64, &tot);
       ex = ex > carry ? ex : carry;
       if (c < kP) {
         const uint32_t pm = (uint32_t)(v > ex ? v : ex);
-        if (in_lds) l_pm[c] = pm; else A.f_pm[a + c] = pm;
+        if (in_lds) l_pm[c] = pm; else g_pm[c] = pm;
       }
       carry = tot > carry ? tot : carry;
     }
     __syncthreads();
-    const uint32_t* __restrict__ c_qs = in_lds ? l_qs : A.f_qs + a;
-    const uint32_t* __restrict__ c_qe = in_lds ? l_qe : A.f_qe + a;
-    const uint32_t* __restrict__ c_ts = in_lds ? l_ts : A.f_ts + a;
-    const uint32_t* __restrict__ c_pm = in_lds ? l_pm : A.f_pm + a;
+    const uint32_t* __restrict__ c_qs = in_lds ? l_qs : g_qs;
+    const uint32_t* __restrict__ c_qe = in_lds ? l_qe : g_qe;
+    const uint32_t* __restrict__ c_ts = in_lds ? l_ts : g_ts;
+    const uint32_t* __restrict__ c_pm = in_lds ? l_pm : g_pm;
     const uint64_t gap = A.gap, max_dev = A.max_dev;
     for (uint32_t p = m_plus + tid; p < M; p += NT) {
       const uint32_t iw = A.s_idx[a + p];
@@ -2728,7 +2859,11 @@
   PairSum* sum = swg_alloc<PairSum>(ctx, n_runs);
   uint32_t* n_out_pair = swg_alloc<uint32_t>(ctx, n_runs);
   const uint32_t cap_chunks = n / PAIR_CELL + 2 * n_runs + 16;
-  SpecBlock* chunks = swg_alloc<SpecBlock>(ctx, cap_chunks);
+  static const bool ranked_knob = !(getenv("SWG_PAIR_RANKED") && atoi(getenv("SWG_PAIR_RANKED")) == 0);
+  const bool ranked = ranked_knob && !limited && !rescue && !need_wid && sweep_assumed_identity && !by_hash;
+  SpecBlock* chunks = swg_alloc<SpecBlock>(ctx, (size_t)cap_chunks + (ranked ? ((size_t)cap_chunks + 3) / 4 : 0));
+  uint32_t* chunk_pass = ranked ? reinterpret_cast<uint32_t*>(chunks + cap_chunks) : nullptr;
+  unsigned long long* ranked_stat = ranked && dbg ? swg_alloc<unsigned long long>(ctx, 2) : nullptr;
   const uint32_t cap_long = n / LABEL_CAP_ELEMS + 1;
   uint32_t* long_list = swg_alloc<uint32_t>(ctx, cap_long);
   SWG_CHECK_ARENA(ctx);
@@ -2743,7 +2878,8 @@
   }
   SWG_HIP(ctx, hipMemsetAsync(n_out_pair, 0, (size_t)n_runs * sizeof(uint32_t), st));
   if (!by_hash) {
-    SWG_HIP(ctx, hipMemsetAsync(chunks, 0, (size_t)cap_chunks * sizeof(SpecBlock), st));
+    SWG_HIP(ctx, hipMemsetAsync(chunks, 0, (size_t)cap_chunks * (sizeof(SpecBlock) + (ranked ? sizeof(uint32_t) : 0)), st));
+    if (ranked_stat) SWG_HIP(ctx, hipMemsetAsync(ranked_stat, 0, 2 * sizeof(unsigned long long), st));
     SWG_HIP(ctx, hipMemsetD32Async(reinterpret_cast<hipDeviceptr_t>(&C->n_chunks), (int)cap_chunks, 1, st));
   }
   PairSortArgs SA{};
@@ -2757,7 +2893,7 @@
   SA.perm = perm;
   SA.orig = plan_in->orig;
   SA.code = code; SA.s_qs = s_qs; SA.s_qe = s_qe; SA.s_ts = s_ts; SA.s_te = s_te; SA.s_m = need_wid ? s_m : nullptr; SA.s_b = need_wid ? s_b : nullptr; SA.s_idx = s_idx; SA.pred = pred;
-  SA.info = info; SA.chunks = chunks; SA.cap_chunks = cap_chunks; SA.chunks_by_place = by_hash ? 0 : 1; SA.long_list = long_list; SA.cap_long = cap_long; SA.C = C; SA.gl_first = gl_first; SA.seq_genome_last = r->seq_genome_last;
+  SA.info = info; SA.chunks = chunks; SA.cap_chunks = cap_chunks; SA.chunks_by_place = by_hash ? 0 : 1; SA.ranked = ranked ? 1 : 0; SA.long_list = long_list; SA.cap_long = cap_long; SA.C = C; SA.gl_first = gl_first; SA.seq_genome_last = r->seq_genome_last;
   if (by_hash) {
     for (int c = 2; c >= 0; --c) {
       if (!ncls[c]) continue;
@@ -2804,9 +2940,10 @@
     SWG_TRY(pair_walk_launch(ctx, cap_chunks, &C->n_chunks, chunks, s_qs, s_qe, s_ts, s_te, cfg->scaffold_gap, bps, pred));
     return SWG_OK;
   };
+  const LabelRanked LR{chunk_pass, s_m, s_b, &C->flags, PF_FALLBACK};
   auto short_label = [&]() -> int {
     return pair_label_launch(ctx, cap_chunks, &C->n_chunks, chunks, pred, s_qs, s_qe, s_ts, s_te, lab_m, lab_b, cfg->min_scaffold_length,
-                             cfg->min_scaffold_identity, hd, ok_head, head_rec, &C->n_heads);
+                             cfg->min_scaffold_identity, hd, ok_head, head_rec, &C->n_heads, ranked ? &LR : nullptr);
   };
   auto long_walk = [&](hipStream_t ls) -> int {
     SWG_TRY(pair_walk_long_launch(ctx, ls, cap_long, &C->n_long, long_list, chunks, n, s_qs, s_qe, s_ts, s_te, cfg->scaffold_gap, bps, pred,
@@ -2914,6 +3051,8 @@
   FA.anum = anum;
   FA.n_out_pair = n_out_pair;
   FA.fin = fin;
+  FA.chunks = ranked ? chunks : nullptr; FA.cap_chunks = cap_chunks; FA.chunk_pass = chunk_pass; FA.rec_w = reinterpret_cast<uint32_t*>(head_rec);
+  FA.ranked_stat = ranked_stat;
   for (int c = 0; c < 3; ++c) {
     const uint32_t nb = c == 2 ? ncls[2] + ncls[3] : ncls[c];
     if (!nb) continue;
@@ -3019,6 +3158,13 @@
     (void)hipMemcpyToSymbol(HIP_SYMBOL(g_fin_t), z, sizeof z);
   }
 #endif
+  if (ranked_stat) {
+    uint64_t hr[2];
+    SWG_TRY(swg_read_scalars(ctx, reinterpret_cast<const uint64_t*>(ranked_stat), hr, 2));
+    fprintf(stderr, "[swg] pair path: ranked form: %llu of %u pairs, %llu of %u records\n", (unsigned long long)hr[0], n_runs, (unsigned long long)hr[1], n);
+  } else if (dbg) {
+    fprintf(stderr, "[swg] pair path: ranked form: off\n");
+  }
   if (stats) {
     stats->n_retained = hc[5];
     stats->n_swept = hc[6];
diff --git a/sweepga_amd/csrc/swg_scaffold_internal.h b/sweepga_amd/csrc/swg_scaffold_internal.h
--- a/sweepga_amd/csrc/swg_scaffold_internal.h
+++ b/sweepga_amd/csrc/swg_scaffold_internal.h
@@ -145,6 +145,15 @@
 }
 #endif
 constexpr uint32_t LABEL_CAP_ELEMS = WALK_CHUNK + BIG_UNIT;
+constexpr uint32_t LABEL_FAST_ELEMS = 1536;
+constexpr uint32_t CHUNK_RANKED = 2u;
+constexpr uint32_t RANKED_MAX_CHUNKS = 128;
+struct LabelRanked {
+  uint32_t* chunk_pass;
+  uint32_t *t_qs, *t_qe;
+  uint32_t* flags;
+  uint32_t fallback_bit;
+};
 
 int pair_walk_launch(swg_ctx* ctx, uint32_t cap_chunks, const uint32_t* n_chunks_dev, const SpecBlock* desc, const uint32_t* s_qs,
                      const uint32_t* s_qe, const uint32_t* s_ts, const uint32_t* s_te, uint64_t max_gap, unsigned long long* bps,
@@ -155,7 +164,7 @@
 int pair_label_launch(swg_ctx* ctx, uint32_t cap_chunks, const uint32_t* n_chunks_dev, const SpecBlock* chunks, const uint32_t* pred,
                       const uint32_t* s_qs, const uint32_t* s_qe, const uint32_t* s_ts, const uint32_t* s_te, const uint32_t* s_m,
                       const uint32_t* s_b, uint64_t min_len, double min_ident, uint32_t* hd, uint8_t* ok_head, HeadRec* rec,
-                      unsigned long long* n_heads);
+                      unsigned long long* n_heads, const LabelRanked* ranked = nullptr);
 int pair_label_long_launch(swg_ctx* ctx, hipStream_t st, uint32_t cap_long, const uint32_t* n_long_dev, const uint32_t* long_list, const SpecBlock* chunks,
                            const uint32_t* pred, const uint32_t* s_qs, const uint32_t* s_qe, const uint32_t* s_ts, const uint32_t* s_te,
                            const uint32_t* s_m, const uint32_t* s_b, uint64_t min_len, double min_ident, uint32_t* hd, uint8_t* ok_head,
```

Result: faster. 13.62 billion mappings/s (median of 6 runs) (+8.2%).
